# SciML/NeuralPDE.jl

Hardware: AMD Instinct MI355X
Metric: collocation-point residual+grad evals/sec, 2D Poisson 4x64 MLP (higher is better)
Workload: dtype f32, hidden-layer forward / dA / dW GEMMs as 3-piece bf16 split products (6 bf16 MFMAs per product block, fp32 accumulation; 24 mantissa bits rebuilt; the five small piece products on an accumulator of their own: zero-mean, a third of the rms error of an fp32-MFMA fmaf chain per GEMM output, tools/m

## Files before the change

### neuralpde.jl_amd/csrc/adam.cpp

```cpp
#include "resident.hpp"
#include "adam_host.hpp"
#include "adam_kernels.hpp"

using namespace pe;

namespace {

int adam_init_f32(pinn_engine& E, const float* theta) {
    const int64_t p = E.ntheta;
    const int K = (int)E.terms.size();
    if (!E.d_opt_theta) {
        E.d_opt_theta = (float*)plat_malloc(sizeof(float) * p);
        E.d_opt_m = (float*)plat_malloc(sizeof(float) * p);
        E.d_opt_v = (float*)plat_malloc(sizeof(float) * p);
        E.d_opt_out = (float*)plat_malloc(sizeof(float) * (p + K));
        E.d_w_over_n = (float*)plat_malloc(sizeof(float) * K);
        if (!E.d_opt_theta || !E.d_opt_m || !E.d_opt_v || !E.d_opt_out || !E.d_w_over_n) return fail("device allocation failed (optimiser state)");
    }
    plat_h2d(E.d_opt_theta, theta, sizeof(float) * p, E.stream);
    plat_memset(E.d_opt_m, 0, sizeof(float) * p, E.stream);
    plat_memset(E.d_opt_v, 0, sizeof(float) * p, E.stream);
    plat_sync(E.stream);
    E.opt_t = 0;
    return 0;
}

int adam_get_f32(pinn_engine& E, float* theta) {
    if (!E.d_opt_theta) return fail("pinn_adam_get: no optimiser state (call pinn_adam_init first)");
    if (plat_d2h(theta, E.d_opt_theta, sizeof(float) * E.ntheta, E.stream)) return fail("D2H copy failed");
    if (plat_sync(E.stream)) return fail(std::string("device error: ") + plat_last_error());
    return 0;
}

bool upload_c12(pinn_engine& E, int nsteps, float beta1, float beta2, std::vector<float>& c12) {
    if (!dev_grow(E.d_c12, E.c12_cap, 2 * (size_t)nsteps, E.stream)) return false;
    c12.resize(2 * (size_t)nsteps);
    for (int s = 0; s < nsteps; ++s) {
        c12[2 * s] = adam_bias(beta1, E.opt_t + s + 1);
        c12[2 * s + 1] = adam_bias(beta2, E.opt_t + s + 1);
    }
    plat_h2d(E.d_c12, c12.data(), sizeof(float) * c12.size(), E.stream);
    return true;
}

int upload_resample_table(pinn_engine& E, int* max_n) {
    std::vector<pk::TrainSampler> samp;
    *max_n = 0;
    for (auto& T : E.terms) {
        if (T.sampler == 0) continue;
        if (!T.emb_cols.empty() || T.ndata > 0 || T.pw_n > 0 || T.coupled >= 0 || T.src_root.size() > (size_t)aux::SRC_MAX) return -1;
        pk::TrainSampler S;
        std::memset(&S, 0, sizeof S);
        S.pts = T.d_pts; S.n = (int)T.n; S.d = T.d; S.kind = T.sampler; S.lb = T.d_lb; S.ub = T.d_ub;
        S.seed = sampler_seed(E, T); S.draw0 = T.draws;
        S.has_src = T.src_root.empty() ? 0 : 1;
        if (S.has_src) {
            S.src.pts = T.d_pts; S.src.N = (int)T.n; S.src.d = T.d; S.src.prog = T.d_src_prog; S.src.nops = (int)T.src_prog.size();
            S.src.nsrc = (int)T.src_root.size();
            for (int j = 0; j < S.src.nsrc; ++j) S.src.root[j] = T.src_root[(size_t)j];
            S.src.out = T.d_src; S.src.data = nullptr;
        }
        *max_n = std::max(*max_n, S.n);
        samp.push_back(S);
// ... 69 lines not shown
    const Group& G = E.groups[0];
    if (G.kind != 0 || !G.spec || G.spec->family != 1 || !G.spec->train) return false;
    if (G.ga.act != pk::ACT_TANH && G.ga.act != pk::ACT_SIGMOID) return false;
    const char* lim = std::getenv("PINN_REDUCE_DIRECT_MAX");
    const int direct_max = lim ? std::atoi(lim) : aux::REDUCE_DIRECT_MAX;
    return G.blocks <= direct_max && G.blocks <= 32 && G.blocks <= E.ncu;
}
bool train_thread_per_element(const pinn_engine& E) {
    return E.groups[0].blocks * 256 >= (int)E.ntheta + (int)E.terms.size() && E.max_contrib <= pk::TRAIN_MAX_CONTRIB;
}
bool train_eligible(pinn_engine& E) {
    if (!train_shape_ok(E) || E.ne != 0 || !E.inv_ok || !E.d_inv_ptr) return false;
    for (auto& T : E.terms)
        if (T.sampler != 0 && (!T.emb_cols.empty() || T.ndata > 0 || T.pw_n > 0 || T.coupled >= 0 || T.src_root.size() > (size_t)aux::SRC_MAX)) return false;
    if (!train_thread_per_element(E) || E.max_inv_pos > pk::TRAIN_MAX_POS) return std::getenv("PINN_TRAIN_GENERAL") != nullptr;
    return true;
}
bool eval_eligible(pinn_engine& E) {
    return E.timing_level == 0 && !std::getenv("PINN_NO_FUSED_EVAL") && train_shape_ok(E) && train_thread_per_element(E);
}

int train_common(pinn_engine& E, pk::TrainArgs& ta, const float* term_w) {
    const int K = (int)E.terms.size(), P = (int)E.ntheta;
    Group& G = E.groups[0];
    if (!E.d_bar) {
        E.d_bar = (unsigned*)plat_malloc(sizeof(unsigned) * 16);
        E.d_sums2 = (float*)plat_malloc(sizeof(float) * 2 * (size_t)std::max(K, 1));
        E.h_flag = (unsigned*)plat_host_alloc(sizeof(unsigned) * 4);
        if (!E.d_bar || !E.d_sums2 || !E.h_flag) return fail("device allocation failed (grid barrier words)");
        E.h_flag[0] = 0;
        E.bar_arrivals = 0;
        plat_memset(E.d_bar, 0, sizeof(unsigned) * 16, E.stream);
        if (plat_sync(E.stream)) return fail(std::string("device error: ") + plat_last_error());
    }
    for (size_t j = 0; j < G.terms.size(); ++j) {
        const int ti = G.terms[j];
        G.ga.terms[j].scale = (float)(2.0 * (double)(term_w ? term_w[ti] : 1.0f) / (double)E.terms[ti].n_norm);
    }
    G.ga.slabs = G.d_slabs;
    G.ga.chain = 0;
    G.active = true;
    G.timed = false;
    G.launched_blocks = G.blocks;
    G.launched_by = 0;
    std::memset(&ta, 0, sizeof ta);
    ta.slabs = G.d_slabs; ta.losspart = G.d_losspart; ta.row_ptr = E.d_gr_ptr; ta.row_ent = E.d_gr_ent;
    ta.slab_floats = G.slab_floats; ta.nblocks = G.blocks;
    ta.P = P; ta.K = K;
    ta.sums2 = E.d_sums2;
    ta.bar = E.d_bar;
    ta.hflag = E.h_flag;
    ta.cached = (train_thread_per_element(E) && E.max_inv_pos <= pk::TRAIN_MAX_POS && std::getenv("PINN_TRAIN_NO_CACHE") == nullptr) ? 1 : 0;
    if (ta.cached && (!E.d_own_r || E.own_blocks != G.blocks)) {
        const std::vector<int> own = train_thread_map(G.row_theta, G.row_ptr, G.row_off, G.blocks, P, K,
                                                      std::getenv("PINN_TRAIN_NO_COALESCE") == nullptr, &E.hist_gid);
        plat_sync(E.stream);
        plat_free(E.d_own_r);
        E.d_own_r = (int*)plat_malloc(sizeof(int) * own.size());
        if (!E.d_own_r) return fail("device allocation failed (training kernel: thread map)");
        plat_h2d(E.d_own_r, own.data(), sizeof(int) * own.size(), E.stream);
        if (plat_sync(E.stream)) return fail(std::string("device error: ") + plat_last_error());
        E.own_blocks = G.blocks;
    }
    ta.own_r = E.d_own_r;
    ta.hist_gid = ta.cached ? E.hist_gid : 0;
    return 0;
}
bool train_timed_out(pinn_engine& E) {
    if (E.h_flag[0] == 0 && std::getenv("PINN_TRAIN_FORCE_TIMEOUT") == nullptr) return false;
    E.h_flag[0] = 0;
    E.bar_arrivals = 0;
    plat_memset(E.d_bar, 0, sizeof(unsigned) * 16, E.stream);
    plat_sync(E.stream);
    E.persistent = false;
    std::fprintf(stderr, "[pinn] the persistent kernel's grid barrier timed out (its workgroups were not all resident: is the device shared?); "
                         "this handle continues with the stand-alone kernels\n");
    return true;
}

int eval_fused(pinn_engine& E, const float* d_theta, float* d_out, const float* term_w, double* lossraw) {
    Group& G = E.groups[0];
    pk::TrainArgs ta;
    if (train_common(E, ta, term_w)) return 1;
    pack_all(E, d_theta, false);
    ta.out = d_out; ta.lossraw = lossraw ? lossraw : E.d_lossraw;
    ta.eval_only = 1; ta.nsteps = 1;
    ta.arrivals0 = E.bar_arrivals;
    E.bar_arrivals += (unsigned)G.blocks;
    G.spec->train(G.ga, ta, G.blocks, E.stream);
    return 0;
}

void opt_snapshot(pinn_engine& E, bool restore) {
    const size_t P = (size_t)E.ntheta;
    float* const state[3] = {E.d_opt_theta, E.d_opt_m, E.d_opt_v};
    for (size_t j = 0; j < 3; ++j) {
        float* const bak = E.d_opt_bak + j * P;
        plat_d2d(restore ? state[j] : bak, restore ? bak : state[j], sizeof(float) * P, E.stream);
    }
}

int adam_steps_train(pinn_engine& E, int nsteps, float lr, float beta1, float beta2, float eps, const float* term_w) {
    const int P = (int)E.ntheta;
    Group& G = E.groups[0];
    pk::TrainArgs ta;
    if (train_common(E, ta, term_w)) return 1;
    std::vector<float> c12;
    if (!upload_c12(E, nsteps, beta1, beta2, c12)) return fail("device allocation failed (bias-correction table)");
    if (!E.d_opt_bak) {
        E.d_opt_bak = (float*)plat_malloc(sizeof(float) * 3 * (size_t)P);
        if (!E.d_opt_bak) return fail("device allocation failed (optimiser snapshot)");
    }
    opt_snapshot(E, false);
    std::vector<unsigned> draws0(E.terms.size());
    for (size_t t = 0; t < E.terms.size(); ++t) draws0[t] = E.terms[t].draws;
    if (plat_sync(E.stream)) return fail(std::string("device error: ") + plat_last_error());
    pack_all(E, E.d_opt_theta, false);
    ta.out = E.d_opt_out; ta.lossraw = E.d_lossraw;
    ta.theta = E.d_opt_theta; ta.m = E.d_opt_m; ta.v = E.d_opt_v;
    ta.lr = lr; ta.b1 = beta1; ta.b2 = beta2; ta.eps = eps;
    ta.inv_ptr = E.d_inv_ptr; ta.inv_pos = E.d_inv_pos; ta.packed = E.netplans[G.net].d_packed;
    ta.w_over_n = E.d_w_over_n;
    bool any_sampler = false;
    for (auto& T : E.terms) any_sampler = any_sampler || T.sampler != 0;
    ta.fenced = any_sampler ? 1 : 0;
    const char* chunk_env = std::getenv("PINN_TRAIN_CHUNK");
    const int TRAIN_CHUNK = (chunk_env && std::atoi(chunk_env) > 0) ? std::atoi(chunk_env) : 4096;
    for (int s0 = 0; s0 < nsteps; s0 += TRAIN_CHUNK) {
        ta.nsteps = std::min(TRAIN_CHUNK, nsteps - s0);
        ta.c12 = E.d_c12 + 2 * (size_t)s0;
        ta.hist = E.d_hist + s0;
        if (any_sampler) {
            int max_n = 0;
            const int ns = upload_resample_table(E, &max_n);
            if (ns < 0) return ns == -2 ? 1 : fail("pinn_adam_steps: a redrawn term of the persistent kernel carries embeddings or per-point data");
            aux::launch_resample((const pk::TrainSampler*)E.d_train_samp, ns, max_n, 0, E.stream);
            for (auto& T : E.terms) if (T.sampler != 0) T.draws += (unsigned)ta.nsteps;
            ta.nsamp = ns;
            ta.samp = (const pk::TrainSampler*)E.d_train_samp;
        }
        ta.arrivals0 = E.bar_arrivals;
        E.bar_arrivals += (unsigned)G.blocks * 2u * (unsigned)ta.nsteps;
        G.spec->train(G.ga, ta, G.blocks, E.stream);
    }
    if (plat_sync(E.stream)) return fail(std::string("device error: ") + plat_last_error());
    if (train_timed_out(E)) {
        opt_snapshot(E, true);
        for (size_t t = 0; t < E.terms.size(); ++t) E.terms[t].draws = draws0[t];
        if (plat_sync(E.stream)) return fail(std::string("device error: ") + plat_last_error());
        return 2;
    }
    E.opt_t += nsteps;
    return 0;
}

int adam_prepare(pinn_engine& E, int nsteps, const float* term_w, const char* who) {
    if (!E.d_opt_theta) return fail(std::string(who) + ": call pinn_adam_init first");
    if (nsteps <= 0) return fail(std::string(who) + ": nsteps must be positive");
    if (ensure_points(E)) return 1;
    const int K = (int)E.terms.size();
    for (auto& T : E.terms)
        if (T.sampler == 3 && T.seed == 0 && E.comm_size > 1)
            return fail(std::string(who) + ": an un-randomised Sobol design (seed 0) is the same on every rank and cannot be sharded; give the sampler a seed");
    if (!dev_grow(E.d_hist, E.hist_cap, (size_t)nsteps, E.stream)) return fail("device allocation failed (loss history)");
    std::vector<float> wn(K);
    for (int k = 0; k < K; ++k) wn[k] = (term_w ? term_w[k] : 1.0f) / (float)E.terms[k].n_norm;
    plat_h2d(E.d_w_over_n, wn.data(), sizeof(float) * K, E.stream);
    return plat_sync(E.stream) ? fail(std::string("device error: ") + plat_last_error()) : 0;
}

int adam_finish(pinn_engine** es, int ndev, int nsteps, double* loss_history, std::vector<float>* last_out = nullptr) {
    {
        pinn_engine& E = *es[0];
        DeviceScope scope(E.device);
        if (loss_history && plat_d2h(loss_history, E.d_hist, sizeof(double) * nsteps, E.stream)) return fail("D2H copy failed");
        if (last_out && plat_d2h(last_out->data(), E.d_opt_out, sizeof(float) * last_out->size(), E.stream)) return fail("D2H copy failed");
    }
    for (int i = 0; i < ndev; ++i) {
        DeviceScope scope(es[i]->device);
        if (plat_sync(es[i]->stream)) return fail(std::string("device error: ") + plat_last_error());
    }
    return 0;
}

}

int pe::eval_one_launch(pinn_engine& E, float* d_out, const float* term_w, double* lossraw) {
    if (!eval_eligible(E)) return 2;
    if (eval_fused(E, E.d_theta, d_out, term_w, lossraw)) return 1;
    if (plat_sync(E.stream)) return fail(std::string("device error: ") + plat_last_error());
    return train_timed_out(E) ? 2 : 0;
}

extern "C" {

int pinn_adam_steps(pinn_handle h, int nsteps, float lr, float beta1, float beta2, float eps, const float* term_w, double* loss_history) {
    if (!h) return fail("null handle");
    pinn_engine& E = *h;
    DeviceScope scope(E.device);
    if (E.comm && !E.comm_per_process && E.comm_size > 1)
        return fail("pinn_adam_steps: the handle belongs to a single-process communicator (pinn_comm_init_all): use pinn_adam_steps_sharded");
    if (E.f64) {
        if (nsteps <= 0) return fail("pinn_adam_steps: nsteps must be positive");
        E.adam_path = 1;
        return f64_adam_steps(E, nsteps, (double)lr, (double)beta1, (double)beta2, (double)eps, term_w, loss_history);
    }
    if (adam_prepare(E, nsteps, term_w, "pinn_adam_steps")) return 1;
    pinn_engine* es[1] = {&E};
    E.adam_path = 1;
    if (train_eligible(E)) {
        E.adam_path = 2;
        const int rc = adam_steps_train(E, nsteps, lr, beta1, beta2, eps, term_w);
        if (rc == 1) return 1;
        if (rc == 0) return adam_finish(es, 1, nsteps, loss_history);
        E.adam_path = 1;
    }
    if (adam_loop(es, 1, nsteps, lr, beta1, beta2, eps, term_w)) return 1;
    std::vector<float> gs;
    if (E.gemm_auto && !E.comm) gs.resize((size_t)E.ntheta + E.terms.size());
    if (adam_finish(es, 1, nsteps, loss_history, gs.empty() ? nullptr : &gs)) return 1;
    if (!gs.empty()) {
        measure_grad_health(E, gs.data(), term_w);
        if (gemm_auto_check(E, E.d_opt_theta, term_w, E.opt_t)) return 1;
// ... 81 lines not shown
```

### neuralpde.jl_amd/csrc/aux_kernels.hpp

```cpp
#pragma once
#include <cstdlib>
#include "aux_limits.hpp"
#include "int_limits.hpp"
#include "plat.hpp"
#include "rprog.hpp"
#include "sample_rules.hpp"

namespace aux {

#ifdef PINN_EMU
#define AUX_DEV inline
#else
#define AUX_DEV __device__ __forceinline__
#endif

struct alignas(16) F4 { float x, y, z, w; };

struct Reduce1Args {
    double* tmp[MAX_GROUPS];
    const float* slabs[MAX_GROUPS];
    const double* losspart[MAX_GROUPS];
    int slab[MAX_GROUPS], nblocks[MAX_GROUPS], nsplit[MAX_GROUPS], nent[MAX_GROUPS], active[MAX_GROUPS];
    int nwpb[MAX_GROUPS];
    int K;
};
struct Reduce2Args {
    float* out;
    float* sums;
    double* lossraw;
    const int* row_ptr;
    const int* row_grp;
    const int* row_ent;
    const double* tmp[MAX_GROUPS];
    int stride[MAX_GROUPS], nsplit[MAX_GROUPS], nent[MAX_GROUPS], active[MAX_GROUPS];
    int ent_active[MAX_GROUPS];
    int ngroups, P, K;
    int skip_grad;
    const int* perm;
};
struct ReduceOneArgs {
    const float* slabs;
    int slab, nblocks, nent;
    const int* ent_theta;
    float* out;
    float* sums;
    double* lossraw;
    int P, K;
    int nloss;
    const double* losspart[MAX_GROUPS];
    int nrows[MAX_GROUPS];
};
constexpr int RONE_CHUNKS = 32, RONE_ENT = 32;

struct ExprArgs {
    const float* pts;
    int N, d, nparams, nparams_estim;
    const float* params;
    int nslots;
    const float* jets[EXPR_MAX_SLOTS];
    float* ubar[EXPR_MAX_SLOTS];
    int nzero;
    float* zero[EXPR_MAX_SLOTS];
    const rp::Instr* prog;
    int nops, out_row;
    float scale;
    double* losspart;
    float* pslab;
    int K, term_id;
    float* resid;
    int loss_only;
    const float* data;
    const float* pw;
};
AUX_DEV float expr_point(int p, const ExprArgs& a, float (&pb)[4]) {
    float v[EXPR_MAX_ROWS], g[EXPR_MAX_ROWS];
    const int R0 = a.d + a.nparams + a.nslots;
    for (int i = 0; i < a.d; ++i) v[i] = a.pts[(size_t)p * a.d + i];
    for (int j = 0; j < a.nparams; ++j) v[a.d + j] = a.params[j];
    for (int s = 0; s < a.nslots; ++s) v[a.d + a.nparams + s] = a.jets[s][p];
    for (int q = 0; q < a.nops; ++q) {
        const rp::Instr ins = a.prog[q];
        const float va = rp::is_nullary(ins.code) ? 0.f : v[ins.a];
        const float vb = rp::is_binary(ins.code) ? v[ins.b] : 0.f;
        v[R0 + q] = (ins.code == rp::OP_DATA) ? a.data[(size_t)(int)ins.imm * a.N + p] : rp::apply<float>(ins.code, va, vb, ins.imm);
    }
    const float r = v[a.out_row];
// ... 132 lines not shown
    }
    for (int j = 0; j < a.nparams_estim; ++j) pb[j] = rbar * g[a.d + j];
    for (int k = 0; k < a.nnodes; ++k) {
        const IntNodeDev nd = a.node[k];
        const float ibar = rbar * g[RI + k] * half[k];
        const int Ri = a.d + a.nparams + nd.nslots;
        for (int q = 0; q < a.Q; ++q) {
            const int site = 1 + k * a.Q + q;
            int_integrand(p, site, nd, a, vi);
            for (int t = 0; t < Ri + nd.nops; ++t) gi[t] = 0.f;
            gi[nd.out_row] = 1.0f;
            for (int t = nd.nops - 1; t >= 0; --t) {
                const rp::Instr ins = a.iprog[nd.prog_off + t];
                if (rp::is_nullary(ins.code)) continue;
                const float vb = rp::is_binary(ins.code) ? vi[ins.b] : 0.f;
                float da, db;
                rp::adjoint<float>(ins.code, vi[ins.a], vb, vi[Ri + t], ins.imm, gi[Ri + t], da, db);
                gi[ins.a] += da;
                if (rp::is_binary(ins.code)) gi[ins.b] += db;
            }
            const float fbar = ibar * a.w[q];
            const size_t sp = (size_t)site * a.N + p;
            for (int c = 0; c < a.C; ++c) {
                const int s = a.node_slot_of_chan[k][c];
                a.ubar[(size_t)c * SN + sp] = s >= 0 ? fbar * gi[a.d + a.nparams + (s - nd.slot0)] : 0.f;
            }
            for (int j = 0; j < a.nparams_estim; ++j) pb[j] += fbar * gi[a.d + j];
        }
    }
    return rs;
}

AUX_DEV void sums_from_double_body(int k, float* out_sums, const double* raw) { out_sums[k] = (float)raw[k]; }
constexpr int PACK_BF_MAX_LAYERS = 16;
struct PackBfArgs {
    const float* theta;
    unsigned* out_fwd;
    unsigned* out_tr;
    int nhh, hp;
    float* packed;
    const int* idx;
    int n_gather;
    int woff[PACK_BF_MAX_LAYERS], nout[PACK_BF_MAX_LAYERS], nin[PACK_BF_MAX_LAYERS];
};
AUX_DEV unsigned bf16_rne(float x) {
    unsigned u;
    __builtin_memcpy(&u, &x, 4);
    if ((u & 0x7FFFFFFFu) > 0x7F800000u) return (u >> 16) | 0x40u;
    u += 0x7FFFu + ((u >> 16) & 1u);
    return u >> 16;
}
AUX_DEV float bf16_val(unsigned h) { const unsigned u = h << 16; float x; __builtin_memcpy(&x, &u, 4); return x; }
AUX_DEV unsigned bf16_piece(float v, int piece) {
    const unsigned h = bf16_rne(v);
    if (piece == 0) return h;
    const float r = v - bf16_val(h);
    const unsigned m = bf16_rne(r);
    if (piece == 1) return m;
    return bf16_rne(r - bf16_val(m));
}
AUX_DEV void pack_bf16_body(int e, const PackBfArgs& a) {
    const int mt = a.hp / 16, kbn = a.hp / 32;
    const int total = a.nhh * mt * kbn * 3 * 256;
    if (e >= 2 * total) return;
    const bool tr = e >= total;
    int r = tr ? e - total : e;
    const int j2 = r & 3; r >>= 2;
    const int lane = r & 63; r >>= 6;
    const int piece = r % 3; r /= 3;
    const int kb = r % kbn; r /= kbn;
    const int ta = r % mt; r /= mt;
    const int hl = r;
    const int g = lane >> 4, c = lane & 15;
    unsigned word = 0;
    for (int half = 0; half < 2; ++half) {
        const int j = 2 * j2 + half;
        const int other = 16 * (2 * kb + (j >> 2)) + 4 * g + (j & 3), mine = 16 * ta + c;
        const int out = tr ? other : mine, in = tr ? mine : other;
        const float v = (out < a.nout[hl] && in < a.nin[hl]) ? a.theta[a.woff[hl] + out + in * a.nout[hl]] : 0.f;
        word |= bf16_piece(v, piece) << (16 * half);
    }
    (tr ? a.out_tr : a.out_fwd)[tr ? e - total : e] = word;
}
struct EmbedArgs {
    const float* upts;
    float* pts;
    int n, du, dx;
    int src[4], is_cos[4];
    double omega[4];
};
AUX_DEV void embed_body(int p, const EmbedArgs& a) {
    if (p >= a.n) return;
    for (int i = 0; i < a.du; ++i) a.pts[(size_t)p * a.dx + i] = a.upts[(size_t)p * a.du + i];
    for (int k = 0; k < a.dx - a.du; ++k) {
        const double ph = a.omega[k] * (double)a.upts[(size_t)p * a.du + a.src[k]];
        a.pts[(size_t)p * a.dx + a.du + k] = (float)(a.is_cos[k] ? cos(ph) : sin(ph));
    }
}
AUX_DEV void pack_body(int i, float* packed, const int* idx, const float* theta) {
    const int j = idx[i];
    packed[i] = (j >= 0) ? theta[j] : 0.f;
}
AUX_DEV void params_body(int j, float* params, const float* theta, const float* defaults, int ne, int p_off) {
    params[j] = (j < ne) ? theta[p_off + j] : defaults[j];
}
#ifdef PINN_EMU
#define AUX_UNROLL8
#else
#define AUX_UNROLL8 _Pragma("unroll 8")
#endif
AUX_DEV void reduce1_body(int e4, int chunk, int g, const Reduce1Args& a) {
    if (!a.active[g] || chunk >= a.nsplit[g]) return;
    const int nb = a.nblocks[g], ns = a.nsplit[g];
    const int per = (nb + ns - 1) / ns;
    const int b0 = chunk * per, b1 = (b0 + per < nb) ? b0 + per : nb;
    double* out = a.tmp[g] + chunk;
    const int nq = a.nent[g] / 4;
    if (e4 < nq) {
        double s0 = 0.0, s1 = 0.0, s2 = 0.0, s3 = 0.0;
        const float* p = a.slabs[g] + 4 * e4;
        AUX_UNROLL8
        for (int b = b0; b < b1; ++b) {
            const F4 q = *reinterpret_cast<const F4*>(p + (size_t)b * a.slab[g]);
            s0 += (double)q.x; s1 += (double)q.y; s2 += (double)q.z; s3 += (double)q.w;
        }
        out[(size_t)(4 * e4) * ns] = s0; out[(size_t)(4 * e4 + 1) * ns] = s1;
        out[(size_t)(4 * e4 + 2) * ns] = s2; out[(size_t)(4 * e4 + 3) * ns] = s3;
    } else if (e4 < nq + a.K) {
        const int k = e4 - nq;
        const double* p = a.losspart[g] + k;
        double s = 0.0;
        AUX_UNROLL8
        for (int wv = b0 * a.nwpb[g]; wv < b1 * a.nwpb[g]; ++wv) s += p[(size_t)wv * a.K];
        out[(size_t)(a.nent[g] + k) * ns] = s;
    }
}
AUX_DEV void reduce_one_chunk(int e4, int ch, const ReduceOneArgs& a, double (&s)[4]) {
    const int per = (a.nblocks + RONE_CHUNKS - 1) / RONE_CHUNKS;
    const int b0 = ch * per, b1 = (b0 + per < a.nblocks) ? b0 + per : a.nblocks;
    s[0] = s[1] = s[2] = s[3] = 0.0;
    const float* p = a.slabs + 4 * e4;
    AUX_UNROLL8
    for (int b = b0; b < b1; ++b) {
        const F4 q = *reinterpret_cast<const F4*>(p + (size_t)b * a.slab);
        s[0] += (double)q.x; s[1] += (double)q.y; s[2] += (double)q.z; s[3] += (double)q.w;
    }
}
AUX_DEV double reduce_one_loss_part(int k, int t, int nthreads, const ReduceOneArgs& a) {
    double s = 0.0;
    for (int i = 0; i < a.nloss; ++i)
        for (int r = t; r < a.nrows[i]; r += nthreads) s += a.losspart[i][(size_t)r * a.K + k];
    return s;
}
AUX_DEV void reduce2_body(int r, const Reduce2Args& a) {
    if (r < a.P) {
        if (a.skip_grad) return;
        double s = 0.0;
        const int i0 = a.row_ptr[r], i1 = a.row_ptr[r + 1];
        for (int i = i0; i < i1; i += 4) {
            const double* t[4];
            int ns[4];
            for (int j = 0; j < 4; ++j) {
                const int ii = (i + j < i1) ? i + j : i;
                const int g = a.row_grp[ii];
                ns[j] = (i + j < i1 && a.ent_active[g]) ? a.nsplit[g] : 0;
                t[j] = a.tmp[g] + (size_t)a.row_ent[ii] * a.nsplit[g];
            }
            for (int j = 0; j < 4; ++j) {
                AUX_UNROLL8
                for (int ch = 0; ch < ns[j]; ++ch) s += t[j][ch];
            }
        }
        a.out[r] = (float)s;
    } else if (r < a.P + a.K) {
        const int k = r - a.P;
        double s = 0.0;
        for (int g = 0; g < a.ngroups; ++g) {
            if (!a.active[g]) continue;
            const double* t = a.tmp[g] + (size_t)(a.nent[g] + k) * a.nsplit[g];
            AUX_UNROLL8
            for (int ch = 0; ch < a.nsplit[g]; ++ch) s += t[ch];
        }
        a.sums[k] = (float)s;
        if (a.lossraw) a.lossraw[k] = s;
    }
}
// ... 16 lines not shown
    } else if (r < a.P + a.K) {
        const int k = r - a.P;
        double s = 0.0;
        for (int g = 0; g < a.ngroups; ++g) {
            if (!a.active[g]) continue;
            const double* p = a1.losspart[g] + k;
            const int nw = a1.nblocks[g] * a1.nwpb[g];
            AUX_UNROLL8
            for (int wv = 0; wv < nw; ++wv) s += p[(size_t)wv * a.K];
        }
        a.sums[k] = (float)s;
        if (a.lossraw) a.lossraw[k] = s;
    }
}

inline bool reduce_is_small(const Reduce1Args& a1, const Reduce2Args& a2) {
    const char* e = std::getenv("PINN_REDUCE_DIRECT_MAX");
    const int lim = e ? std::atoi(e) : REDUCE_DIRECT_MAX;
    for (int g = 0; g < a2.ngroups; ++g)
        if (a1.active[g] && a1.nblocks[g] > lim) return false;
    return true;
}
#ifdef PINN_EMU
inline void launch_pack(float* packed, const int* idx, const float* theta, int n, plat_stream) {
    for (int i = 0; i < n; ++i) pack_body(i, packed, idx, theta);
}
inline void launch_embed(const EmbedArgs& a, plat_stream) {
    for (int p = 0; p < a.n; ++p) embed_body(p, a);
}
inline void launch_params(float* params, const float* theta, const float* defaults, int np, int ne, int p_off, plat_stream) {
    for (int j = 0; j < np; ++j) params_body(j, params, theta, defaults, ne, p_off);
}
inline void launch_pack_bf16(const PackBfArgs& a, plat_stream) {
    const int total = a.nhh * (a.hp / 16) * (a.hp / 32) * 3 * 256;
    for (int i = 0; i < a.n_gather; ++i) pack_body(i, a.packed, a.idx, a.theta);
    for (int e = 0; e < 2 * total; ++e) pack_bf16_body(e, a);
}
inline void launch_sums_from_double(float* out_sums, const double* raw, int K, plat_stream) {
    for (int k = 0; k < K; ++k) sums_from_double_body(k, out_sums, raw);
}
inline void launch_sample(int kind, float* pts, int n_elems, int d, const float* lb, const float* ub, unsigned seed, unsigned draw, plat_stream) {
    for (int e = 0; e < n_elems; ++e) {
        if (kind == 3) sample_sobol_body(e, pts, d, lb, ub, seed, draw);
        else if (kind == 2) sample_lhs_body(e, pts, d, n_elems / d, lb, ub, seed, draw);
        else sample_body(e, pts, d, lb, ub, seed, draw);
    }
}
inline void launch_src(const SrcArgs& a, plat_stream) {
    for (int p = 0; p < a.N; ++p) src_point(p, a);
}
inline void launch_expr(const ExprArgs& a, int nblocks, plat_stream) {
    for (int b = 0; b < nblocks; ++b)
        for (int w = 0; w < 4; ++w) {
            double ls = 0.0;
            double ps[4] = {0, 0, 0, 0};
            for (int l = 0; l < 64; ++l) {
                const int p = (b * 4 + w) * 64 + l;
                if (p >= a.N) continue;
                float pb[4];
                const float r = expr_point(p, a, pb);
                ls += (double)r * (double)r;
                for (int j = 0; j < 4; ++j) ps[j] += (double)pb[j];
            }
            if (!a.resid) {
                a.losspart[(size_t)(b * 4 + w) * a.K + a.term_id] = ls;
                for (int j = 0; j < 4; ++j) a.pslab[(size_t)(b * 4 + w) * 4 + j] = (float)ps[j];
            }
        }
}
inline void launch_int_sites(const IntSitesArgs& a, plat_stream) {
    for (int e = 0; e < a.N * a.nnodes * a.Q; ++e) int_site_body(e, a);
}
inline void launch_int_expr(const IntExprArgs& a, int nblocks, plat_stream) {
    for (int b = 0; b < nblocks; ++b)
        for (int w = 0; w < 4; ++w) {
            double ls = 0.0;
            double ps[4] = {0, 0, 0, 0};
            for (int l = 0; l < 64; ++l) {
                const int p = (b * 4 + w) * 64 + l;
                if (p >= a.N) continue;
                float pb[4];
                const float r = int_expr_point(p, a, pb);
                ls += (double)r * (double)r;
                for (int j = 0; j < 4; ++j) ps[j] += (double)pb[j];
            }
            if (!a.resid) {
                a.losspart[(size_t)(b * 4 + w) * a.K + a.term_id] = ls;
                for (int j = 0; j < 4; ++j) a.pslab[(size_t)(b * 4 + w) * 4 + j] = (float)ps[j];
            }
        }
}
inline void launch_reduce_one(const ReduceOneArgs& a, plat_stream) {
    for (int e4 = 0; e4 < a.nent / 4; ++e4) {
        double tot[4] = {0, 0, 0, 0}, s[4];
        for (int ch = 0; ch < RONE_CHUNKS; ++ch) {
            reduce_one_chunk(e4, ch, a, s);
            for (int e = 0; e < 4; ++e) tot[e] += s[e];
        }
        for (int e = 0; e < 4; ++e)
            if (a.ent_theta[4 * e4 + e] >= 0) a.out[a.ent_theta[4 * e4 + e]] = (float)tot[e];
    }
    for (int k = 0; k < a.K; ++k) {
        double part[256], s = 0.0;
        for (int t = 0; t < 256; ++t) part[t] = reduce_one_loss_part(k, t, 256, a);
        for (int st = 128; st >= 1; st >>= 1)
            for (int t = 0; t < st; ++t) part[t] += part[t + st];
        s = part[0];
        a.sums[k] = (float)s;
        if (a.lossraw) a.lossraw[k] = s;
    }
}
inline void launch_reduce(const Reduce1Args& a1, const Reduce2Args& a2, int max_n1, int max_split, plat_stream) {
    if (reduce_is_small(a1, a2)) {
        for (int r = 0; r < a2.P + a2.K; ++r) reduce_direct_body(r, a1, a2);
        return;
    }
    for (int g = 0; g < a2.ngroups; ++g)
        for (int ch = 0; ch < max_split; ++ch)
            for (int e = 0; e < max_n1; ++e) reduce1_body(e, ch, g, a1);
    for (int r = 0; r < a2.P + a2.K; ++r) reduce2_body(r, a2);
}
#else
__global__ void k_pack(float* packed, const int* idx, const float* theta, int n) {
    const int i = blockIdx.x * blockDim.x + threadIdx.x;
    if (i < n) pack_body(i, packed, idx, theta);
}
__global__ void k_params(float* params, const float* theta, const float* defaults, int np, int ne, int p_off) {
    const int j = threadIdx.x;
    if (j < np) params_body(j, params, theta, defaults, ne, p_off);
}
__global__ void k_sample(float* pts, int n_elems, int d, const float* lb, const float* ub, unsigned seed, unsigned draw) {
    const int e = blockIdx.x * blockDim.x + threadIdx.x;
    if (e < n_elems) sample_body(e, pts, d, lb, ub, seed, draw);
}
__global__ void k_sample_lhs(float* pts, int n_elems, int d, const float* lb, const float* ub, unsigned seed, unsigned draw) {
    const int e = blockIdx.x * blockDim.x + threadIdx.x;
    if (e < n_elems) sample_lhs_body(e, pts, d, n_elems / d, lb, ub, seed, draw);
}
__global__ void k_sample_sobol(float* pts, int n_elems, int d, const float* lb, const float* ub, unsigned seed, unsigned draw) {
    const int e = blockIdx.x * blockDim.x + threadIdx.x;
    if (e < n_elems) sample_sobol_body(e, pts, d, lb, ub, seed, draw);
}
inline void launch_sample(int kind, float* pts, int n_elems, int d, const float* lb, const float* ub, unsigned seed, unsigned draw, plat_stream st) {
    if (kind == 3) hipLaunchKernelGGL(k_sample_sobol, dim3((n_elems + 255) / 256), dim3(256), 0, st, pts, n_elems, d, lb, ub, seed, draw);
// ... 4 lines not shown
    __shared__ double sh[5][256];
    const int p = blockIdx.x * 256 + threadIdx.x;
    float pb[4] = {0.f, 0.f, 0.f, 0.f};
    float r = 0.f;
    if (p < a.N) r = expr_point(p, a, pb);
    if (a.resid) return;
    sh[0][threadIdx.x] = (double)r * (double)r;
    for (int j = 0; j < 4; ++j) sh[1 + j][threadIdx.x] = (double)pb[j];
    __syncthreads();
    if (threadIdx.x < 20) {
        const int w = threadIdx.x & 3, q = threadIdx.x >> 2;
        double s = 0.0;
        for (int l = 0; l < 64; ++l) s += sh[q][w * 64 + l];
        if (q == 0) a.losspart[(size_t)(blockIdx.x * 4 + w) * a.K + a.term_id] = s;
        else a.pslab[(size_t)(blockIdx.x * 4 + w) * 4 + (q - 1)] = (float)s;
    }
}
__global__ void k_reduce1(const Reduce1Args a) {
    reduce1_body((int)(blockIdx.x * blockDim.x + threadIdx.x), (int)blockIdx.y, (int)blockIdx.z, a);
}
__global__ void k_reduce2(const Reduce2Args a) {
    reduce2_body((int)(blockIdx.x * blockDim.x + threadIdx.x), a);
}
inline void launch_pack(float* packed, const int* idx, const float* theta, int n, plat_stream st) {
    hipLaunchKernelGGL(k_pack, dim3((n + 255) / 256), dim3(256), 0, st, packed, idx, theta, n);
}
__global__ void k_embed(const EmbedArgs a) { embed_body((int)(blockIdx.x * blockDim.x + threadIdx.x), a); }
inline void launch_embed(const EmbedArgs& a, plat_stream st) {
    hipLaunchKernelGGL(k_embed, dim3((a.n + 255) / 256), dim3(256), 0, st, a);
}
inline void launch_params(float* params, const float* theta, const float* defaults, int np, int ne, int p_off, plat_stream st) {
    if (np > 0) hipLaunchKernelGGL(k_params, dim3(1), dim3(64), 0, st, params, theta, defaults, np, ne, p_off);
}
__global__ void k_pack_bf16(const PackBfArgs a) {
    const int e = (int)(blockIdx.x * blockDim.x + threadIdx.x);
    if (e < a.n_gather) pack_body(e, a.packed, a.idx, a.theta);
    else pack_bf16_body(e - a.n_gather, a);
}
inline void launch_pack_bf16(const PackBfArgs& a, plat_stream st) {
    const int total = a.nhh * (a.hp / 16) * (a.hp / 32) * 3 * 256;
    hipLaunchKernelGGL(k_pack_bf16, dim3((a.n_gather + 2 * total + 255) / 256), dim3(256), 0, st, a);
}
__global__ void k_sums_from_double(float* out_sums, const double* raw, int K) {
    const int k = (int)(blockIdx.x * blockDim.x + threadIdx.x);
    if (k < K) sums_from_double_body(k, out_sums, raw);
}
inline void launch_sums_from_double(float* out_sums, const double* raw, int K, plat_stream st) {
    hipLaunchKernelGGL(k_sums_from_double, dim3((K + 63) / 64), dim3(64), 0, st, out_sums, raw, K);
}
__global__ void __launch_bounds__(256) k_src(const SrcArgs a) {
    const int p = blockIdx.x * 256 + threadIdx.x;
    if (p < a.N) src_point(p, a);
}
inline void launch_src(const SrcArgs& a, plat_stream st) {
    hipLaunchKernelGGL(k_src, dim3((a.N + 255) / 256), dim3(256), 0, st, a);
}
inline void launch_expr(const ExprArgs& a, int nblocks, plat_stream st) {
    hipLaunchKernelGGL(k_expr, dim3(nblocks), dim3(256), 0, st, a);
}
__global__ void __launch_bounds__(256) k_int_sites(const IntSitesArgs a) { int_site_body((int)(blockIdx.x * 256 + threadIdx.x), a); }
inline void launch_int_sites(const IntSitesArgs& a, plat_stream st) {
    hipLaunchKernelGGL(k_int_sites, dim3((a.N * a.nnodes * a.Q + 255) / 256), dim3(256), 0, st, a);
}
__global__ void __launch_bounds__(256) k_int_expr(const IntExprArgs a) {
    __shared__ double sh[5][256];
    const int p = blockIdx.x * 256 + threadIdx.x;
    float pb[4] = {0.f, 0.f, 0.f, 0.f};
    float r = 0.f;
    if (p < a.N) r = int_expr_point(p, a, pb);
    if (a.resid) return;
    sh[0][threadIdx.x] = (double)r * (double)r;
    for (int j = 0; j < 4; ++j) sh[1 + j][threadIdx.x] = (double)pb[j];
    __syncthreads();
    if (threadIdx.x < 20) {
        const int w = threadIdx.x & 3, q = threadIdx.x >> 2;
        double s = 0.0;
        for (int l = 0; l < 64; ++l) s += sh[q][w * 64 + l];
        if (q == 0) a.losspart[(size_t)(blockIdx.x * 4 + w) * a.K + a.term_id] = s;
        else a.pslab[(size_t)(blockIdx.x * 4 + w) * 4 + (q - 1)] = (float)s;
    }
}
inline void launch_int_expr(const IntExprArgs& a, int nblocks, plat_stream st) {
    hipLaunchKernelGGL(k_int_expr, dim3(nblocks), dim3(256), 0, st, a);
}
__global__ void __launch_bounds__(256) k_reduce_one(const ReduceOneArgs a) {
    __shared__ double sh[RONE_CHUNKS][RONE_ENT + 1];
    const int tid = (int)threadIdx.x;
    const int nentblocks = (a.nent + RONE_ENT - 1) / RONE_ENT;
    if ((int)blockIdx.x < nentblocks) {
        const int j = tid & 7, ch = tid >> 3;
        const int e4 = (int)blockIdx.x * (RONE_ENT / 4) + j;
        double s[4] = {0.0, 0.0, 0.0, 0.0};
        if (4 * e4 < a.nent) reduce_one_chunk(e4, ch, a, s);
        for (int e = 0; e < 4; ++e) sh[ch][4 * j + e] = s[e];
        __syncthreads();
        if (tid < RONE_ENT) {
            const int ent = (int)blockIdx.x * RONE_ENT + tid;
            if (ent < a.nent) {
                double tot = 0.0;
                for (int c2 = 0; c2 < RONE_CHUNKS; ++c2) tot += sh[c2][tid];
                const int th = a.ent_theta[ent];
                if (th >= 0) a.out[th] = (float)tot;
            }
        }
    } else {
        const int k = (int)blockIdx.x - nentblocks;
        double* part = &sh[0][0];
        part[tid] = reduce_one_loss_part(k, tid, 256, a);
        __syncthreads();
        for (int st = 128; st >= 1; st >>= 1) {
            if (tid < st) part[tid] += part[tid + st];
            __syncthreads();
        }
        if (tid == 0) {
            a.sums[k] = (float)part[0];
            if (a.lossraw) a.lossraw[k] = part[0];
        }
    }
}
inline void launch_reduce_one(const ReduceOneArgs& a, plat_stream st) {
    hipLaunchKernelGGL(k_reduce_one, dim3((a.nent + RONE_ENT - 1) / RONE_ENT + a.K), dim3(256), 0, st, a);
}
__global__ void k_reduce_direct(const Reduce1Args a1, const Reduce2Args a2) {
    reduce_direct_body((int)(blockIdx.x * blockDim.x + threadIdx.x), a1, a2);
}
inline void launch_reduce(const Reduce1Args& a1, const Reduce2Args& a2, int max_n1, int max_split, plat_stream st) {
    if (reduce_is_small(a1, a2)) {
        hipLaunchKernelGGL(k_reduce_direct, dim3((a2.P + a2.K + 63) / 64), dim3(64), 0, st, a1, a2);
        return;
    }
    hipLaunchKernelGGL(k_reduce1, dim3((max_n1 + 255) / 256, max_split, a2.ngroups), dim3(256), 0, st, a1);
    hipLaunchKernelGGL(k_reduce2, dim3((a2.P + a2.K + 255) / 256), dim3(256), 0, st, a2);
}
#endif

}
```

### neuralpde.jl_amd/csrc/comm.cpp

```cpp
#include "engine_types.hpp"

using namespace pe;

#ifndef PINN_EMU
#include <dlfcn.h>
#include <rccl/rccl.h>

namespace {
struct Rccl {
    void* lib = nullptr;
    ncclResult_t (*GetUniqueId)(ncclUniqueId*) = nullptr;
    ncclResult_t (*CommInitRank)(ncclComm_t*, int, ncclUniqueId, int) = nullptr;
    ncclResult_t (*CommInitAll)(ncclComm_t*, int, const int*) = nullptr;
    ncclResult_t (*CommDestroy)(ncclComm_t) = nullptr;
    ncclResult_t (*AllReduce)(const void*, void*, size_t, ncclDataType_t, ncclRedOp_t, ncclComm_t, hipStream_t) = nullptr;
    ncclResult_t (*GroupStart)() = nullptr;
    ncclResult_t (*GroupEnd)() = nullptr;
    const char* (*GetErrorString)(ncclResult_t) = nullptr;
    std::string err;
};
Rccl& rccl() {
    static Rccl R = [] {
        Rccl r;
        for (const char* name : {"librccl.so.1", "librccl.so", "/opt/rocm/lib/librccl.so.1"}) {
// ... 251 lines not shown
        rc = comm_all_reduce_f64(es, 1, vec, E.ntheta + (int64_t)E.terms.size());
    }
    E.stream = saved;
    return rc;
}

int pinn_loss_grad_sharded_f64(pinn_handle* hs, int ndev, const double* theta, int64_t p, const double* term_w, double* term_losses, double* grad) {
    if (!hs || ndev < 1 || !theta) return fail("pinn_loss_grad_sharded_f64: null argument");
    for (int i = 0; i < ndev; ++i) {
        if (!hs[i] || !hs[i]->comm || hs[i]->comm_size != ndev || hs[i]->comm_rank != i)
            return fail("pinn_loss_grad_sharded_f64: pass the handles of one pinn_comm_init_all communicator, in rank order");
        if (!hs[i]->f64) return fail("pinn_loss_grad_sharded_f64: every handle must be in the float64 evaluation mode");
        if (p != hs[i]->ntheta) return fail("pinn_loss_grad_sharded_f64: theta length mismatch");
    }
    const int64_t P = hs[0]->ntheta;
    const int K = (int)hs[0]->terms.size();
    std::vector<double*> vec(ndev);
    for (int i = 0; i < ndev; ++i) {
        pinn_engine& E = *hs[i];
        DeviceScope scope(E.device);
        if (check_shards(E)) return 1;
        if (f64_eval_sharded_local(E, theta, term_w, &vec[i])) return 1;
    }
    if (comm_all_reduce_f64(hs, ndev, vec.data(), P + K)) return 1;
    std::vector<double> out((size_t)(P + K));
    {
        pinn_engine& E0 = *hs[0];
        DeviceScope scope(E0.device);
        if (plat_d2h(out.data(), vec[0], sizeof(double) * (size_t)(P + K), E0.stream)) return fail("D2H copy failed");
    }
    for (int i = 0; i < ndev; ++i) {
        DeviceScope scope(hs[i]->device);
        if (plat_sync(hs[i]->stream)) return fail(std::string("device error: ") + plat_last_error());
    }
    if (term_losses) for (int k = 0; k < K; ++k) term_losses[k] = out[(size_t)P + k] / (double)hs[0]->terms[k].n_norm;
    if (grad) std::memcpy(grad, out.data(), sizeof(double) * (size_t)P);
    return 0;
}

int pinn_loss_grad_sharded_device(pinn_handle h, const float* d_theta, const float* term_w, float* d_out, void* stream) {
    if (!h || !d_theta || !d_out) return fail("pinn_loss_grad_sharded_device: null argument");
    pinn_engine& E = *h;
    if (!E.comm) return fail("pinn_loss_grad_sharded_device: the handle has no communicator (pinn_comm_init_rank / pinn_comm_init_all)");
    DeviceScope scope(E.device);
    if (check_shards(E)) return 1;
    plat_stream st = (plat_stream)stream;
    plat_stream saved = E.stream;
    E.stream = st;
    int rc = run_loss_grad(E, d_theta, d_out, term_w, -1, true);
    E.stream = saved;
    if (rc) return rc;
    E.timing_valid = E.timing_level >= 2;
    if (!E.comm_per_process && E.comm_size > 1)
        return fail("pinn_loss_grad_sharded_device: the handle belongs to a single-process communicator (pinn_comm_init_all): use pinn_loss_grad_sharded");
    {
        pinn_engine* es[1] = {&E};
        float* vec[1] = {d_out};
        double* raw[1] = {E.d_lossraw};
        E.stream = st;
        rc = comm_all_reduce(es, 1, vec, raw);
        E.stream = saved;
        if (rc) return rc;
    }
    sums_from_double(d_out + E.ntheta, E.d_lossraw, (int)E.terms.size(), st);
    return 0;
}
// ... 2 lines not shown
    if (!hs || ndev < 1 || !theta) return fail("pinn_loss_grad_sharded: null argument");
    for (int i = 0; i < ndev; ++i) {
        if (!hs[i] || !hs[i]->comm || hs[i]->comm_size != ndev || hs[i]->comm_rank != i)
            return fail("pinn_loss_grad_sharded: pass the handles of one pinn_comm_init_all communicator, in rank order");
        if (i > 0 && hs[i]->comm != hs[0]->comm
#ifndef PINN_EMU
            && false
#endif
        ) return fail("pinn_loss_grad_sharded: handles of different communicators");
    }
    const int64_t P = hs[0]->ntheta;
    const int K = (int)hs[0]->terms.size();
    for (int i = 0; i < ndev; ++i) {
        pinn_engine& E = *hs[i];
        DeviceScope scope(E.device);
        if (check_shards(E) || upload_theta(E, theta, p)) return 1;
        if (run_loss_grad(E, E.d_theta, E.d_out, term_w, -1, false)) return 1;
    }
    {
        std::vector<float*> vec(ndev);
        std::vector<double*> raw(ndev);
        for (int i = 0; i < ndev; ++i) { vec[i] = hs[i]->d_out; raw[i] = hs[i]->d_lossraw; }
        if (comm_all_reduce(hs, ndev, vec.data(), raw.data())) return 1;
    }
    pinn_engine& E0 = *hs[0];
    {
        DeviceScope scope(E0.device);
        if (plat_d2h(E0.hp_out, E0.d_out, sizeof(float) * (P + K), E0.stream)) return fail("D2H copy failed");
        if (plat_d2h(E0.hp_raw, E0.d_lossraw, sizeof(double) * K, E0.stream)) return fail("D2H copy failed");
    }
    for (int i = 0; i < ndev; ++i) {
        DeviceScope scope(hs[i]->device);
        if (plat_sync(hs[i]->stream)) return fail(std::string("device error: ") + plat_last_error());
    }
    if (term_losses)
        for (int k = 0; k < K; ++k) term_losses[k] = E0.hp_raw[k] / (double)E0.terms[k].n_norm;
    if (grad) std::memcpy(grad, E0.hp_out, sizeof(float) * P);
    return 0;
}

}
```

### neuralpde.jl_amd/csrc/engine.cpp

```cpp
#include "resident.hpp"
#include "aux_kernels.hpp"

#ifdef PINN_EMU
namespace wv {
thread_local void (*emu_barrier_hook)(void*) = nullptr;
thread_local void* emu_barrier_ctx = nullptr;
thread_local void (*emu_grid_hook)(void*) = nullptr;
thread_local void* emu_grid_ctx = nullptr;
}
#endif

namespace pk {
std::deque<SpecInfo>& registry() {
    static std::deque<SpecInfo> r;
    return r;
}
std::deque<PairInfo>& pair_registry() {
    static std::deque<PairInfo> r;
    return r;
}
}

namespace pe {
thread_local std::string g_err;
// ... 35 lines not shown
    aux::launch_int_sites(a, E.stream);
}
void eval_sources(pinn_engine& E, Term& T) {
    if (T.src_root.empty() || T.coupled >= 0) return;
    aux::SrcArgs a;
    std::memset(&a, 0, sizeof a);
    a.pts = T.d_pts; a.N = (int)T.n; a.d = T.d; a.prog = T.d_src_prog; a.nops = (int)T.src_prog.size();
    a.nsrc = (int)T.src_root.size();
    for (int j = 0; j < a.nsrc; ++j) a.root[j] = T.src_root[j];
    a.out = T.d_src;
    a.data = T.d_data;
    if (T.ndata > 0 && T.data_n != T.n) return;
    aux::launch_src(a, E.stream);
}

}

void pe::redraw_term(pinn_engine& E, Term& T, bool sources) {
    aux::launch_sample(T.sampler, user_pts(T), (int)(T.n * T.d_user), T.d_user, T.d_lb, T.d_ub, sampler_seed(E, T), T.draws++, E.stream);
    embed_points(E, T);
    if (sources) eval_sources(E, T);
}

int pe::ensure_points(pinn_engine& E) {
    for (size_t t = 0; t < E.terms.size(); ++t) {
        if (!E.terms[t].d_pts || E.terms[t].n <= 0)
            return fail("term " + std::to_string(t) + " has no collocation points (call pinn_set_points first)");
        if (E.terms[t].ndata > 0 && E.terms[t].data_n != E.terms[t].n)
            return fail("term " + std::to_string(t) + " uses per-point data channels but none are installed for its current point set (call pinn_set_point_data after pinn_set_points)");
    }
    return 0;
}

void pe::pack_all(pinn_engine& E, const float* d_theta, bool packed_fresh) {
    const float* th = d_theta ? d_theta : E.d_theta;
    for (size_t n = 0; n < E.nets.size(); ++n) {
        NetPlan& NP = E.netplans[n];
        if (!NP.spec) continue;
        if (NP.spec->family == 3) { NP.cur = th + E.nets[n].theta_off; continue; }
        NP.cur = NP.d_packed;
        const bool gather = !packed_fresh;
        if (gather && !NP.spec->BFX) aux::launch_pack(NP.d_packed, NP.d_pack_idx, th, NP.npacked, E.stream);
        if (NP.spec->BFX) {
            const Net& N = E.nets[n];
            aux::PackBfArgs pa;
            std::memset(&pa, 0, sizeof pa);
            pa.theta = th; pa.out_fwd = (unsigned*)(NP.d_packed + NP.spec->OFF_WB); pa.out_tr = (unsigned*)(NP.d_packed + NP.spec->OFF_WTB);
            pa.nhh = NP.spec->NHH; pa.hp = NP.spec->HP;
            pa.packed = NP.d_packed; pa.idx = NP.d_pack_idx; pa.n_gather = gather ? NP.spec->OFF_WB : 0;
            if (pa.nhh > aux::PACK_BF_MAX_LAYERS) return;
            int o = N.theta_off;
            for (size_t j = 0; j + 1 < N.sizes.size(); ++j) {
                if (j >= 1 && j <= (size_t)pa.nhh) { pa.woff[j - 1] = o; pa.nin[j - 1] = N.sizes[j]; pa.nout[j - 1] = N.sizes[j + 1]; }
                o += N.sizes[j + 1] * N.sizes[j] + N.sizes[j + 1];
            }
            aux::launch_pack_bf16(pa, E.stream);
        }
    }
    for (auto& G : E.groups) G.ga.packed = E.netplans[G.net].cur;
    aux::launch_params(E.d_params, th, E.d_defaults, E.np, E.ne, E.p_theta_off, E.stream);
}

namespace {

aux::ExprArgs expr_args(pinn_engine& E, Coupled& Cp, float scale, float* resid) {
    Term& T = E.terms[Cp.term];
    aux::ExprArgs a;
    std::memset(&a, 0, sizeof a);
    a.pts = T.d_pts; a.N = (int)T.n; a.d = T.d; a.nparams = E.np; a.nparams_estim = E.ne; a.params = E.d_params;
    a.nslots = (int)T.slots.size();
    std::vector<std::vector<char>> used(Cp.nets.size());
    for (size_t i = 0; i < Cp.nets.size(); ++i) used[i].assign(E.groups[Cp.groups[i]].spec->C, 0);
    for (int si = 0; si < a.nslots; ++si) {
        const int i = Cp.slot_net[si], ch = T.chan_of_slot[si];
        a.jets[si] = Cp.d_jets[i] + (size_t)ch * T.n;
        a.ubar[si] = Cp.d_ubar[i] + (size_t)ch * T.n;
        used[i][ch] = 1;
    }
    for (size_t i = 0; i < Cp.nets.size(); ++i)
        for (size_t ch = 0; ch < used[i].size(); ++ch)
            if (!used[i][ch] && a.nzero < aux::EXPR_MAX_SLOTS) a.zero[a.nzero++] = Cp.d_ubar[i] + ch * T.n;
    a.prog = Cp.d_prog; a.nops = (int)T.ops.size(); a.out_row = T.out_row; a.scale = scale;
    a.losspart = Cp.d_losspart; a.pslab = Cp.d_pslab; a.K = (int)E.terms.size(); a.term_id = Cp.term; a.resid = resid;
    a.data = T.d_data;
    a.pw = (T.pw_n == T.n && T.pw_n > 0) ? T.d_pw : nullptr;
    return a;
}

aux::IntExprArgs int_expr_args(pinn_engine& E, Coupled& Cp, float scale, float* resid) {
// ... 23 lines not shown
    return a;
}

int upload_int_rule(pinn_engine& E, int q) {
    std::vector<double> xi((size_t)q), w((size_t)q);
    const double PI = 3.14159265358979323846264338327950288;
    for (int i = 0; i < q; ++i) {
        double x = -std::cos(PI * (i + 0.75) / (q + 0.5)), dp = 1.0;
        for (int it = 0; it < 100; ++it) {
            double p0 = 1.0, p1 = x;
            for (int n = 2; n <= q; ++n) { const double p2 = ((2.0 * n - 1.0) * x * p1 - (n - 1.0) * p0) / n; p0 = p1; p1 = p2; }
            dp = q * (x * p1 - p0) / (x * x - 1.0);
            const double dx = p1 / dp;
            x -= dx;
            if (std::fabs(dx) < 1e-16) break;
        }
        {
            double p0 = 1.0, p1 = x;
            for (int n = 2; n <= q; ++n) { const double p2 = ((2.0 * n - 1.0) * x * p1 - (n - 1.0) * p0) / n; p0 = p1; p1 = p2; }
            dp = q * (x * p1 - p0) / (x * x - 1.0);
        }
        xi[(size_t)i] = x;
        w[(size_t)i] = 2.0 / ((1.0 - x * x) * dp * dp);
    }
    std::vector<float> wf(w.begin(), w.end());
    if (!E.d_int_xi) {
        E.d_int_xi = (double*)plat_malloc(sizeof(double) * aux::INT_MAX_Q);
        E.d_int_w = (float*)plat_malloc(sizeof(float) * aux::INT_MAX_Q);
        if (!E.d_int_xi || !E.d_int_w) return fail("device allocation failed (quadrature rule)");
    }
    plat_h2d(E.d_int_xi, xi.data(), sizeof(double) * q, E.stream);
    plat_h2d(E.d_int_w, wf.data(), sizeof(float) * q, E.stream);
    if (plat_sync(E.stream)) return fail(std::string("device error: ") + plat_last_error());
    return 0;
}

}

int pe::run_loss_grad(pinn_engine& E, const float* d_theta, float* d_out, const float* term_w, int only_term , bool timing,
                  double* lossraw , bool packed_fresh, bool loss_only, float* d_sums) {
    if (!d_sums) d_sums = d_out + E.ntheta;
    if (ensure_points(E)) return 1;
    const int K = (int)E.terms.size();
    const bool phase_ev = timing && E.timing_level >= 2;
    auto group_ev = [&](size_t g) { return timing && E.timing_level >= 1 && (E.timing_group < 0 || E.timing_group == (int)g); };
    if (phase_ev) plat_event_record(E.ev0, E.stream);
    pack_all(E, d_theta, packed_fresh);
    if (phase_ev) plat_event_record(E.ev1, E.stream);
    aux::Reduce1Args a1;
    aux::Reduce2Args a2;
    std::memset(&a1, 0, sizeof a1);
    std::memset(&a2, 0, sizeof a2);
    int max_n1 = 1, max_split = 1;
    auto scale_of = [&](int ti) -> float {
        const float w = term_w ? term_w[ti] : 1.0f;
        const bool on = (only_term < 0 || only_term == ti);
        return on ? (float)(2.0 * (double)w / (double)E.terms[ti].n_norm) : 0.f;
    };
    int nfused_active = 0;
    bool all_small = true;
    for (auto& G : E.groups) {
        bool on = false;
        for (int ti : G.terms) on = on || (only_term < 0 || only_term == ti);
        if (G.kind == 0 && on) {
            ++nfused_active;
            const int per_round = G.max_blocks * (G.spec->family == 2 ? 1 : 4);
            if (2 * G.ga.ntiles > 3 * per_round) all_small = false;
        }
    }
    static const bool want_concurrent = std::getenv("PINN_CONCURRENT_GROUPS") != nullptr;
    const bool concurrent = want_concurrent && nfused_active >= 2 && all_small;
    static const bool no_chain = std::getenv("PINN_NO_CHAIN") != nullptr;
    const bool no_merge = std::getenv("PINN_NO_MERGE") != nullptr;
    const bool may_merge = !no_merge && !no_chain && !concurrent && only_term < 0;
    int nforked = 0;
    int nslabsets = 0, slabset_group = -1;
    if (concurrent) plat_event_record(E.ev_fork, E.stream);
    for (size_t g = 0; g < E.groups.size(); ++g) {
        Group& G = E.groups[g];
        bool any = false;
// ... 46 lines not shown
            ga_one.sub_terms0 = (int)G.terms.size();
            ga_one.sub_tiles0 = G.ga.ntiles;
            ga_one.ntiles = G.ga.ntiles + T2.ga.ntiles;
            ga_one.scratch = mu->d_scratch;
            ga_one.scr_stride = mu->pair->SCR;
            ga_one.losspart = mu->d_losspart;
            a1.losspart[g] = mu->d_losspart;
            ga_one.chain = 0;
            blocks = std::max(1, std::min(loss_only ? E.ncu * mu->pair->WG_FWD : mu->max_blocks, ga_one.ntiles));
            ga_launch = &ga_one;
        }
        G.launched_blocks = blocks;
        G.launched_by = (int)g;
        const int epe = G.spec->family == 1 ? 4 : 1;
        const int nsplit_g = std::max(1, std::min(REDUCE_SPLIT, (int)std::ceil(std::sqrt((double)blocks / epe))));
        a1.slab[g] = G.slab_floats; a1.nblocks[g] = blocks; a1.nsplit[g] = nsplit_g; a1.nent[g] = nent; a1.active[g] = any; a1.nwpb[g] = G.spec->NW;
        a2.stride[g] = nent + K; a2.nsplit[g] = nsplit_g; a2.nent[g] = nent; a2.active[g] = any;
        a2.ent_active[g] = any && !chained && !loss_only;
        if (!any) continue;
        if (a2.ent_active[g]) { ++nslabsets; slabset_group = (int)g; }
        max_n1 = std::max(max_n1, nent / 4 + K);
        max_split = std::max(max_split, nsplit_g);
        if (G.kind == 1) {
            G.spec->launch(G.ga, (G.use_rec && !loss_only) ? pk::MODE_FWDREC : pk::MODE_FWD,
                           std::max(1, std::min(E.ncu * G.spec->WG_FWD, G.spec->family == 1 ? (G.ga.ntiles + 3) / 4 : G.ga.ntiles)), E.stream);
            continue;
        }
        if (G.kind == 2) continue;
        plat_stream st = E.stream;
        const bool forked = concurrent && nforked++ > 0;
        if (forked) {
            st = E.aux_stream[nforked % 2];
            plat_stream_wait_event(st, E.ev_fork);
        }
        if (group_ev(g)) plat_event_record(G.ev_a, st);
        if (merged_head) mu->pair->launch(*ga_launch, loss_only ? pk::MODE_LOSS : pk::MODE_FUSED, blocks, st);
        else if (loss_only) {
            const int tiles = ga_launch->ntiles;
            const int fb = std::max(1, std::min(E.ncu * G.spec->WG_FWD, G.spec->family == 1 ? (tiles + 3) / 4 : tiles));
            a1.nblocks[g] = fb;
            G.launched_blocks = fb;
            G.spec->launch(*ga_launch, pk::MODE_LOSS, fb, st);
        } else G.spec->launch(*ga_launch, pk::MODE_FUSED, blocks, st);
        if (group_ev(g)) plat_event_record(G.ev_b, st);
        G.timed = group_ev(g);
        if (forked) {
            plat_event_record(E.ev_join[g], st);
            plat_stream_wait_event(E.stream, E.ev_join[g]);
        }
    }
    bool coupled_active = false;
    for (size_t c = 0; c < E.coupled.size(); ++c) {
        Coupled& Cp = E.coupled[c];
        const int g = (int)(E.groups.size() + c);
        const bool on = (only_term < 0 || only_term == Cp.term);
        const int nsplit = std::min(REDUCE_SPLIT, Cp.blocks);
        const int nent = loss_only ? 0 : 16;
        a1.tmp[g] = Cp.d_tmp; a1.slabs[g] = Cp.d_pslab; a1.losspart[g] = Cp.d_losspart;
        a1.slab[g] = 16; a1.nblocks[g] = Cp.blocks; a1.nsplit[g] = nsplit; a1.nent[g] = nent; a1.active[g] = on; a1.nwpb[g] = 4;
        a2.tmp[g] = Cp.d_tmp; a2.stride[g] = nent + K; a2.nsplit[g] = nsplit; a2.nent[g] = nent; a2.active[g] = on; a2.ent_active[g] = on && !loss_only;
        bool groups_active = false;
        for (int gi : Cp.groups) groups_active = groups_active || E.groups[gi].active;
        if (!groups_active) continue;
        coupled_active = true;
        if (Cp.tail >= 0) {
            Group& G = E.groups[Cp.groups[Cp.tail]];
// ... 8 lines not shown
            if (group_ev((size_t)Cp.groups[Cp.tail])) plat_event_record(G.ev_b, E.stream);
            G.timed = group_ev((size_t)Cp.groups[Cp.tail]);
            continue;
        }
        max_n1 = std::max(max_n1, nent / 4 + K);
        max_split = std::max(max_split, nsplit);
        if (!E.terms[Cp.term].inodes.empty()) {
            aux::IntExprArgs ia = int_expr_args(E, Cp, scale_of(Cp.term), nullptr);
            ia.loss_only = loss_only ? 1 : 0;
            aux::launch_int_expr(ia, Cp.blocks, E.stream);
            continue;
        }
        aux::ExprArgs ea = expr_args(E, Cp, scale_of(Cp.term), nullptr);
        ea.loss_only = loss_only ? 1 : 0;
        aux::launch_expr(ea, Cp.blocks, E.stream);
    }
    for (size_t g = 0; g < E.groups.size() && !loss_only; ++g) {
        Group& G = E.groups[g];
        if (G.kind != 1 || !G.active) continue;
        if (group_ev(g)) plat_event_record(G.ev_a, E.stream);
        G.spec->launch(G.ga, G.use_rec ? pk::MODE_GRADREC : pk::MODE_GRADIN, G.blocks, E.stream);
        if (group_ev(g)) plat_event_record(G.ev_b, E.stream);
        G.timed = group_ev(g);
    }
    if (phase_ev) plat_event_record(E.ev2, E.stream);
    a1.K = K;
    a2.out = d_out; a2.sums = d_sums; a2.lossraw = lossraw ? lossraw : E.d_lossraw; a2.row_ptr = E.d_gr_ptr; a2.row_grp = E.d_gr_grp; a2.row_ent = E.d_gr_ent;
    a2.ngroups = (int)(E.groups.size() + E.coupled.size()); a2.P = (int)E.ntheta; a2.K = K;
    a2.skip_grad = loss_only ? 1 : 0;
    a2.perm = std::getenv("PINN_NO_REDUCE_PERM") ? nullptr : E.d_red_perm;
    const bool no_reduce_one = std::getenv("PINN_NO_REDUCE_ONE") != nullptr;
    const Group* RG = (nslabsets == 1 && !coupled_active && !loss_only && !no_reduce_one) ? &E.groups[slabset_group] : nullptr;
    const bool one_kernel = ((RG && RG->d_ent_theta && RG->ent_covers_theta) || (loss_only && !no_reduce_one)) && !aux::reduce_is_small(a1, a2);
    if (one_kernel) {
        aux::ReduceOneArgs ro;
        std::memset(&ro, 0, sizeof ro);
        if (RG) { ro.slabs = RG->d_slabs; ro.slab = RG->slab_floats; ro.nblocks = a1.nblocks[slabset_group]; ro.nent = RG->nent; ro.ent_theta = RG->d_ent_theta; }
        ro.out = d_out; ro.sums = d_sums; ro.lossraw = a2.lossraw; ro.P = (int)E.ntheta; ro.K = K;
        for (int g = 0; g < a2.ngroups; ++g)
            if (a1.active[g]) { ro.losspart[ro.nloss] = a1.losspart[g]; ro.nrows[ro.nloss] = a1.nblocks[g] * a1.nwpb[g]; ++ro.nloss; }
        aux::launch_reduce_one(ro, E.stream);
    } else {
        aux::launch_reduce(a1, a2, max_n1, max_split, E.stream);
    }
    if (phase_ev) plat_event_record(E.ev3, E.stream);
    { const std::string e = jit_take_launch_error(); if (!e.empty()) return fail(e); }
    return 0;
}

void pe::sums_from_double(float* d_out_sums, const double* d_raw, int K, plat_stream st) { aux::launch_sums_from_double(d_out_sums, d_raw, K, st); }

int pe::upload_theta(pinn_engine& E, const float* theta, int64_t p) {
    if (p != E.ntheta) return fail("theta length " + std::to_string(p) + " != ntheta " + std::to_string(E.ntheta));
    std::memcpy(E.hp_theta, theta, sizeof(float) * p);
    if (plat_h2d(E.d_theta, E.hp_theta, sizeof(float) * p, E.stream)) return fail(std::string("H2D copy of theta failed: ") + plat_last_error());
    return 0;
}

extern "C" {

const char* pinn_backend(void) { return plat_name(); }
int pinn_abi_version(void) { return 1; }
const char* pinn_last_error(void) { return g_err.c_str(); }

int pinn_create(const char* descriptor, pinn_handle* out) { return pinn_create_on(descriptor, -1, out); }

int pinn_create_on(const char* descriptor, int device, pinn_handle* out) {
    if (!descriptor || !out) return fail("pinn_create: null argument");
    *out = nullptr;
    std::string err;
    if (plat_init(err)) return fail(err);
    if (device >= plat_device_count()) return fail("pinn_create_on: device " + std::to_string(device) + " does not exist (" + std::to_string(plat_device_count()) + " visible)");
    const int dev = device < 0 ? plat_get_device() : device;
    DeviceScope scope(dev);
    std::unique_ptr<pinn_engine> E(new pinn_engine());
    E->device = dev;
    if (const char* gm = std::getenv("PINN_GEMM")) {
        if (std::string(gm) == "fp32") E->gemm = pk::GEMM_FP32;
        else if (std::string(gm) == "split") E->gemm = pk::GEMM_SPLIT;
        else return fail(std::string("PINN_GEMM must be \"split\" or \"fp32\", not \"") + gm + "\"");
    }
    if (parse_descriptor(descriptor, *E)) return 1;
    E->terms0 = E->terms;
    E->ncu = plat_num_cus();
    E->stream = plat_stream_create();
    const int K = (int)E->terms.size();
    E->d_theta = (float*)plat_malloc(sizeof(float) * E->ntheta);
    E->d_params = (float*)plat_malloc(sizeof(float) * pk::MAX_PARAMS);
    E->d_defaults = (float*)plat_malloc(sizeof(float) * pk::MAX_PARAMS);
    E->d_lossraw = (double*)plat_malloc(sizeof(double) * K);
    E->d_out = (float*)plat_malloc(sizeof(float) * (E->ntheta + K));
    plat_event_create(E->ev0); plat_event_create(E->ev1); plat_event_create(E->ev2); plat_event_create(E->ev3);
    plat_event_create(E->ev_fork);
    for (auto& e : E->ev_join) plat_event_create(e);
    for (auto& st : E->aux_stream) st = plat_stream_create();
    if (!E->d_theta || !E->d_params || !E->d_defaults || !E->d_lossraw || !E->d_out) {
        pinn_destroy(E.release());
        return fail("device allocation failed");
    }
    plat_h2d(E->d_defaults, E->p_defaults32.data(), sizeof(float) * pk::MAX_PARAMS, E->stream);
    E->hp_theta = (float*)plat_host_alloc(sizeof(float) * (2 * E->ntheta + K + 2) + sizeof(double) * K);
    if (!E->hp_theta) {
        pinn_destroy(E.release());
        return fail("pinned host allocation failed");
    }
    E->hp_out = E->hp_theta + E->ntheta;
    E->hp_raw = (double*)(E->hp_theta + ((2 * E->ntheta + K + 1) / 2) * 2);
    bool any_int = false;
    for (auto& T : E->terms) any_int = any_int || !T.inodes.empty();
    if ((any_int && upload_int_rule(*E, E->int_q)) || build_plan(*E)) {
        const std::string msg = g_err;
        pinn_destroy(E.release());
        g_err = msg;
        return 1;
    }
    *out = E.release();
    return 0;
}

int pinn_destroy(pinn_handle h) {
    if (!h) return 0;
    pinn_engine& E = *h;
    DeviceScope scope(E.device);
    pinn_comm_destroy(h);
    plat_sync(E.stream);
    hmc_free(E);
    lbfgs_free(E);
    ens_free(E);
    f64_destroy(E);
    free_plan(E);
    for (auto& T : E.terms) { plat_free(T.d_pts); plat_free(T.d_upts); plat_free(T.d_resid); plat_free(T.d_lb); plat_free(T.d_ub); plat_free(T.d_data); plat_free(T.d_pw); }
    plat_free(E.d_opt_theta); plat_free(E.d_opt_m); plat_free(E.d_opt_v); plat_free(E.d_opt_out); plat_free(E.d_w_over_n); plat_free(E.d_hist); plat_free(E.d_c12); plat_free(E.d_bar); plat_free(E.d_sums2); plat_free(E.d_own_r); plat_free(E.d_train_samp); plat_free(E.d_opt_bak); plat_host_free(E.h_flag);
    plat_free(E.d_theta); plat_free(E.d_params); plat_free(E.d_defaults); plat_free(E.d_lossraw);
    plat_free(E.d_int_xi); plat_free(E.d_int_w);
    plat_free(E.d_out); plat_free(E.d_phi_pts); plat_free(E.d_phi_out); plat_free(E.d_phi_scr);
    plat_host_free(E.hp_theta);
    plat_event_destroy(E.ev0); plat_event_destroy(E.ev1); plat_event_destroy(E.ev2); plat_event_destroy(E.ev3);
    plat_event_destroy(E.ev_fork);
    for (auto& e : E.ev_join) plat_event_destroy(e);
    for (auto& st : E.aux_stream) plat_stream_destroy(st);
    if (E.own_stream) plat_stream_destroy(E.stream);
    delete h;
    return 0;
}

int pinn_num_terms(pinn_handle h) { return h ? (int)h->terms.size() : -1; }
int64_t pinn_num_theta(pinn_handle h) { return h ? h->ntheta : -1; }

static int term_installed(pinn_engine& E, int term);
static int set_points_impl(pinn_handle h, int term, const float* pts, int64_t n, int64_t n_norm, bool device) {
    if (!h) return fail("null handle");
    pinn_engine& E = *h;
    DeviceScope scope(E.device);
    if (term < 0 || term >= (int)E.terms.size()) return fail("pinn_set_points: term index out of range");
    if (!pts || n <= 0) return fail("pinn_set_points: empty point set (the reference's mean(abs2, .) over an empty set is NaN; refusing)");
    Term& T = E.terms[term];
    if (n * T.d >= (int64_t)1 << 31) return fail("pinn_set_points: point set too large for 32-bit indexing; shard it");
    const int64_t S = T.sites();
    if (S > 1 && n * S * std::max(T.d, aux::INT_MAX_C) >= (int64_t)1 << 31)
        return fail("pinn_set_points: the site set of integral term " + std::to_string(term) + " (" + std::to_string(n) + " points x (1 + " +
                    std::to_string(T.inodes.size()) + " integral node(s) x " + std::to_string(T.int_q) + " quadrature nodes) = " + std::to_string(n * S) +
                    " sites) exceeds what one launch group takes (32-bit indexing of its jet channels); shard the point set or lower integral_nodes");
    if (n > T.pts_cap || !T.d_pts) {
        plat_sync(E.stream);
        plat_free(T.d_pts);
        plat_free(T.d_upts);
        T.d_upts = nullptr;
// ... 65 lines not shown
    if (Cp.cap_blocks < Cp.blocks) {
        plat_free(Cp.d_losspart); plat_free(Cp.d_pslab);
        Cp.d_losspart = (double*)plat_malloc(sizeof(double) * (size_t)Cp.blocks * 4 * K);
        Cp.d_pslab = (float*)plat_malloc(sizeof(float) * (size_t)Cp.blocks * 16);
        if (!Cp.d_losspart || !Cp.d_pslab) return fail("device allocation failed (coupled partials)");
        plat_memset(Cp.d_losspart, 0, sizeof(double) * (size_t)Cp.blocks * 4 * K, E.stream);
        plat_memset(Cp.d_pslab, 0, sizeof(float) * (size_t)Cp.blocks * 16, E.stream);
        plat_sync(E.stream);
        Cp.cap_blocks = Cp.blocks;
    }
    for (int gi : Cp.groups) retile(E, gi);
    return 0;
}
int pinn_set_points(pinn_handle h, int term, const float* pts, int64_t n, int64_t n_norm) { return set_points_impl(h, term, pts, n, n_norm, false); }
int pinn_set_points_device(pinn_handle h, int term, const float* d_pts, int64_t n, int64_t n_norm) { return set_points_impl(h, term, d_pts, n, n_norm, true); }
int pinn_set_points_f64(pinn_handle h, int term, const double* pts, int64_t n, int64_t n_norm) {
    if (!h || !pts || n <= 0) return fail("pinn_set_points_f64: null argument / empty point set");
    if (term < 0 || term >= (int)h->terms.size()) return fail("pinn_set_points_f64: term index out of range");
    auto p32 = as<float>(pts, (size_t)n * h->terms[term].d_user);
    if (set_points_impl(h, term, p32.get(), n, n_norm, false)) return 1;
    if (!h->f64) return 0;
    DeviceScope scope(h->device);
    return f64_set_points(*h, term, pts, n);
}

extern "C++" int pe::eval_and_sync(pinn_engine& E, float* d_out, const float* term_w, double* lossraw, bool timing) {
    E.eval_path = 1;
    if (ensure_points(E)) return 1;
    const int one = eval_one_launch(E, d_out, term_w, lossraw);
    if (one == 1) return 1;
    if (one == 0) { E.eval_path = 2; return 0; }
    if (run_loss_grad(E, E.d_theta, d_out, term_w, -1, timing, lossraw, false, false)) return 1;
    if (plat_sync(E.stream)) return fail(std::string("device error: ") + plat_last_error());
    return 0;
}

static int loss_grad_f32(pinn_engine& E, const float* theta, const float* term_w, double* term_losses, float* grad) {
    const int K = (int)E.terms.size();
    if (upload_theta(E, theta, E.ntheta)) return 1;
    if (grad) {
        if (eval_and_sync(E, E.hp_out, term_w, E.hp_raw, true)) return 1;
    } else {
        if (run_loss_grad(E, E.d_theta, E.hp_out, term_w, -1, true, E.hp_raw, false, true)) return 1;
        if (plat_sync(E.stream)) return fail(std::string("device error: ") + plat_last_error());
    }
    E.timing_valid = E.timing_level >= 2;
    if (term_losses)
        for (int k = 0; k < K; ++k) term_losses[k] = E.hp_raw[k] / (double)E.terms[k].n_norm;
    if (grad) std::memcpy(grad, E.hp_out, sizeof(float) * E.ntheta);
    if (grad && E.gemm_auto) {
        std::vector<float> gs((size_t)E.ntheta + K);
        std::memcpy(gs.data(), E.hp_out, sizeof(float) * E.ntheta);
        for (int k = 0; k < K; ++k) gs[(size_t)E.ntheta + k] = (float)E.hp_raw[k];
        measure_grad_health(E, gs.data(), term_w);
        if (gemm_auto_check(E, E.d_theta, term_w, ++E.eval_count)) return 1;
    }
    return 0;
}

static void loglik_from_sse(const pinn_engine& E, const double* stds, const double* sse, double* loglik, double* grad_std) {
    const int K = (int)E.terms.size();
    double ll = 0.0;
    for (int k = 0; k < K; ++k) {
        const double N = (double)E.terms[k].n, sd = stds[k];
        ll += -0.5 * N * std::log(2.0 * 3.14159265358979323846) - N * std::log(sd) - sse[k] / (2.0 * sd * sd);
        if (grad_std) grad_std[k] = -N / sd + sse[k] / (sd * sd * sd);
    }
    *loglik = ll;
}
static int loglik_f64(pinn_engine& E, const double* theta, const double* stds, double* loglik, double* grad_theta, double* grad_std) {
    const int K = (int)E.terms.size();
    std::vector<double> w(K), L(K), g(grad_theta ? (size_t)E.ntheta : 0);
    for (int k = 0; k < K; ++k) w[k] = (double)E.terms[k].n_norm / (2.0 * stds[k] * stds[k]);
    if (f64_eval(E, theta, w.data(), L.data(), grad_theta ? g.data() : nullptr)) return 1;
    for (int k = 0; k < K; ++k) L[k] *= (double)E.terms[k].n_norm;
    loglik_from_sse(E, stds, L.data(), loglik, grad_std);
    if (grad_theta) for (int64_t i = 0; i < E.ntheta; ++i) grad_theta[i] = -g[(size_t)i];
    return 0;
}

static int loglik_f32(pinn_engine& E, const float* theta, const double* stds, double* loglik, float* grad_theta, double* grad_std) {
    const int K = (int)E.terms.size();
    std::vector<float> w(K);
    for (int k = 0; k < K; ++k) w[k] = (float)((double)E.terms[k].n_norm / (2.0 * stds[k] * stds[k]));
    if (upload_theta(E, theta, E.ntheta)) return 1;
    if (run_loss_grad(E, E.d_theta, E.hp_out, w.data(), -1, false, E.hp_raw)) return 1;
    if (plat_sync(E.stream)) return fail(std::string("device error: ") + plat_last_error());
    loglik_from_sse(E, stds, E.hp_raw, loglik, grad_std);
    if (grad_theta)
        for (int64_t i = 0; i < E.ntheta; ++i) grad_theta[i] = -E.hp_out[i];
    return 0;
}

static int term_grads_f64(pinn_engine& E, const double* theta, double* term_losses, double* term_grads) {
    const int K = (int)E.terms.size();
    const int64_t p = E.ntheta;
    std::vector<double> w(K), L(K);
    for (int k = 0; k < K; ++k) {
        for (int j = 0; j < K; ++j) w[j] = (j == k) ? 1.0 : 0.0;
        if (f64_eval(E, theta, w.data(), L.data(), term_grads + (size_t)k * p)) return 1;
        if (term_losses) term_losses[k] = L[k];
    }
    return 0;
}

static int term_grads_f32(pinn_engine& E, const float* theta, double* term_losses, float* term_grads) {
    const int K = (int)E.terms.size();
    const int64_t p = E.ntheta;
    if (upload_theta(E, theta, p)) return 1;
    for (int k = 0; k < K; ++k) {
        if (run_loss_grad(E, E.d_theta, E.hp_out, nullptr, k, false, E.hp_raw)) return 1;
        if (plat_sync(E.stream)) return fail(std::string("device error: ") + plat_last_error());
        std::memcpy(term_grads + (size_t)k * p, E.hp_out, sizeof(float) * p);
        if (term_losses) term_losses[k] = E.hp_raw[k] / (double)E.terms[k].n_norm;
    }
    return 0;
}

int pinn_loss_grad_device(pinn_handle h, const float* d_theta, const float* term_w, float* d_out, void* stream) {
    if (!h || !d_theta || !d_out) return fail("pinn_loss_grad_device: null argument");
    pinn_engine& E = *h;
    DeviceScope scope(E.device);
    const int K = (int)E.terms.size();
    plat_stream user = (plat_stream)stream;
    plat_stream saved = E.stream;
    E.stream = user;
    int rc = E.f64 ? f64_eval_from_device_f32(E, d_theta, term_w, d_out, true) : run_loss_grad(E, d_theta, d_out, term_w, -1, true);
    E.stream = saved;
    if (rc && g_err.empty()) return fail("pinn_loss_grad_device failed");
    E.timing_valid = (rc == 0) && E.timing_level >= 2;
    return rc;
}

int pinn_loss_grad_device_f64(pinn_handle h, const double* d_theta, const float* term_w, double* d_out, void* stream) {
    if (!h || !d_theta || !d_out) return fail("pinn_loss_grad_device_f64: null argument");
    pinn_engine& E = *h;
    if (!E.f64) return fail("pinn_loss_grad_device_f64: the handle is not in the float64 evaluation mode (pinn_set_option(h, \"precision\", \"f64\"))");
    DeviceScope scope(E.device);
    plat_stream saved = E.stream;
    E.stream = (plat_stream)stream;
    const int rc = f64_eval_from_device_f64(E, d_theta, term_w, d_out);
    E.stream = saved;
    if (rc && g_err.empty()) return fail("pinn_loss_grad_device_f64 failed");
    return rc;
}
// ... 15 lines not shown
    if (!h || group < 0 || group >= (int)h->groups.size()) return -1;
    return h->groups[group].launched_by;
}

static int residual_f32(pinn_engine& E, int term, const float* theta, float* r) {
    Term& T = E.terms[term];
    if (!T.d_pts) return fail("pinn_residual: term has no points");
    if (upload_theta(E, theta, E.ntheta)) return 1;
    pack_all(E);
    jit_take_launch_error();
    if (T.resid_cap < T.n) {
        plat_free(T.d_resid);
        T.d_resid = (float*)plat_malloc(sizeof(float) * T.n);
        T.resid_cap = T.n;
        if (!T.d_resid) return fail("device allocation failed (residual)");
    }
    if (T.coupled >= 0) {
        Coupled& Cp = E.coupled[T.coupled];
        for (int gi : Cp.groups) {
            Group& G = E.groups[gi];
            pk::GroupArgs ga = G.ga;
            int j = 0;
            for (size_t q = 0; q < G.terms.size(); ++q) if (G.terms[q] == term) j = (int)q;
            ga.nterms = 1;
            ga.terms[0] = G.ga.terms[j];
            ga.terms[0].tile0 = 0;
            ga.ntiles = ga.terms[0].ntiles;
            G.spec->launch(ga, pk::MODE_FWD, std::max(1, std::min(E.ncu * G.spec->WG_FWD, G.spec->family == 1 ? (ga.ntiles + 3) / 4 : ga.ntiles)), E.stream);
        }
        if (!T.inodes.empty()) aux::launch_int_expr(int_expr_args(E, Cp, 0.f, T.d_resid), Cp.blocks, E.stream);
        else aux::launch_expr(expr_args(E, Cp, 0.f, T.d_resid), Cp.blocks, E.stream);
        if (plat_d2h(r, T.d_resid, sizeof(float) * T.n, E.stream)) return fail("D2H copy failed");
        if (plat_sync(E.stream)) return fail(std::string("device error: ") + plat_last_error());
        { const std::string le = jit_take_launch_error(); if (!le.empty()) return fail("pinn_residual: " + le); }
        return 0;
    }
    Group& G = E.groups[T.group];
    pk::GroupArgs ga = G.ga;
    ga.nterms = 1;
    ga.terms[0] = G.ga.terms[T.slot_in_group];
    ga.terms[0].tile0 = 0;
    ga.terms[0].out = T.d_resid;
    ga.ntiles = ga.terms[0].ntiles;
    const int blocks = std::max(1, std::min(E.ncu * G.spec->WG_FWD, G.spec->family == 1 ? (ga.ntiles + 3) / 4 : ga.ntiles));
    G.spec->launch(ga, pk::MODE_RESID, blocks, E.stream);
    if (plat_d2h(r, T.d_resid, sizeof(float) * T.n, E.stream)) return fail("D2H copy failed");
    if (plat_sync(E.stream)) return fail(std::string("device error: ") + plat_last_error());
    { const std::string le = jit_take_launch_error(); if (!le.empty()) return fail("pinn_residual: " + le); }
    return 0;
}

static int forward_jets(pinn_engine& E, int net, const pk::SpecInfo* sp, const float* theta, const float* pts, int64_t n) {
    const Net& N = E.nets[net];
    if (!E.netplans[net].spec) return fail("network is not used by any term");
    if (sp->family != E.netplans[net].spec->family || sp->PACKED != E.netplans[net].spec->PACKED)
        return fail("internal: forward kernel and the network's packed weight image disagree");
    if (upload_theta(E, theta, E.ntheta)) return 1;
    pack_all(E);
    jit_take_launch_error();
    if (E.phi_cap < n || E.phi_chan < sp->C) {
        plat_sync(E.stream);
        plat_free(E.d_phi_pts); plat_free(E.d_phi_out);
        E.phi_cap = std::max(E.phi_cap, n);
        E.phi_chan = std::max(E.phi_chan, sp->C);
        E.d_phi_pts = (float*)plat_malloc(sizeof(float) * E.phi_cap * 8);
        E.d_phi_out = (float*)plat_malloc(sizeof(float) * E.phi_cap * E.phi_chan);
        if (!E.d_phi_pts || !E.d_phi_out) { E.phi_cap = 0; E.phi_chan = 0; return fail("device allocation failed (phi)"); }
    }
    if (!N.emb_idx.empty()) {
        const std::vector<float> feats = N.features(pts, n);
        plat_h2d(E.d_phi_pts, feats.data(), sizeof(float) * feats.size(), E.stream);
        plat_sync(E.stream);
    } else
        plat_h2d(E.d_phi_pts, pts, sizeof(float) * n * N.sizes[0], E.stream);
    pk::GroupArgs ga;
    std::memset(&ga, 0, sizeof ga);
    ga.packed = E.netplans[net].cur;
    ga.params = E.d_params;
    ga.nterms = 1;
    ga.nterms_total = 1;
// ... 20 lines not shown
        ga.dgm_modes = N.sizes[1];
        ga.dgm_npad = ga.ntiles * 64;
        ga.dgm_nparams = N.nparams();
    }
    const int blocks = std::max(1, std::min(E.ncu * sp->WG_FWD, sp->family == 1 ? (ga.ntiles + 3) / 4 : ga.ntiles));
    sp->launch(ga, pk::MODE_FWD, blocks, E.stream);
    { const std::string le = jit_take_launch_error(); if (!le.empty()) return fail("forward kernel: " + le); }
    return 0;
}

static int net_eval_f32(const char* who, pinn_engine& E, int net, const float* theta, const float* pts, int64_t n, int order, const int* axes, float* out) {
    GemmScope gs(E.gemm);
    const Net& N = E.nets[net];
    if (!E.netplans[net].spec) return fail(std::string(who) + ": network is not used by any term");
    Slot sl;
    sl.net = net; sl.order = order; sl.lap = 0;
    for (int a = 0; a < MAX_DERIV_ORDER; ++a) sl.axes[a] = a < order ? axes[a] : 0;
    std::sort(sl.axes, sl.axes + order);
    unsigned need_first = 0, need_hi = 0;
    std::vector<std::pair<int, int>> need_pairs;
    if (slot_is_general(sl)) need_hi = GEN_FLAG | (unsigned)gen_set_id({slot_mi(sl)});
    else {
        for (int a = 0; a < order; ++a) need_first |= 1u << sl.axes[a];
        if (order >= 2) need_pairs.push_back({sl.axes[0], sl.axes[1]});
        if (order >= 3) need_hi = (unsigned)order << (4 * sl.axes[0]);
    }
    const pk::SpecInfo* sp = ensure_spec(N, need_first, need_pairs, need_hi, E.netplans[net].spec->family);
    if (!sp) return fail(std::string(who) + (order == 0 ? ": no value-only kernel" : ": no kernel carries this derivative") + " for this network shape (" + g_err + ")");
    const int ch = chan_of(*sp, sl);
    if (ch < 0) return fail("internal: derivative has no channel");
    if (forward_jets(E, net, sp, theta, pts, n)) return 1;
    if (plat_d2h(out, E.d_phi_out + (size_t)ch * n, sizeof(float) * n, E.stream)) return fail("D2H copy failed");
    if (plat_sync(E.stream)) return fail(std::string("device error: ") + plat_last_error());
    return 0;
}

int pinn_set_sampler(pinn_handle h, int term, int kind, const float* lb, const float* ub, int64_t n, uint64_t seed) {
    if (!h) return fail("null handle");
    pinn_engine& E = *h;
    DeviceScope scope(E.device);
    if (term < 0 || term >= (int)E.terms.size()) return fail("pinn_set_sampler: term index out of range");
    Term& T = E.terms[term];
    if (kind < 0 || kind > 3) return fail("pinn_set_sampler: kind must be 0 (fixed set), 1 (uniform), 2 (Latin hypercube) or 3 (Sobol)");
    if (kind == 3 && T.d_user > 8) return fail("pinn_set_sampler: the Sobol sampler covers up to 8 axes");
    if (kind == 0) { T.sampler = 0; return 0; }
    if (!lb || !ub || n <= 0) return fail("pinn_set_sampler: bounds and a positive point count are required");
    if (!T.d_lb) { T.d_lb = (float*)plat_malloc(sizeof(float) * 8); T.d_ub = (float*)plat_malloc(sizeof(float) * 8); }
    if (!T.d_lb || !T.d_ub) return fail("device allocation failed (sampler)");
    plat_h2d(T.d_lb, lb, sizeof(float) * T.d_user, E.stream);
    plat_h2d(T.d_ub, ub, sizeof(float) * T.d_user, E.stream);
    T.seed = (unsigned)(seed ^ (seed >> 32)) + 0x9E3779B9U * (unsigned)(term + 1);
    if (kind == 3 && seed == 0) T.seed = 0;
    T.draws = 0;
    std::vector<float> tmp((size_t)n * T.d_user, 0.f);
    if (set_points_impl(h, term, tmp.data(), n, 0, false)) return 1;
    T.sampler = kind;
    aux::launch_sample(kind, user_pts(T), (int)(n * T.d_user), T.d_user, T.d_lb, T.d_ub, T.seed, T.draws++, E.stream);
    embed_points(E, T);
    eval_sources(E, T);
    if (E.f64 && f64_points_from_device(E, term)) return 1;
    plat_sync(E.stream);
    return 0;
}

int pinn_set_point_data(pinn_handle h, int term, const float* data, int ndata, int64_t n) {
    if (!h || !data) return fail("pinn_set_point_data: null argument");
    pinn_engine& E = *h;
    DeviceScope scope(E.device);
    if (term < 0 || term >= (int)E.terms.size()) return fail("pinn_set_point_data: term index out of range");
    Term& T = E.terms[term];
    if (T.ndata == 0) return fail("pinn_set_point_data: the term's residual has no DATA channels");
    if (ndata != T.ndata) return fail("pinn_set_point_data: the term's residual uses " + std::to_string(T.ndata) + " data channel(s)");
    if (!T.d_pts || n != T.n) return fail("pinn_set_point_data: the term holds " + std::to_string(T.n) + " points (install the point set first)");
    if (T.sampler != 0) return fail("pinn_set_point_data: per-point data cannot follow a resampled point set");
    plat_sync(E.stream);
    if (T.data_cap < n) {
        plat_free(T.d_data);
        T.d_data = (float*)plat_malloc(sizeof(float) * (size_t)T.ndata * n);
        if (!T.d_data) return fail("device allocation failed (point data)");
        T.data_cap = n;
    }
    if (plat_h2d(T.d_data, data, sizeof(float) * (size_t)T.ndata * n, E.stream)) return fail("H2D copy of point data failed");
    T.data_n = n;
    eval_sources(E, T);
    if (plat_sync(E.stream)) return fail(std::string("device error: ") + plat_last_error());
    return f64_set_point_data(E, term, nullptr);
}
int pinn_set_point_data_f64(pinn_handle h, int term, const double* data, int ndata, int64_t n) {
    if (!h || !data || ndata <= 0 || n <= 0) return fail("pinn_set_point_data_f64: null argument / empty data");
    auto d32 = as<float>(data, (size_t)ndata * (size_t)n);
    if (pinn_set_point_data(h, term, d32.get(), ndata, n)) return 1;
    if (!h->f64) return 0;
    DeviceScope scope(h->device);
    return f64_set_point_data(*h, term, data);
}

int pinn_set_point_weights(pinn_handle h, int term, const float* w, int64_t n) {
    if (!h) return fail("pinn_set_point_weights: null handle");
    pinn_engine& E = *h;
    DeviceScope scope(E.device);
    if (term < 0 || term >= (int)E.terms.size()) return fail("pinn_set_point_weights: term index out of range");
    Term& T = E.terms[term];
    plat_sync(E.stream);
    if (!w) {
        T.pw_n = 0;
    } else {
        if (!T.d_pts || n != T.n) return fail("pinn_set_point_weights: the term holds " + std::to_string(T.n) + " points (install the point set first)");
        if (T.sampler != 0) return fail("pinn_set_point_weights: weights cannot follow a resampled point set");
        std::vector<float> s((size_t)n);
        for (int64_t i = 0; i < n; ++i) {
            if (!(w[i] >= 0.f)) return fail("pinn_set_point_weights: weights must be non-negative");
            s[i] = (float)std::sqrt((double)w[i] * (double)T.n_norm);
        }
        if (T.pw_cap < n) {
            plat_free(T.d_pw);
            T.d_pw = (float*)plat_malloc(sizeof(float) * (size_t)n);
            if (!T.d_pw) return fail("device allocation failed (point weights)");
            T.pw_cap = n;
        }
        if (plat_h2d(T.d_pw, s.data(), sizeof(float) * (size_t)n, E.stream)) return fail("H2D copy of point weights failed");
        if (plat_sync(E.stream)) return fail(std::string("device error: ") + plat_last_error());
        T.pw_n = n;
    }
    if (T.coupled < 0) retile(E, T.group);
    else for (int gi : E.coupled[T.coupled].groups) retile(E, gi);
    return 0;
}

int pinn_get_points(pinn_handle h, int term, float* pts, int64_t n) {
    if (!h || !pts) return fail("pinn_get_points: null argument");
    pinn_engine& E = *h;
    DeviceScope scope(E.device);
    if (term < 0 || term >= (int)E.terms.size()) return fail("pinn_get_points: term index out of range");
    Term& T = E.terms[term];
    if (!T.d_pts || n != T.n) return fail("pinn_get_points: the term holds " + std::to_string(T.n) + " points");
    if (plat_d2h(pts, user_pts(T), sizeof(float) * (size_t)n * T.d_user, E.stream)) return fail("D2H copy failed");
    if (plat_sync(E.stream)) return fail(std::string("device error: ") + plat_last_error());
    return 0;
}

extern "C++" int pe::replan_gemm(pinn_engine& E, int mode) {
    if (mode == E.gemm) return 0;
    if (plat_sync(E.stream)) return fail(std::string("device error: ") + plat_last_error());
    const int prev = E.gemm;
    free_plan(E);
    E.gemm = mode;
    int rc = build_plan(E);
    if (rc) {
        const std::string why = g_err;
        free_plan(E);
        E.gemm = prev;
        if (build_plan(E)) return fail("pinn_set_option: the kernel plan could not be rebuilt (" + why + "); the handle is unusable");
        g_err = why;
    }
    for (size_t t = 0; t < E.terms.size(); ++t)
        if (E.terms[t].d_pts && E.terms[t].n > 0 && term_installed(E, (int)t)) return 1;
    for (size_t t = 0; t < E.terms.size(); ++t) {
        Term& T = E.terms[t];
        if (T.ndata > 0 && T.data_n == T.n && T.n > 0) eval_sources(E, T);
    }
    if (plat_sync(E.stream)) return fail(std::string("device error: ") + plat_last_error());
    return rc;
}

constexpr double GEMM_DELTA_UP = 1e-5, GEMM_DELTA_DOWN = 3e-6;
constexpr long long GEMM_CHECK_EVERY = 1000;
extern "C++" void pe::measure_grad_health(pinn_engine& E, const float* grad_and_sums, const float* term_w) {
    const int K = (int)E.terms.size();
    const int64_t P = E.ntheta;
    double g2 = 0.0, L = 0.0;
    for (int64_t i = 0; i < P; ++i) g2 += (double)grad_and_sums[i] * (double)grad_and_sums[i];
    for (int k = 0; k < K; ++k) L += (term_w ? (double)term_w[k] : 1.0) * (double)grad_and_sums[P + k] / (double)E.terms[k].n_norm;
    E.grad_health = L > 0.0 ? std::sqrt(g2) / std::sqrt(L) : -1.0;
}
extern "C++" int pe::gemm_auto_check(pinn_engine& E, const float* d_theta, const float* term_w, long long now) {
    if (!E.gemm_auto || E.f64 || E.comm) return 0;
    if (E.gemm_check_t >= 0 && now - E.gemm_check_t < GEMM_CHECK_EVERY && now >= E.gemm_check_t) return 0;
    bool has_twin = false;
    for (const NetPlan& NP : E.netplans) has_twin = has_twin || (NP.spec && NP.spec->family == 2 && NP.spec->twin);
    if (!has_twin) return 0;
    const int64_t P = E.ntheta;
    const int start = E.gemm;
    std::vector<float> ga((size_t)P), gb((size_t)P);
    if (run_loss_grad(E, d_theta, E.d_out, term_w, -1, false)) return 1;
    if (plat_d2h(ga.data(), E.d_out, sizeof(float) * P, E.stream) || plat_sync(E.stream)) return fail("D2H copy failed");
    if (replan_gemm(E, start == pk::GEMM_SPLIT ? pk::GEMM_FP32 : pk::GEMM_SPLIT)) return 1;
    if (E.gemm == start) return 0;
    if (run_loss_grad(E, d_theta, E.d_out, term_w, -1, false)) return 1;
    if (plat_d2h(gb.data(), E.d_out, sizeof(float) * P, E.stream) || plat_sync(E.stream)) return fail("D2H copy failed");
    const std::vector<float>& gs = start == pk::GEMM_SPLIT ? ga : gb;
    const std::vector<float>& gf = start == pk::GEMM_SPLIT ? gb : ga;
    double d2 = 0.0, n2 = 0.0;
    for (int64_t i = 0; i < P; ++i) { const double d = (double)gs[(size_t)i] - (double)gf[(size_t)i]; d2 += d * d; n2 += (double)gf[(size_t)i] * (double)gf[(size_t)i]; }
    E.gemm_delta = n2 > 0.0 ? std::sqrt(d2 / n2) : 0.0;
    E.gemm_check_t = now;
    const int want = (start == pk::GEMM_SPLIT) ? (E.gemm_delta > GEMM_DELTA_UP ? pk::GEMM_FP32 : pk::GEMM_SPLIT)
                                               : (E.gemm_delta < GEMM_DELTA_DOWN ? pk::GEMM_SPLIT : pk::GEMM_FP32);
    return replan_gemm(E, want);
}

int pinn_set_option(pinn_handle h, const char* name, const char* value) {
    if (!h || !name || !value) return fail("pinn_set_option: null argument");
    pinn_engine& E = *h;
    DeviceScope scope(E.device);
    const std::string k = name, v = value;
    if (k == "gemm") {
        if (v == "split") { E.gemm_auto = false; return replan_gemm(E, pk::GEMM_SPLIT); }
        if (v == "fp32") { E.gemm_auto = false; return replan_gemm(E, pk::GEMM_FP32); }
        if (v == "auto") { E.gemm_auto = true; E.gemm_check_t = -1; return 0; }
        return fail("pinn_set_option: gemm must be \"split\", \"fp32\" or \"auto\"");
    }
    if (k == "precision") {
        if (v == "f64") return f64_enable(E);
        if (v == "f32") { plat_sync(E.stream); f64_destroy(E); return 0; }
        return fail("pinn_set_option: precision must be \"f32\" or \"f64\"");
    }
    if (k == "persistent") {
        if (v == "on" || v == "1") { E.persistent = true; return 0; }
        if (v == "off" || v == "0") { E.persistent = false; return 0; }
        return fail("pinn_set_option: persistent must be \"on\" or \"off\"");
    }
    if (k == "integral_nodes") {
        char* end = nullptr;
        const long q = std::strtol(v.c_str(), &end, 10);
        if (v.empty() || *end || q < 2 || q > aux::INT_MAX_Q) return fail("pinn_set_option: integral_nodes must be an integer in 2.." + std::to_string(aux::INT_MAX_Q) + ", not \"" + v + "\"");
        if (plat_sync(E.stream)) return fail(std::string("device error: ") + plat_last_error());
        for (auto& T : E.terms)
            if (!T.inodes.empty() && T.d_pts && T.n > 0 && T.n * (1 + (int64_t)T.inodes.size() * q) * std::max(T.d, aux::INT_MAX_C) >= (int64_t)1 << 31)
                return fail("pinn_set_option: integral_nodes = " + std::to_string(q) + " makes a site set of " + std::to_string(T.n * (1 + (int64_t)T.inodes.size() * q)) +
                            " sites, more than one launch group takes; the handle keeps " + std::to_string(E.int_q));
        bool any = false;
        for (auto& T : E.terms) any = any || !T.inodes.empty();
        if (!any) { E.int_q = (int)q; return 0; }
        std::vector<float*> nbuf(E.terms.size(), nullptr);
        for (size_t t = 0; t < E.terms.size(); ++t) {
            Term& T = E.terms[t];
            if (T.inodes.empty() || !T.d_pts || T.n <= 0) continue;
            const int64_t new_sites = 1 + (int64_t)T.inodes.size() * q;
            if (T.n * new_sites <= T.pts_cap * (int64_t)T.sites()) continue;
            nbuf[t] = (float*)plat_malloc(sizeof(float) * (size_t)T.n * new_sites * T.d);
            if (!nbuf[t]) {
                for (float* b : nbuf) plat_free(b);
                return fail("pinn_set_option: device allocation failed (site set for integral_nodes = " + std::to_string(q) + "); the handle keeps " + std::to_string(E.int_q));
            }
        }
        if (upload_int_rule(E, (int)q)) {
            for (float* b : nbuf) plat_free(b);
            if (E.d_int_xi) upload_int_rule(E, E.int_q);
            return 1;
        }
        E.int_q = (int)q;
        for (size_t t = 0; t < E.terms.size(); ++t) {
            Term& T = E.terms[t];
            if (T.inodes.empty()) continue;
            const int64_t room = T.pts_cap * (int64_t)T.sites();
            T.int_q = E.int_q;
            if (!T.d_pts || T.n <= 0) { T.pts_cap = 0; continue; }
            if (nbuf[t]) {
                plat_d2d(nbuf[t], T.d_pts, sizeof(float) * (size_t)T.n * T.d, E.stream);
                plat_sync(E.stream);
                plat_free(T.d_pts);
                T.d_pts = nbuf[t];
                T.pts_cap = T.n;
            } else T.pts_cap = room / T.sites();
            expand_sites(E, T);
            if (term_installed(E, (int)t)) return 1;
        }
        if (plat_sync(E.stream)) return fail(std::string("device error: ") + plat_last_error());
        return 0;
    }
    if (k == "derivative") {
        if (v == "stencil") return f64_stencil_enable(E, true);
        if (v == "exact") return E.f64 ? f64_stencil_enable(E, false) : 0;
        return fail("pinn_set_option: derivative must be \"exact\" or \"stencil\"");
    }
    if (k == "lbfgs_chunk") {
        char* end = nullptr;
        const long q = std::strtol(v.c_str(), &end, 10);
        if (v.empty() || *end || q < 1 || q > 64) return fail("pinn_set_option: lbfgs_chunk must be an integer in 1..64, not \"" + v + "\"");
        E.lbfgs_chunk = (int)q;
        return 0;
    }
    return fail("pinn_set_option: unknown option \"" + k + "\" (known: gemm, precision, persistent, derivative, integral_nodes, lbfgs_chunk)");
}

int pinn_get_option(pinn_handle h, const char* name, char* buf, int64_t buflen) {
    if (!h || !name || !buf || buflen <= 0) return fail("pinn_get_option: bad argument");
    const std::string k = name;
    if (k == "gemm") { std::snprintf(buf, (size_t)buflen, h->gemm_auto ? "auto(%s)" : "%s", h->gemm == pk::GEMM_FP32 ? "fp32" : "split"); return 0; }
    if (k == "grad_health") { std::snprintf(buf, (size_t)buflen, "%.9g", h->grad_health); return 0; }
    if (k == "gemm_delta") { std::snprintf(buf, (size_t)buflen, "%.9g", h->gemm_delta); return 0; }
    if (k == "precision") { std::snprintf(buf, (size_t)buflen, "%s", h->f64 ? "f64" : "f32"); return 0; }
    if (k == "persistent") { std::snprintf(buf, (size_t)buflen, "%s", h->persistent ? "on" : "off"); return 0; }
    if (k == "integral_nodes") { std::snprintf(buf, (size_t)buflen, "%d", h->int_q); return 0; }
    if (k == "derivative") { std::snprintf(buf, (size_t)buflen, "%s", pe::f64_stencil_on(*h) ? "stencil" : "exact"); return 0; }
    if (k == "eval_path") { std::snprintf(buf, (size_t)buflen, "%s", h->eval_path == 2 ? "one launch" : (h->eval_path == 1 ? "stand-alone kernels" : "none")); return 0; }
    if (k == "f64_path") { std::snprintf(buf, (size_t)buflen, "%s", pe::f64_path(*h)); return 0; }
    if (k == "f64_affine") { std::snprintf(buf, (size_t)buflen, "%d", pe::f64_affine_terms(*h)); return 0; }
    if (k == "f64_merged") { std::snprintf(buf, (size_t)buflen, "%d", pe::f64_merged(*h)); return 0; }
    if (k == "f64_chunks") { std::snprintf(buf, (size_t)buflen, "%d", pe::f64_chunks(*h)); return 0; }
    if (k == "adam_path") { std::snprintf(buf, (size_t)buflen, "%s", h->adam_path == 2 ? "persistent" : (h->adam_path == 1 ? "loop" : "none")); return 0; }
    if (k == "lbfgs_chunk") { std::snprintf(buf, (size_t)buflen, "%d", h->lbfgs_chunk); return 0; }
    if (k == "ens_passes") { std::snprintf(buf, (size_t)buflen, "%d", pe::ens_counter(*h, 0)); return 0; }
    if (k == "ens_point_passes") { std::snprintf(buf, (size_t)buflen, "%d", pe::ens_counter(*h, 1)); return 0; }
    if (k == "ens_scratch_passes") { std::snprintf(buf, (size_t)buflen, "%d", pe::ens_counter(*h, 2)); return 0; }
    return fail("pinn_get_option: unknown option \"" + k + "\" (known: gemm, precision, persistent, derivative, integral_nodes, lbfgs_chunk, grad_health, gemm_delta, adam_path, eval_path, f64_path, f64_merged, f64_chunks, f64_affine, ens_passes, ens_point_passes, ens_scratch_passes)");
}

int pinn_set_timing(pinn_handle h, int level, int group) {
    if (!h) return fail("pinn_set_timing: null handle");
    if (level < 0 || level > 2) return fail("pinn_set_timing: level must be 0, 1 or 2");
    if (group < -1 || group >= (int)h->groups.size()) return fail("pinn_set_timing: group index out of range");
    h->timing_level = level; h->timing_group = group;
    h->timing_valid = false;
    for (auto& G : h->groups) G.timed = false;
    return 0;
}

int pinn_last_timing(pinn_handle h, float* kernel_ms, float* total_ms) {
    if (!h) return fail("null handle");
    if (!h->timing_valid) return fail("no timing available: switch the phase events on (pinn_set_timing(h, 2, -1)), then call pinn_loss_grad");
    plat_event_sync(h->ev3);
    if (kernel_ms) *kernel_ms = plat_event_ms(h->ev1, h->ev2);
    if (total_ms) *total_ms = plat_event_ms(h->ev0, h->ev3);
    return 0;
}

int pinn_num_groups(pinn_handle h) { return h ? (int)h->groups.size() : -1; }

#ifdef PINN_STAMP
int pinn_debug_train_stamps(pinn_handle h, unsigned long long* out4) {
    if (!h || !h->d_bar || !out4) return -1;
    plat_sync(h->stream);
    plat_d2h(out4, h->d_bar + 4, sizeof(unsigned long long) * 4, h->stream);
    plat_sync(h->stream);
    return 0;
}
int pinn_debug_slab(pinn_handle h, int group, int blk, float* dst, int64_t n) {
    if (!h || group < 0 || group >= (int)h->groups.size()) return -1;
// ... 189 lines not shown
```

### neuralpde.jl_amd/csrc/engine_types.hpp

```cpp
#pragma once
#include <algorithm>
#include <cmath>
#include <cstdio>
#include <cstdlib>
#include <map>
#include <memory>
#include <sstream>
#include <string>
#include <type_traits>
#include <vector>

#include "../../include/pinn_hip.h"
#include "aux_limits.hpp"
#include "int_limits.hpp"
#include "plat.hpp"
#include "spec_registry.hpp"

namespace pe {

constexpr int REDUCE_SPLIT = 32;

extern thread_local std::string g_err;
int fail(const std::string& m);

// ... 216 lines not shown
    double* hp_raw = nullptr;
    plat_event ev0, ev1, ev2, ev3;
    plat_stream aux_stream[2] = {nullptr, nullptr};
    plat_event ev_fork, ev_join[aux::MAX_GROUPS];
    float last_kernel_ms = 0.f, last_total_ms = 0.f;
    bool timing_valid = false;
    int timing_level = 0;
    int timing_group = -1;
    float* d_opt_theta = nullptr;
    float* d_opt_m = nullptr;
    float* d_opt_v = nullptr;
    float* d_opt_out = nullptr;
    float* d_w_over_n = nullptr;
    double* d_hist = nullptr;
    size_t hist_cap = 0;
    long long opt_t = 0;
    int adam_path = 0;
    int* d_inv_ptr = nullptr;
    int* d_inv_pos = nullptr;
    bool inv_ok = false;
    int max_contrib = 0, max_inv_pos = 0;
    bool persistent = true;
    float* d_c12 = nullptr;
    size_t c12_cap = 0;
    unsigned* d_bar = nullptr;
    unsigned* h_flag = nullptr;
    unsigned bar_arrivals = 0;
    float* d_sums2 = nullptr;
    int* d_own_r = nullptr;
    int own_blocks = 0, hist_gid = 0;
    void* d_train_samp = nullptr;
    size_t train_samp_cap = 0;
    float* d_opt_bak = nullptr;
    int eval_path = 0;
    int int_q = 16;
    double* d_int_xi = nullptr;
    float* d_int_w = nullptr;
    float* d_phi_pts = nullptr;
    float* d_phi_out = nullptr;
    float* d_phi_scr = nullptr;
    size_t phi_scr_cap = 0;
    int64_t phi_cap = 0;
    int phi_chan = 0;
    pe::HmcState* hmc = nullptr;
    pe::LbfgsState* lbfgs = nullptr;
    int lbfgs_history = 0;
    int lbfgs_chunk = 8;
    pe::EnsState* ens = nullptr;
};

namespace pe {
int parse_descriptor(const char* text, pinn_engine& E);
int apply_embeddings(pinn_engine& E);
struct SexprContext {
    std::vector<std::string> params;
    std::vector<std::string> depvars;
    std::vector<std::vector<std::string>> depvar_inputs;
};
int lower_sexpr_term(const SexprContext& C, const std::vector<std::string>& indvars, const std::string& lhs, const std::string& rhs,
                     int np, Term& T);
void analyse_static(Term& T, int np);
bool fuse_laplacian(Term& T, int np);
int run_loss_grad(pinn_engine& E, const float* d_theta, float* d_out, const float* term_w, int only_term, bool timing, double* lossraw = nullptr,
                  bool packed_fresh = false, bool loss_only = false, float* d_sums = nullptr);
int upload_theta(pinn_engine& E, const float* theta, int64_t p);
void sums_from_double(float* d_out_sums, const double* d_raw, int K, plat_stream st);
int ensure_points(pinn_engine& E);
int eval_and_sync(pinn_engine& E, float* d_out, const float* term_w, double* lossraw, bool timing);
int replan_gemm(pinn_engine& E, int mode);
void pack_all(pinn_engine& E, const float* d_theta = nullptr, bool packed_fresh = false);
inline unsigned sampler_seed(const pinn_engine& E, const Term& T) {
    return E.comm_size > 1 ? T.seed + 0x85EBCA6BU * (unsigned)(E.comm_rank + 1) : T.seed;
}
void redraw_term(pinn_engine& E, Term& T, bool sources);
void measure_grad_health(pinn_engine& E, const float* grad_and_sums, const float* term_w);
int gemm_auto_check(pinn_engine& E, const float* d_theta, const float* term_w, long long now);
int eval_one_launch(pinn_engine& E, float* d_out, const float* term_w, double* lossraw);
inline int check_theta(const pinn_engine& E, const char* who, int64_t p) {
    return p == E.ntheta ? 0 : fail(std::string(who) + ": theta length " + std::to_string(p) + " != ntheta " + std::to_string(E.ntheta));
}
template <class V, class T> class As {
    static constexpr bool same = std::is_same_v<V, std::remove_const_t<T>>;
    T* x_;
    std::vector<V> copy_;
public:
    As(T* x, size_t n) : x_(x) {
        if constexpr (!same) {
            if (x && std::is_const_v<T>) copy_.assign(x, x + n);
            else if (x) copy_.resize(n);
        }
    }
    auto get() {
        if constexpr (same) return x_;
        else return x_ ? copy_.data() : nullptr;
    }
    int put() {
        if constexpr (!same) if (x_) std::copy(copy_.begin(), copy_.end(), x_);
        return 0;
    }
};
template <class V, class T> As<V, T> as(T* x, size_t n) { return As<V, T>(x, n); }
void hmc_free(pinn_engine& E);
void lbfgs_free(pinn_engine& E);
// ... 66 lines not shown
```

### neuralpde.jl_amd/csrc/hmc.cpp

```cpp
#include "resident.hpp"
#include "hmc_kernels.hpp"

using namespace pe;

struct pe::HmcState {
    hmc::Args a;
    ResidentEval ev;
    double* d_state = nullptr;
    double* d_tab = nullptr;
    int* d_kind = nullptr;
    double* d_samples = nullptr; double* d_stat = nullptr; double* d_mom = nullptr; double* d_uni = nullptr;
    size_t samples_cap = 0, stat_cap = 0, mom_cap = 0, uni_cap = 0;
    unsigned long long draws = 0;
};

namespace {

void hmc_release(HmcState* H) {
    if (!H) return;
    H->ev.release();
    plat_free(H->d_state); plat_free(H->d_tab); plat_free(H->d_kind);
    plat_free(H->d_samples); plat_free(H->d_stat); plat_free(H->d_mom); plat_free(H->d_uni);
    delete H;
}
// ... 61 lines not shown
    a.P = (int)p; a.K = K; a.n_prior = n_prior; a.nn = (int)p - n_prior;
    a.sse_roundtrip = f64 ? 1 : 0;
    a.th_cur = H->d_state; a.th_prop = a.th_cur + P; a.r = a.th_prop + P; a.g_cur = a.r + P; a.g_prop = a.g_cur + P;
    double* minv = a.g_prop + P;
    a.minv = minv; a.sc = minv + P;
    a.nn_mu = nn_mu; a.nn_sigma = nn_sigma; a.nn_var = nn_sigma * nn_sigma;
    a.nn_const = (double)a.nn * (std::log(nn_sigma) + 0.5 * std::log(2.0 * 3.14159265358979323846));
    double* tab = H->d_tab;
    a.pr_mu = tab; a.pr_sigma = tab + n_prior; a.lik_c = tab + 2 * n_prior; a.lik_d = a.lik_c + K; a.lik_n = a.lik_d + K;
    a.pr_kind = H->d_kind;
    a.th_eval64 = H->ev.theta64(E);
    a.th_eval32 = H->ev.theta32();
    std::vector<double> st(6 * P + hmc::SC_COUNT, 0.0);
    std::copy(theta, theta + P, st.begin());
    std::copy(theta, theta + P, st.begin() + P);
    std::fill(st.begin() + 5 * P, st.begin() + 6 * P, 1.0);
    std::vector<int> kinds(prior_kind, prior_kind + n_prior);
    if (plat_h2d(H->d_state, st.data(), sizeof(double) * st.size(), E.stream) || plat_h2d(H->d_tab, tb.data(), sizeof(double) * tb.size(), E.stream) ||
        (n_prior > 0 && plat_h2d(H->d_kind, kinds.data(), sizeof(int) * kinds.size(), E.stream)))
        return fail(std::string(who) + ": H2D copy failed");
    if (f64) {
        if (plat_h2d(a.th_eval64, theta, sizeof(double) * P, E.stream)) return fail(std::string(who) + ": H2D copy failed");
    } else {
        std::vector<float> t32(P);
        for (size_t i = 0; i < P; ++i) t32[i] = (float)theta[i];
        if (plat_h2d(a.th_eval32, t32.data(), sizeof(float) * P, E.stream) || plat_sync(E.stream)) return fail(std::string(who) + ": H2D copy failed");
    }
    if (H->ev.eval(E)) return 1;
    hmc_leap(E, *H, true, 0.0, 0.0, 0);
    hmc::launch_energy(a, 1, H->ev.sums(P), E.stream);
    plat_d2d(a.g_cur, a.g_prop, sizeof(double) * P, E.stream);
    plat_d2d(a.sc + hmc::SC_LP_CUR, a.sc + hmc::SC_LP_PROP, sizeof(double), E.stream);
    if (plat_sync(E.stream)) return fail(std::string("device error: ") + plat_last_error());
    hmc_free(E);
    E.hmc = H.release();
    return 0;
}

int pinn_hmc_set_metric(pinn_handle h, const double* inv_metric, int64_t p) {
    const char* who = "pinn_hmc_set_metric";
    if (!h) return fail(std::string(who) + ": null argument");
    pinn_engine& E = *h;
    if (hmc_ready(E, who) || check_theta(E, who, p)) return 1;
    HmcState& H = *E.hmc;
    std::vector<double> m((size_t)p, 1.0);
    for (int64_t i = 0; inv_metric && i < p; ++i) {
        if (!(inv_metric[i] > 0.0) || !std::isfinite(inv_metric[i])) return fail(std::string(who) + ": the inverse metric must be positive and finite");
        m[(size_t)i] = inv_metric[i];
    }
    DeviceScope scope(E.device);
    if (plat_h2d((double*)H.a.minv, m.data(), sizeof(double) * (size_t)p, E.stream) || plat_sync(E.stream)) return fail(std::string(who) + ": H2D copy failed");
    return 0;
}

int pinn_hmc_draws(pinn_handle h, int ndraws, int n_leapfrog, double eps, uint64_t seed, const double* momenta, const double* uniforms,
                   double* samples, int64_t p, double* accept_prob, double* logp) {
    const char* who = "pinn_hmc_draws";
    if (!h || !accept_prob || !logp) return fail(std::string(who) + ": null argument");
    pinn_engine& E = *h;
    if (hmc_ready(E, who) || check_theta(E, who, p) || hmc_refuse_target(E, who)) return 1;
    if (ndraws < 1) return fail(std::string(who) + ": ndraws must be at least 1");
    if (n_leapfrog < 1) return fail(std::string(who) + ": n_leapfrog must be at least 1");
    if (!(eps > 0.0) || !std::isfinite(eps)) return fail(std::string(who) + ": the step size eps must be positive and finite");
    HmcState& H = *E.hmc;
    DeviceScope scope(E.device);
    H.a.th_eval64 = H.ev.theta64(E);
    const size_t P = (size_t)p, nd = (size_t)ndraws;
    if ((samples && !dev_grow(H.d_samples, H.samples_cap, nd * P, E.stream)) || !dev_grow(H.d_stat, H.stat_cap, 2 * nd, E.stream) ||
        (momenta && !dev_grow(H.d_mom, H.mom_cap, nd * P, E.stream)) || (uniforms && !dev_grow(H.d_uni, H.uni_cap, nd, E.stream)))
        return fail(std::string(who) + ": device allocation failed");
    if ((momenta && plat_h2d(H.d_mom, momenta, sizeof(double) * nd * P, E.stream)) || (uniforms && plat_h2d(H.d_uni, uniforms, sizeof(double) * nd, E.stream)))
        return fail(std::string(who) + ": H2D copy failed");
    double* d_acc = H.d_stat;
    double* d_lp = H.d_stat + nd;
    for (int d = 0; d < ndraws; ++d) {
        const unsigned ctr = (unsigned)H.draws;
        hmc::launch_momentum(H.a, momenta ? H.d_mom + (size_t)d * P : nullptr, seed, ctr, E.stream);
        hmc::launch_energy(H.a, 0, nullptr, E.stream);
        hmc_leap(E, H, false, 0.5 * eps, eps, 1);
        for (int s = 0; s < n_leapfrog; ++s) {
            if (H.ev.eval(E)) return 1;
            const bool last = s == n_leapfrog - 1;
            hmc_leap(E, H, true, last ? 0.5 * eps : eps, eps, last ? 0 : 1);
        }
        hmc::launch_energy(H.a, 1, H.ev.sums(P), E.stream);
        hmc::launch_accept(H.a, d, uniforms ? H.d_uni : nullptr, seed, ctr, samples ? H.d_samples : nullptr, d_acc, d_lp, E.stream);
        ++H.draws;
    }
    if ((samples && plat_d2h(samples, H.d_samples, sizeof(double) * nd * P, E.stream)) || plat_d2h(accept_prob, d_acc, sizeof(double) * nd, E.stream) ||
        plat_d2h(logp, d_lp, sizeof(double) * nd, E.stream))
        return fail(std::string(who) + ": D2H copy failed");
    if (plat_sync(E.stream)) return fail(std::string("device error: ") + plat_last_error());
    return 0;
}

int pinn_hmc_get(pinn_handle h, double* theta, int64_t p, double* logp, double* grad) {
    const char* who = "pinn_hmc_get";
    if (!h || !theta) return fail(std::string(who) + ": null argument");
    pinn_engine& E = *h;
    if (hmc_ready(E, who) || check_theta(E, who, p)) return 1;
    HmcState& H = *E.hmc;
    DeviceScope scope(E.device);
    if (plat_d2h(theta, H.a.th_cur, sizeof(double) * (size_t)p, E.stream) || (logp && plat_d2h(logp, H.a.sc + hmc::SC_LP_CUR, sizeof(double), E.stream)) ||
        (grad && plat_d2h(grad, H.a.g_cur, sizeof(double) * (size_t)p, E.stream)) || plat_sync(E.stream))
        return fail(std::string(who) + ": D2H copy failed");
    return 0;
}

}
```

### neuralpde.jl_amd/csrc/lbfgs.cpp

```cpp
#include "resident.hpp"
#include "lbfgs_kernels.hpp"

using namespace pe;

namespace {

struct GemmFloorSwitch {
    pinn_engine& E;
    bool switched = false, armed = false, has_twin = false;
    explicit GemmFloorSwitch(pinn_engine& e) : E(e) {
        for (const NetPlan& NP : E.netplans) has_twin = has_twin || (NP.spec && NP.spec->family == 2 && NP.spec->twin);
    }
    ~GemmFloorSwitch() { if (armed && E.gemm != pk::GEMM_SPLIT) { const std::string keep = g_err; replan_gemm(E, pk::GEMM_SPLIT); if (!keep.empty()) g_err = keep; } }
    bool eligible() const { return !E.f64 && E.gemm == pk::GEMM_SPLIT && !switched && has_twin && std::getenv("PINN_LBFGS_KEEP_GEMM") == nullptr; }
    int engage() {
        if (replan_gemm(E, pk::GEMM_FP32)) { if (E.gemm != pk::GEMM_SPLIT || E.groups.empty()) return 1; g_err.clear(); return 2; }
        switched = E.gemm == pk::GEMM_FP32;
        armed = switched;
        return 0;
    }
    int finish() {
        if (!switched) return 0;
        armed = false;
        return replan_gemm(E, pk::GEMM_SPLIT) ? 1 : 0;
// ... 4 lines not shown

extern "C" {

int pinn_lbfgs(pinn_handle h, double* theta, int64_t p, int maxiters, int history, double gtol, const float* term_w, double* loss_history,
               int* iters_done) {
    if (!h || !theta) return fail("pinn_lbfgs: null argument");
    pinn_engine& E = *h;
    DeviceScope scope(E.device);
    if (p != E.ntheta) return fail("pinn_lbfgs: theta length " + std::to_string(p) + " != ntheta " + std::to_string(E.ntheta));
    if (maxiters <= 0 || history <= 0 || history > 64) return fail("pinn_lbfgs: maxiters must be positive and history in 1..64");
    for (auto& T : E.terms)
        if (T.sampler != 0) return fail("pinn_lbfgs: a term redraws its points on the device; L-BFGS needs a fixed objective (fixed point sets)");
    if (ensure_points(E)) return 1;
    const int K = (int)E.terms.size();
    const size_t P = (size_t)p;
    std::vector<float> th32(P);
    std::vector<double> g(P), x(theta, theta + P), xn(P), gn(P), d(P), q(P);
    auto eval = [&](const std::vector<double>& at, std::vector<double>* grad, double& f) -> int {
        if (E.f64) {
            std::vector<double> w(K, 1.0), L(K);
            if (term_w) for (int k = 0; k < K; ++k) w[k] = term_w[k];
            if (f64_eval(E, at.data(), w.data(), L.data(), grad ? grad->data() : nullptr)) return 1;
            f = 0.0;
            for (int k = 0; k < K; ++k) f += w[k] * L[k];
            return 0;
        }
        for (size_t i = 0; i < P; ++i) th32[i] = (float)at[i];
        if (upload_theta(E, th32.data(), p)) return 1;
        if (grad) {
            if (eval_and_sync(E, E.hp_out, term_w, E.hp_raw, false)) return 1;
        } else {
            if (run_loss_grad(E, E.d_theta, E.hp_out, term_w, -1, false, E.hp_raw, false, true)) return 1;
            if (plat_sync(E.stream)) return fail(std::string("device error: ") + plat_last_error());
        }
        f = 0.0;
        for (int k = 0; k < K; ++k) f += (double)(term_w ? term_w[k] : 1.0f) * E.hp_raw[k] / (double)E.terms[k].n_norm;
        if (grad)
            for (size_t i = 0; i < P; ++i) (*grad)[i] = (double)E.hp_out[i];
        return 0;
    };
    auto dot = [&](const std::vector<double>& a, const std::vector<double>& b) { double s = 0.0; for (size_t i = 0; i < P; ++i) s += a[i] * b[i]; return s; };
    double f = 0.0;
    if (eval(x, &g, f)) return 1;
    std::deque<std::vector<double>> S, Y;
    std::deque<double> RHO;
    GemmFloorSwitch floor_switch(E);
    int it = 0;
    for (; it < maxiters; ++it) {
        double gmax = 0.0;
        for (size_t i = 0; i < P; ++i) gmax = std::max(gmax, std::fabs(g[i]));
        if (!(gmax > gtol)) break;
        q = g;
        std::vector<double> alpha(S.size());
        for (int i = (int)S.size() - 1; i >= 0; --i) {
            alpha[i] = RHO[i] * dot(S[i], q);
            for (size_t j = 0; j < P; ++j) q[j] -= alpha[i] * Y[i][j];
        }
        double gamma = 1.0;
        if (!S.empty()) gamma = dot(S.back(), Y.back()) / dot(Y.back(), Y.back());
        for (size_t j = 0; j < P; ++j) q[j] *= gamma;
        for (size_t i = 0; i < S.size(); ++i) {
            const double beta = RHO[i] * dot(Y[i], q);
            for (size_t j = 0; j < P; ++j) q[j] += (alpha[i] - beta) * S[i][j];
        }
        for (size_t j = 0; j < P; ++j) d[j] = -q[j];
        double gd = dot(g, d);
// ... 54 lines not shown
    double* d_state = nullptr;
    lbfgs::Ctl* d_ctl = nullptr;
    double* d_tab = nullptr;
    double* d_hist = nullptr;
    size_t hist_cap = 0;
};

namespace {

void lbfgs_release(LbfgsState* H) {
    if (!H) return;
    H->ev.release();
    plat_free(H->d_state); plat_free(H->d_ctl); plat_free(H->d_tab); plat_free(H->d_hist);
    delete H;
}

int lbfgs_ready(pinn_engine& E, const char* who) {
    if (!E.lbfgs) return fail(std::string(who) + ": no optimiser state (call pinn_lbfgs_init first)");
    return E.lbfgs->ev.ready(E, who, "pinn_lbfgs_init");
}
int lbfgs_refuse_target(pinn_engine& E, const char* who) {
    return resident_refuse_target(E, who, "the resident L-BFGS loop runs on a single device only", "L-BFGS needs a fixed objective");
}
void lbfgs_step(pinn_engine& E, LbfgsState& H, int mode, int it0, int it_end, double gtol) {
    if (H.ev.f64) lbfgs::launch_step<double>(H.a, H.ev.out<double>(), mode, it0, it_end, gtol, E.stream);
    else lbfgs::launch_step<float>(H.a, H.ev.out<float>(), mode, it0, it_end, gtol, E.stream);
}
int lbfgs_adopt(pinn_engine& E, LbfgsState& H) {
    lbfgs_step(E, H, lbfgs::MODE_LOAD, 0, 0, 0.0);
    if (H.ev.eval(E)) return 1;
    lbfgs_step(E, H, lbfgs::MODE_ADOPT, 0, 0, 0.0);
    if (plat_d2h(&H.ctl, H.d_ctl, sizeof(lbfgs::Ctl), E.stream)) return fail("D2H copy failed");
    if (plat_sync(E.stream)) return fail(std::string("device error: ") + plat_last_error());
    return 0;
}

}

void pe::lbfgs_free(pinn_engine& E) {
    lbfgs_release(E.lbfgs);
    E.lbfgs = nullptr;
    E.lbfgs_history = 0;
}

extern "C" {

int pinn_lbfgs_init(pinn_handle h, const double* theta, int64_t p, int history, const float* term_w) {
    const char* who = "pinn_lbfgs_init";
    if (!h || !theta) return fail(std::string(who) + ": null argument");
    pinn_engine& E = *h;
    if (check_theta(E, who, p)) return 1;
    if (history < 1 || history > lbfgs::MAX_HISTORY) return fail(std::string(who) + ": history must be in 1.." + std::to_string(lbfgs::MAX_HISTORY));
    if (lbfgs_refuse_target(E, who)) return 1;
    DeviceScope scope(E.device);
    if (!E.f64 && ensure_points(E)) return 1;
    const size_t P = (size_t)p, m = (size_t)history;
    const int K = (int)E.terms.size();
    std::unique_ptr<LbfgsState, void (*)(LbfgsState*)> H(new LbfgsState, lbfgs_release);
    const size_t nstate = 4 * P + 2 * m * P + m;
    H->d_state = (double*)plat_malloc(sizeof(double) * nstate);
    H->d_ctl = (lbfgs::Ctl*)plat_malloc(sizeof(lbfgs::Ctl));
    H->d_tab = (double*)plat_malloc(sizeof(double) * (size_t)(2 * K));
    if (!H->d_state || !H->d_ctl || !H->d_tab) return fail(std::string(who) + ": device allocation failed");
    std::vector<double> tb((size_t)(2 * K));
    for (int k = 0; k < K; ++k) {
        tb[k] = term_w ? (double)term_w[k] : 1.0;
// ... 19 lines not shown
    E.lbfgs = H.release();
    E.lbfgs_history = history;
    return 0;
}

int pinn_lbfgs_steps(pinn_handle h, int maxiters, int max_evals, double gtol, double* loss_history, int* iters_done, int* evals_done, int* status) {
    const char* who = "pinn_lbfgs_steps";
    if (!h) return fail(std::string(who) + ": null argument");
    pinn_engine& E = *h;
    if (lbfgs_ready(E, who) || lbfgs_refuse_target(E, who)) return 1;
    if (maxiters < 1) return fail(std::string(who) + ": maxiters must be at least 1");
    if (max_evals < 1) return fail(std::string(who) + ": max_evals must be at least 1");
    LbfgsState& H = *E.lbfgs;
    DeviceScope scope(E.device);
    H.a.th_eval64 = H.ev.theta64(E);
    if (!dev_grow(H.d_hist, H.hist_cap, (size_t)maxiters, E.stream)) return fail(std::string(who) + ": device allocation failed");
    H.a.loss_hist = H.d_hist;
    if (H.ctl.status >= lbfgs::ST_CONVERGED) {
        H.ctl.status = lbfgs::ST_RUN;
        if (plat_h2d(H.d_ctl, &H.ctl, sizeof(lbfgs::Ctl), E.stream) || plat_sync(E.stream)) return fail(std::string(who) + ": H2D copy failed");
    }
    const int it0 = H.ctl.it, it_end = it0 + maxiters, ev0 = H.ctl.evals;
    GemmFloorSwitch floor_switch(E);
    for (;;) {
        const int left = max_evals - (H.ctl.evals - ev0);
        if (left <= 0) break;
        const int n = std::min(E.lbfgs_chunk, left);
        for (int s = 0; s < n; ++s) {
            lbfgs_step(E, H, lbfgs::MODE_SLOT, it0, it_end, gtol);
            if (H.ev.eval(E)) return 1;
        }
        if (plat_d2h(&H.ctl, H.d_ctl, sizeof(lbfgs::Ctl), E.stream)) return fail(std::string(who) + ": D2H copy failed");
        if (plat_sync(E.stream)) return fail(std::string("device error: ") + plat_last_error());
        if (H.ctl.status < lbfgs::ST_CONVERGED) continue;
        if (H.ctl.status == lbfgs::ST_STALLED && floor_switch.eligible()) {
            const int sw = floor_switch.engage();
            if (sw == 1) return 1;
            if (sw == 0 && floor_switch.switched) {
                if (lbfgs_adopt(E, H)) return 1;
                continue;
            }
        }
        break;
    }
    const int done = H.ctl.it - it0;
    if (loss_history) {
        if (done > 0 && (plat_d2h(loss_history, H.d_hist, sizeof(double) * (size_t)done, E.stream) || plat_sync(E.stream))) return fail(std::string(who) + ": D2H copy failed");
        for (int i = done; i < maxiters; ++i) loss_history[i] = H.ctl.f;
    }
    if (iters_done) *iters_done = done;
    if (evals_done) *evals_done = H.ctl.evals - ev0;
    if (status) *status = H.ctl.status;
    return floor_switch.finish();
}

int pinn_lbfgs_get(pinn_handle h, double* theta, int64_t p, double* f, double* grad) {
    const char* who = "pinn_lbfgs_get";
    if (!h || !theta) return fail(std::string(who) + ": null argument");
    pinn_engine& E = *h;
    if (lbfgs_ready(E, who) || check_theta(E, who, p)) return 1;
    LbfgsState& H = *E.lbfgs;
    DeviceScope scope(E.device);
    if (plat_d2h(theta, H.a.x, sizeof(double) * (size_t)p, E.stream) || (grad && plat_d2h(grad, H.a.g, sizeof(double) * (size_t)p, E.stream)) || plat_sync(E.stream))
        return fail(std::string(who) + ": D2H copy failed");
    if (f) *f = H.ctl.f;
    return 0;
// ... 4 lines not shown
```

### neuralpde.jl_amd/csrc/pinn_kernels.hpp

```cpp
#pragma once
#include "rprog.hpp"
#include "vec.hpp"

#ifndef PINN_F1_PREFETCH
#define PINN_F1_PREFETCH 1
#endif
#ifndef PINN_F1_RESIDENT
#define PINN_F1_RESIDENT 3
#endif

namespace pk {
using namespace wv;

enum Act : int { ACT_TANH = 0, ACT_SIGMOID = 1, ACT_SIN = 2,
                 ACT_MIXED = 3 ,
                 ACT_SWISH = 4  };
constexpr int NUM_ACTS = 5;
enum ActClass : int { ACLS_A = 0 ,
                      ACLS_Z_SIN = 1 , ACLS_Z_SWISH = 2  };
constexpr int act_class(int actk) { return actk == ACT_SIN ? ACLS_Z_SIN : (actk == ACT_SWISH ? ACLS_Z_SWISH : ACLS_A); }
constexpr bool act_records_z(int acls) { return acls != ACLS_A; }
enum Variant : int { VARIANT_SIN = 1, VARIANT_MIXED = 2, VARIANT_SWISH = 4 };
enum Mode : int { MODE_FUSED = 0, MODE_RESID = 1, MODE_FWD = 2, MODE_GRADIN = 3, MODE_FWDREC = 4, MODE_GRADREC = 5, MODE_LOSS = 6 };
constexpr bool mode_is_forward_only(int mode) { return mode == MODE_RESID || mode == MODE_FWD || mode == MODE_FWDREC || mode == MODE_LOSS; }

constexpr int MAX_GROUP_TERMS = 12;
constexpr int ND = 8;
constexpr int MAX_PARAMS = 4;
constexpr int LIN_MAX_C = 8, LIN_MAX_SRC = 4;

template <unsigned D1MASK_, unsigned long long PAIRS_, int NPAIR_, unsigned HI_>
struct JetSet {
    static constexpr int popc(unsigned x) { int n = 0; while (x) { n += x & 1; x >>= 1; } return n; }
// ... 126 lines not shown
    int dt;
    int hetero;
    int imap[4];
    const float* pw;
    int linear;
    float lin_k;
    float lin_a[LIN_MAX_C];
    float lin_b[LIN_MAX_SRC];
};

struct GroupArgs {
    const float* packed;
    const float* params;
    const rp::Instr* prog;
    float* slabs;
    double* losspart;
    float* scratch;
    float* rec;
    int nterms_total;
    int nterms;
    int ntiles;
    int nparams;
    int nparams_estim;
    int act;
    int act_layers;
    int dgm_modes;
    int dgm_npad;
    int dgm_slab;
    int dgm_nparams;
    int chain;
    int sub_terms0, sub_tiles0;
    int scr_stride;
    TermDev terms[MAX_GROUP_TERMS];
};

template <class V> DEV V sig_poly6(V s) {
    return vfma(vfma(vfma(vfma(vfma(V(-720.0f), s, V(1800.0f)), s, V(-1560.0f)), s, V(540.0f)), s, V(-62.0f)), s, V(1.0f));
}
template <class V> DEV V sig_poly7(V s) {
    return vfma(vfma(vfma(vfma(vfma(vfma(V(5040.0f), s, V(-15120.0f)), s, V(16800.0f)), s, V(-8400.0f)), s, V(1806.0f)), s, V(-126.0f)), s, V(1.0f));
}
template <int NORD, int ACLS, bool MIXED = false, class V = vfloat>
DEV void act_derivs_n(int act, V a, V (&d)[ND]) {
    if (MIXED) {
        const float m = 2.0f - (float)act, im = 0.5f + 0.5f * (float)act, m2 = m * m;
        const V s = (a + V(m - 1.0f)) * V(im);
        const V s1 = s * (V(1.0f) - s);
        const V s2 = s1 * vfma(V(-2.0f), s, V(1.0f));
        const V s3 = s1 * vfma(V(-6.0f), s1, V(1.0f));
        d[1] = V(m2) * s1;
        d[2] = V(m2 * m) * s2;
        d[3] = V(m2 * m2) * s3;
        if (NORD >= 4) d[4] = V(m2 * m2 * m) * (s2 * vfma(V(-12.0f), s1, V(1.0f)));
        if (NORD >= 5) d[5] = V(m2 * m2 * m2) * vfma(s3, vfma(V(-12.0f), s1, V(1.0f)), V(-12.0f) * s2 * s2);
        if (NORD >= 6) d[6] = V(m2 * m2 * m2 * m) * s1 * sig_poly6(s);
        if (NORD >= 7) d[7] = V(m2 * m2 * m2 * m2) * s1 * sig_poly7(s);
        return;
    }
    if (ACLS == ACLS_Z_SWISH) {
        const V z = a, s = vsigmoid_fast(z);
        const V s1 = s * (V(1.0f) - s);
        const V s2 = s1 * vfma(V(-2.0f), s, V(1.0f));
        const V s3 = s1 * vfma(V(-6.0f), s1, V(1.0f));
        d[1] = vfma(z, s1, s);
        d[2] = vfma(z, s2, V(2.0f) * s1);
        d[3] = vfma(z, s3, V(3.0f) * s2);
// ... 719 lines not shown
```

### neuralpde.jl_amd/csrc/pinn_kernels2.hpp

```cpp
#pragma once
#include "pinn_kernels.hpp"

#if defined(PINN_STAMP) && !defined(PINN_EMU)
#define STAMP_MEMBERS unsigned st_acc[24]; unsigned long long st_last;
#define STAMP_INIT(ac) { for (int i_ = 0; i_ < 24; ++i_) (ac).st_acc[i_] = 0; (ac).st_last = __builtin_amdgcn_s_memtime(); }
#define STAMP(i) { const unsigned long long st_now = __builtin_amdgcn_s_memtime(); ac.st_acc[i] += (unsigned)(st_now - ac.st_last); ac.st_last = st_now; }
#define STAMP_EXTRA 128
#else
#define STAMP_MEMBERS
#define STAMP_INIT(ac)
#define STAMP(i)
#define STAMP_EXTRA 0
#endif

#ifndef PINN_F2_REC_LDS
#define PINN_F2_REC_LDS 1
#endif
#ifndef PINN_F2_SWP
#define PINN_F2_SWP 7
#endif
#ifndef PINN_PROBE
#define PINN_PROBE 0
#endif
#ifndef PINN_F2_ADJ_IL
// ... 1119 lines not shown
        v = row_allsum16(v);
        return v;
    };
    PINN_UNROLL for (int t = 0; t < MTW; ++t)
        PINN_UNROLL for (int r = 0; r < 4; ++r) {
            const vint n = vint(16 * (w * MTW + t) + r) + (g << 2);
            PINN_UNROLL for (int l = 0; l < LH; ++l) gstore_masked(slab + S::O_BH + l * HP, n, reduce_cols(ac.bbar[l][t][r]), c0);
            PINN_UNROLL for (int i = 0; i < D; ++i) gstore_masked(slab + S::O_W1 + i * HP, n, reduce_cols(ac.w1bar[i][t][r]), c0);
            gstore_masked(slab + S::O_WL, n, reduce_cols(ac.wLbar[t][r]), c0);
        }
    static_assert(4 * MAX_PARAMS <= 16, "UB holds the per-wave parameter partials");
    const vbool all = vlt(lane, 64);
    float* UBp = UP + S::NW * NG * 16;
    if (w > 0 && w < PG)
        PINN_UNROLL for (int j = 0; j < MAX_PARAMS; ++j)
            lds_store(UBp, vint(w * MAX_PARAMS + j) + (lane & vint(0)), vfloat((float)wave_sum_d(ac.pbar[j], all)));
    if (PG > 1) wg_barrier();
    if (w == 0) {
        float s = (float)wave_sum_d(ac.bLbar, all);
        gstore_masked(slab + S::O_BL, vint(0), vfloat(s), veq(lane, 0));
        PINN_UNROLL for (int j = 0; j < MAX_PARAMS; ++j) {
            vfloat sp = vfloat((float)wave_sum_d(ac.pbar[j], all));
            PINN_UNROLL for (int ws = 1; ws < PG; ++ws) sp = sp + lds_load(UBp, vint(ws * MAX_PARAMS + j) + (lane & vint(0)));
            gstore_masked(slab + S::O_P, vint(j), sp, veq(lane, 0));
        }
    }
#if defined(PINN_STAMP) && !defined(PINN_EMU)
    STAMP(14)
    if ((threadIdx.x & 63) == 0)
        for (int i = 0; i < 24; ++i) reinterpret_cast<unsigned*>(slab + S::SLAB - 128)[w * 24 + i] = ac.st_acc[i];
#endif
}

template <class S, int MODE, int ACTK>
DEV void wave_main2(const GroupArgs& ga, int blk, int nblocks, int w, float* lds) {
    constexpr bool BWD = (MODE == MODE_FUSED || MODE == MODE_GRADIN || MODE == MODE_GRADREC);
    constexpr bool SUMS = (MODE == MODE_FUSED || MODE == MODE_LOSS);
    const int wave = blk * S::NW + w;
    Acc2<typename S::Shape> ac;
    acc2_init<S>(ac, ga, blk, w, BWD);
    if (SUMS)
        for (int j = 0; j < ga.nterms; ++j) ga.losspart[(size_t)wave * ga.nterms_total + ga.terms[j].term_id] = 0.0;
    wave_tiles2<S, MODE, ACTK>(ga, blk, nblocks, w, lds, ac, 0, ga.nterms, 0, ga.ntiles);
    if (SUMS && ac.cur_term >= 0)
        ga.losspart[(size_t)wave * ga.nterms_total + ga.terms[ac.cur_term].term_id] = wave_sum_dd(ac.lsum, veq(lane_id() >> 4, 0));
    if (!BWD) return;
    acc2_store<S>(ac, ga, blk, w, lds);
}

template <class S0, class S1, int ACTK, int MODE = MODE_FUSED>
DEV void wave_main2m(const GroupArgs& ga, int blk, int nblocks, int w, float* lds) {
    static_assert(same_type<typename S0::Shape, typename S1::Shape>::value, "merged launches need members of one network shape and neuron split");
    static_assert(S0::SLAB == S1::SLAB && S0::PACKED == S1::PACKED, "merged launches share the slab and the packed weight image");
    static_assert(S0::DW_NATURAL == S1::DW_NATURAL && S0::BFX_TR == S1::BFX_TR, "merged launches: one order of the dW tiles in the slab, one exchange-image layout");
    static_assert(MODE == MODE_FUSED || MODE == MODE_LOSS, "merged launches: the fused evaluation and the loss-only evaluation");
    const int wave = blk * S0::NW + w;
    Acc2<typename S0::Shape> ac;
    acc2_init<S0>(ac, ga, blk, w, MODE == MODE_FUSED);
    for (int j = 0; j < ga.nterms; ++j) ga.losspart[(size_t)wave * ga.nterms_total + ga.terms[j].term_id] = 0.0;
    wave_tiles2<S0, MODE, ACTK>(ga, blk, nblocks, w, lds, ac, 0, ga.sub_terms0, 0, ga.sub_tiles0);
    wg_barrier();
    wave_tiles2<S1, MODE, ACTK>(ga, blk, nblocks, w, lds, ac, ga.sub_terms0, ga.nterms, ga.sub_tiles0, ga.ntiles);
    if (ac.cur_term >= 0)
        ga.losspart[(size_t)wave * ga.nterms_total + ga.terms[ac.cur_term].term_id] = wave_sum_dd(ac.lsum, veq(lane_id() >> 4, 0));
    if (MODE != MODE_FUSED) return;
    wg_barrier();
    acc2_store<S0, (S0::PG > S1::PG ? S0::PG : S1::PG)>(ac, ga, blk, w, lds);
}

}
```

Baseline: 236.5 million.

## Fold bf16 weight packing and final reduction into the fused evaluation launch

Moves the bf16 three-piece weight-image pack into the head of the fused kernel: the first workgroups to take a ticket do the packing, and every workgroup spin-waits on a device-scope counter before its tiles. It also moves the slab reduction to the tail, where the last R workgroups to finish wait for all blocks and then run the reduce-one blocks. This removes two separate kernel launches and their launch gaps per evaluation. In exchange it adds cross-workgroup spin waits that depend on the workgroups being co-resident, guarded by a timeout flag the host checks after every sync (il_check), which falls back to the separate kernels.

```diff
diff --git a/neuralpde.jl_amd/csrc/adam.cpp b/neuralpde.jl_amd/csrc/adam.cpp
--- a/neuralpde.jl_amd/csrc/adam.cpp
+++ b/neuralpde.jl_amd/csrc/adam.cpp
@@ -29,6 +29,7 @@
     if (!E.d_opt_theta) return fail("pinn_adam_get: no optimiser state (call pinn_adam_init first)");
     if (plat_d2h(theta, E.d_opt_theta, sizeof(float) * E.ntheta, E.stream)) return fail("D2H copy failed");
     if (plat_sync(E.stream)) return fail(std::string("device error: ") + plat_last_error());
+    if (il_check(E)) return 1;
     return 0;
 }
 
@@ -164,6 +165,7 @@
         E.bar_arrivals = 0;
         plat_memset(E.d_bar, 0, sizeof(unsigned) * 16, E.stream);
         if (plat_sync(E.stream)) return fail(std::string("device error: ") + plat_last_error());
+        if (il_check(E)) return 1;
     }
     for (size_t j = 0; j < G.terms.size(); ++j) {
         const int ti = G.terms[j];
@@ -192,6 +194,7 @@
         if (!E.d_own_r) return fail("device allocation failed (training kernel: thread map)");
         plat_h2d(E.d_own_r, own.data(), sizeof(int) * own.size(), E.stream);
         if (plat_sync(E.stream)) return fail(std::string("device error: ") + plat_last_error());
+        if (il_check(E)) return 1;
         E.own_blocks = G.blocks;
     }
     ta.own_r = E.d_own_r;
@@ -247,6 +250,7 @@
     std::vector<unsigned> draws0(E.terms.size());
     for (size_t t = 0; t < E.terms.size(); ++t) draws0[t] = E.terms[t].draws;
     if (plat_sync(E.stream)) return fail(std::string("device error: ") + plat_last_error());
+    if (il_check(E)) return 1;
     pack_all(E, E.d_opt_theta, false);
     ta.out = E.d_opt_out; ta.lossraw = E.d_lossraw;
     ta.theta = E.d_opt_theta; ta.m = E.d_opt_m; ta.v = E.d_opt_v;
@@ -276,10 +280,12 @@
         G.spec->train(G.ga, ta, G.blocks, E.stream);
     }
     if (plat_sync(E.stream)) return fail(std::string("device error: ") + plat_last_error());
+    if (il_check(E)) return 1;
     if (train_timed_out(E)) {
         opt_snapshot(E, true);
         for (size_t t = 0; t < E.terms.size(); ++t) E.terms[t].draws = draws0[t];
         if (plat_sync(E.stream)) return fail(std::string("device error: ") + plat_last_error());
+        if (il_check(E)) return 1;
         return 2;
     }
     E.opt_t += nsteps;
@@ -311,6 +317,7 @@
     for (int i = 0; i < ndev; ++i) {
         DeviceScope scope(es[i]->device);
         if (plat_sync(es[i]->stream)) return fail(std::string("device error: ") + plat_last_error());
+        if (il_check(*es[i])) return 1;
     }
     return 0;
 }
@@ -321,6 +328,7 @@
     if (!eval_eligible(E)) return 2;
     if (eval_fused(E, E.d_theta, d_out, term_w, lossraw)) return 1;
     if (plat_sync(E.stream)) return fail(std::string("device error: ") + plat_last_error());
+    if (il_check(E)) return 1;
     return train_timed_out(E) ? 2 : 0;
 }
 
diff --git a/neuralpde.jl_amd/csrc/aux_kernels.hpp b/neuralpde.jl_amd/csrc/aux_kernels.hpp
--- a/neuralpde.jl_amd/csrc/aux_kernels.hpp
+++ b/neuralpde.jl_amd/csrc/aux_kernels.hpp
@@ -1,20 +1,13 @@
 #pragma once
 #include <cstdlib>
 #include "aux_limits.hpp"
+#include "inlaunch.hpp"
 #include "int_limits.hpp"
 #include "plat.hpp"
 #include "rprog.hpp"
 #include "sample_rules.hpp"
 
 namespace aux {
-
-#ifdef PINN_EMU
-#define AUX_DEV inline
-#else
-#define AUX_DEV __device__ __forceinline__
-#endif
-
-struct alignas(16) F4 { float x, y, z, w; };
 
 struct Reduce1Args {
     double* tmp[MAX_GROUPS];
@@ -38,20 +31,6 @@
     int skip_grad;
     const int* perm;
 };
-struct ReduceOneArgs {
-    const float* slabs;
-    int slab, nblocks, nent;
-    const int* ent_theta;
-    float* out;
-    float* sums;
-    double* lossraw;
-    int P, K;
-    int nloss;
-    const double* losspart[MAX_GROUPS];
-    int nrows[MAX_GROUPS];
-};
-constexpr int RONE_CHUNKS = 32, RONE_ENT = 32;
-
 struct ExprArgs {
     const float* pts;
     int N, d, nparams, nparams_estim;
@@ -250,56 +229,6 @@
 }
 
 AUX_DEV void sums_from_double_body(int k, float* out_sums, const double* raw) { out_sums[k] = (float)raw[k]; }
-constexpr int PACK_BF_MAX_LAYERS = 16;
-struct PackBfArgs {
-    const float* theta;
-    unsigned* out_fwd;
-    unsigned* out_tr;
-    int nhh, hp;
-    float* packed;
-    const int* idx;
-    int n_gather;
-    int woff[PACK_BF_MAX_LAYERS], nout[PACK_BF_MAX_LAYERS], nin[PACK_BF_MAX_LAYERS];
-};
-AUX_DEV unsigned bf16_rne(float x) {
-    unsigned u;
-    __builtin_memcpy(&u, &x, 4);
-    if ((u & 0x7FFFFFFFu) > 0x7F800000u) return (u >> 16) | 0x40u;
-    u += 0x7FFFu + ((u >> 16) & 1u);
-    return u >> 16;
-}
-AUX_DEV float bf16_val(unsigned h) { const unsigned u = h << 16; float x; __builtin_memcpy(&x, &u, 4); return x; }
-AUX_DEV unsigned bf16_piece(float v, int piece) {
-    const unsigned h = bf16_rne(v);
-    if (piece == 0) return h;
-    const float r = v - bf16_val(h);
-    const unsigned m = bf16_rne(r);
-    if (piece == 1) return m;
-    return bf16_rne(r - bf16_val(m));
-}
-AUX_DEV void pack_bf16_body(int e, const PackBfArgs& a) {
-    const int mt = a.hp / 16, kbn = a.hp / 32;
-    const int total = a.nhh * mt * kbn * 3 * 256;
-    if (e >= 2 * total) return;
-    const bool tr = e >= total;
-    int r = tr ? e - total : e;
-    const int j2 = r & 3; r >>= 2;
-    const int lane = r & 63; r >>= 6;
-    const int piece = r % 3; r /= 3;
-    const int kb = r % kbn; r /= kbn;
-    const int ta = r % mt; r /= mt;
-    const int hl = r;
-    const int g = lane >> 4, c = lane & 15;
-    unsigned word = 0;
-    for (int half = 0; half < 2; ++half) {
-        const int j = 2 * j2 + half;
-        const int other = 16 * (2 * kb + (j >> 2)) + 4 * g + (j & 3), mine = 16 * ta + c;
-        const int out = tr ? other : mine, in = tr ? mine : other;
-        const float v = (out < a.nout[hl] && in < a.nin[hl]) ? a.theta[a.woff[hl] + out + in * a.nout[hl]] : 0.f;
-        word |= bf16_piece(v, piece) << (16 * half);
-    }
-    (tr ? a.out_tr : a.out_fwd)[tr ? e - total : e] = word;
-}
 struct EmbedArgs {
     const float* upts;
     float* pts;
@@ -315,18 +244,9 @@
         a.pts[(size_t)p * a.dx + a.du + k] = (float)(a.is_cos[k] ? cos(ph) : sin(ph));
     }
 }
-AUX_DEV void pack_body(int i, float* packed, const int* idx, const float* theta) {
-    const int j = idx[i];
-    packed[i] = (j >= 0) ? theta[j] : 0.f;
-}
 AUX_DEV void params_body(int j, float* params, const float* theta, const float* defaults, int ne, int p_off) {
     params[j] = (j < ne) ? theta[p_off + j] : defaults[j];
 }
-#ifdef PINN_EMU
-#define AUX_UNROLL8
-#else
-#define AUX_UNROLL8 _Pragma("unroll 8")
-#endif
 AUX_DEV void reduce1_body(int e4, int chunk, int g, const Reduce1Args& a) {
     if (!a.active[g] || chunk >= a.nsplit[g]) return;
     const int nb = a.nblocks[g], ns = a.nsplit[g];
@@ -353,23 +273,6 @@
         out[(size_t)(a.nent[g] + k) * ns] = s;
     }
 }
-AUX_DEV void reduce_one_chunk(int e4, int ch, const ReduceOneArgs& a, double (&s)[4]) {
-    const int per = (a.nblocks + RONE_CHUNKS - 1) / RONE_CHUNKS;
-    const int b0 = ch * per, b1 = (b0 + per < a.nblocks) ? b0 + per : a.nblocks;
-    s[0] = s[1] = s[2] = s[3] = 0.0;
-    const float* p = a.slabs + 4 * e4;
-    AUX_UNROLL8
-    for (int b = b0; b < b1; ++b) {
-        const F4 q = *reinterpret_cast<const F4*>(p + (size_t)b * a.slab);
-        s[0] += (double)q.x; s[1] += (double)q.y; s[2] += (double)q.z; s[3] += (double)q.w;
-    }
-}
-AUX_DEV double reduce_one_loss_part(int k, int t, int nthreads, const ReduceOneArgs& a) {
-    double s = 0.0;
-    for (int i = 0; i < a.nloss; ++i)
-        for (int r = t; r < a.nrows[i]; r += nthreads) s += a.losspart[i][(size_t)r * a.K + k];
-    return s;
-}
 AUX_DEV void reduce2_body(int r, const Reduce2Args& a) {
     if (r < a.P) {
         if (a.skip_grad) return;
@@ -452,9 +355,7 @@
     for (int j = 0; j < np; ++j) params_body(j, params, theta, defaults, ne, p_off);
 }
 inline void launch_pack_bf16(const PackBfArgs& a, plat_stream) {
-    const int total = a.nhh * (a.hp / 16) * (a.hp / 32) * 3 * 256;
-    for (int i = 0; i < a.n_gather; ++i) pack_body(i, a.packed, a.idx, a.theta);
-    for (int e = 0; e < 2 * total; ++e) pack_bf16_body(e, a);
+    for (int e = 0; e < pack_image_elems(a); ++e) pack_image_body(e, a);
 }
 inline void launch_sums_from_double(float* out_sums, const double* raw, int K, plat_stream) {
     for (int k = 0; k < K; ++k) sums_from_double_body(k, out_sums, raw);
@@ -510,26 +411,7 @@
             }
         }
 }
-inline void launch_reduce_one(const ReduceOneArgs& a, plat_stream) {
-    for (int e4 = 0; e4 < a.nent / 4; ++e4) {
-        double tot[4] = {0, 0, 0, 0}, s[4];
-        for (int ch = 0; ch < RONE_CHUNKS; ++ch) {
-            reduce_one_chunk(e4, ch, a, s);
-            for (int e = 0; e < 4; ++e) tot[e] += s[e];
-        }
-        for (int e = 0; e < 4; ++e)
-            if (a.ent_theta[4 * e4 + e] >= 0) a.out[a.ent_theta[4 * e4 + e]] = (float)tot[e];
-    }
-    for (int k = 0; k < a.K; ++k) {
-        double part[256], s = 0.0;
-        for (int t = 0; t < 256; ++t) part[t] = reduce_one_loss_part(k, t, 256, a);
-        for (int st = 128; st >= 1; st >>= 1)
-            for (int t = 0; t < st; ++t) part[t] += part[t + st];
-        s = part[0];
-        a.sums[k] = (float)s;
-        if (a.lossraw) a.lossraw[k] = s;
-    }
-}
+inline void launch_reduce_one(const ReduceOneArgs& a, plat_stream) { reduce_one_all(a); }
 inline void launch_reduce(const Reduce1Args& a1, const Reduce2Args& a2, int max_n1, int max_split, plat_stream) {
     if (reduce_is_small(a1, a2)) {
         for (int r = 0; r < a2.P + a2.K; ++r) reduce_direct_body(r, a1, a2);
@@ -600,14 +482,9 @@
 inline void launch_params(float* params, const float* theta, const float* defaults, int np, int ne, int p_off, plat_stream st) {
     if (np > 0) hipLaunchKernelGGL(k_params, dim3(1), dim3(64), 0, st, params, theta, defaults, np, ne, p_off);
 }
-__global__ void k_pack_bf16(const PackBfArgs a) {
-    const int e = (int)(blockIdx.x * blockDim.x + threadIdx.x);
-    if (e < a.n_gather) pack_body(e, a.packed, a.idx, a.theta);
-    else pack_bf16_body(e - a.n_gather, a);
-}
+__global__ void k_pack_bf16(const PackBfArgs a) { pack_image_body((int)(blockIdx.x * blockDim.x + threadIdx.x), a); }
 inline void launch_pack_bf16(const PackBfArgs& a, plat_stream st) {
-    const int total = a.nhh * (a.hp / 16) * (a.hp / 32) * 3 * 256;
-    hipLaunchKernelGGL(k_pack_bf16, dim3((a.n_gather + 2 * total + 255) / 256), dim3(256), 0, st, a);
+    hipLaunchKernelGGL(k_pack_bf16, dim3((pack_image_elems(a) + 255) / 256), dim3(256), 0, st, a);
 }
 __global__ void k_sums_from_double(float* out_sums, const double* raw, int K) {
     const int k = (int)(blockIdx.x * blockDim.x + threadIdx.x);
@@ -651,43 +528,12 @@
 inline void launch_int_expr(const IntExprArgs& a, int nblocks, plat_stream st) {
     hipLaunchKernelGGL(k_int_expr, dim3(nblocks), dim3(256), 0, st, a);
 }
-__global__ void __launch_bounds__(256) k_reduce_one(const ReduceOneArgs a) {
-    __shared__ double sh[RONE_CHUNKS][RONE_ENT + 1];
-    const int tid = (int)threadIdx.x;
-    const int nentblocks = (a.nent + RONE_ENT - 1) / RONE_ENT;
-    if ((int)blockIdx.x < nentblocks) {
-        const int j = tid & 7, ch = tid >> 3;
-        const int e4 = (int)blockIdx.x * (RONE_ENT / 4) + j;
-        double s[4] = {0.0, 0.0, 0.0, 0.0};
-        if (4 * e4 < a.nent) reduce_one_chunk(e4, ch, a, s);
-        for (int e = 0; e < 4; ++e) sh[ch][4 * j + e] = s[e];
-        __syncthreads();
-        if (tid < RONE_ENT) {
-            const int ent = (int)blockIdx.x * RONE_ENT + tid;
-            if (ent < a.nent) {
-                double tot = 0.0;
-                for (int c2 = 0; c2 < RONE_CHUNKS; ++c2) tot += sh[c2][tid];
-                const int th = a.ent_theta[ent];
-                if (th >= 0) a.out[th] = (float)tot;
-            }
-        }
-    } else {
-        const int k = (int)blockIdx.x - nentblocks;
-        double* part = &sh[0][0];
-        part[tid] = reduce_one_loss_part(k, tid, 256, a);
-        __syncthreads();
-        for (int st = 128; st >= 1; st >>= 1) {
-            if (tid < st) part[tid] += part[tid + st];
-            __syncthreads();
-        }
-        if (tid == 0) {
-            a.sums[k] = (float)part[0];
-            if (a.lossraw) a.lossraw[k] = part[0];
-        }
-    }
+__global__ void __launch_bounds__(RONE_THREADS) k_reduce_one(const ReduceOneArgs a) {
+    __shared__ double sh[RONE_LDS_DOUBLES];
+    reduce_one_block((int)blockIdx.x, (int)threadIdx.x, a, sh);
 }
 inline void launch_reduce_one(const ReduceOneArgs& a, plat_stream st) {
-    hipLaunchKernelGGL(k_reduce_one, dim3((a.nent + RONE_ENT - 1) / RONE_ENT + a.K), dim3(256), 0, st, a);
+    hipLaunchKernelGGL(k_reduce_one, dim3(reduce_one_blocks(a.nent, a.K)), dim3(RONE_THREADS), 0, st, a);
 }
 __global__ void k_reduce_direct(const Reduce1Args a1, const Reduce2Args a2) {
     reduce_direct_body((int)(blockIdx.x * blockDim.x + threadIdx.x), a1, a2);
diff --git a/neuralpde.jl_amd/csrc/comm.cpp b/neuralpde.jl_amd/csrc/comm.cpp
--- a/neuralpde.jl_amd/csrc/comm.cpp
+++ b/neuralpde.jl_amd/csrc/comm.cpp
@@ -307,6 +307,7 @@
     for (int i = 0; i < ndev; ++i) {
         DeviceScope scope(hs[i]->device);
         if (plat_sync(hs[i]->stream)) return fail(std::string("device error: ") + plat_last_error());
+        if (il_check(*hs[i])) return 1;
     }
     if (term_losses) for (int k = 0; k < K; ++k) term_losses[k] = out[(size_t)P + k] / (double)hs[0]->terms[k].n_norm;
     if (grad) std::memcpy(grad, out.data(), sizeof(double) * (size_t)P);
@@ -375,6 +376,7 @@
     for (int i = 0; i < ndev; ++i) {
         DeviceScope scope(hs[i]->device);
         if (plat_sync(hs[i]->stream)) return fail(std::string("device error: ") + plat_last_error());
+        if (il_check(*hs[i])) return 1;
     }
     if (term_losses)
         for (int k = 0; k < K; ++k) term_losses[k] = E0.hp_raw[k] / (double)E0.terms[k].n_norm;
diff --git a/neuralpde.jl_amd/csrc/engine.cpp b/neuralpde.jl_amd/csrc/engine.cpp
--- a/neuralpde.jl_amd/csrc/engine.cpp
+++ b/neuralpde.jl_amd/csrc/engine.cpp
@@ -91,29 +91,37 @@
     return 0;
 }
 
-void pe::pack_all(pinn_engine& E, const float* d_theta, bool packed_fresh) {
+namespace {
+aux::PackBfArgs pack_bf_args(const pinn_engine& E, size_t n, const float* th, bool gather) {
+    const NetPlan& NP = E.netplans[n];
+    const Net& N = E.nets[n];
+    aux::PackBfArgs pa;
+    std::memset(&pa, 0, sizeof pa);
+    pa.theta = th; pa.out_fwd = (unsigned*)(NP.d_packed + NP.spec->OFF_WB); pa.out_tr = (unsigned*)(NP.d_packed + NP.spec->OFF_WTB);
+    pa.nhh = NP.spec->NHH; pa.hp = NP.spec->HP;
+    pa.packed = NP.d_packed; pa.idx = NP.d_pack_idx; pa.n_gather = gather ? NP.spec->OFF_WB : 0;
+    int o = N.theta_off;
+    for (size_t j = 0; j + 1 < N.sizes.size(); ++j) {
+        if (j >= 1 && j <= (size_t)pa.nhh && j - 1 < (size_t)aux::PACK_BF_MAX_LAYERS) { pa.woff[j - 1] = o; pa.nin[j - 1] = N.sizes[j]; pa.nout[j - 1] = N.sizes[j + 1]; }
+        o += N.sizes[j + 1] * N.sizes[j] + N.sizes[j + 1];
+    }
+    return pa;
+}
+}
+
+void pe::pack_all(pinn_engine& E, const float* d_theta, bool packed_fresh, int skip_net) {
     const float* th = d_theta ? d_theta : E.d_theta;
     for (size_t n = 0; n < E.nets.size(); ++n) {
         NetPlan& NP = E.netplans[n];
         if (!NP.spec) continue;
         if (NP.spec->family == 3) { NP.cur = th + E.nets[n].theta_off; continue; }
         NP.cur = NP.d_packed;
+        if ((int)n == skip_net) continue;
         const bool gather = !packed_fresh;
         if (gather && !NP.spec->BFX) aux::launch_pack(NP.d_packed, NP.d_pack_idx, th, NP.npacked, E.stream);
         if (NP.spec->BFX) {
-            const Net& N = E.nets[n];
-            aux::PackBfArgs pa;
-            std::memset(&pa, 0, sizeof pa);
-            pa.theta = th; pa.out_fwd = (unsigned*)(NP.d_packed + NP.spec->OFF_WB); pa.out_tr = (unsigned*)(NP.d_packed + NP.spec->OFF_WTB);
-            pa.nhh = NP.spec->NHH; pa.hp = NP.spec->HP;
-            pa.packed = NP.d_packed; pa.idx = NP.d_pack_idx; pa.n_gather = gather ? NP.spec->OFF_WB : 0;
-            if (pa.nhh > aux::PACK_BF_MAX_LAYERS) return;
-            int o = N.theta_off;
-            for (size_t j = 0; j + 1 < N.sizes.size(); ++j) {
-                if (j >= 1 && j <= (size_t)pa.nhh) { pa.woff[j - 1] = o; pa.nin[j - 1] = N.sizes[j]; pa.nout[j - 1] = N.sizes[j + 1]; }
-                o += N.sizes[j + 1] * N.sizes[j] + N.sizes[j + 1];
-            }
-            aux::launch_pack_bf16(pa, E.stream);
+            if (NP.spec->NHH > aux::PACK_BF_MAX_LAYERS) return;
+            aux::launch_pack_bf16(pack_bf_args(E, n, th, gather), E.stream);
         }
     }
     for (auto& G : E.groups) G.ga.packed = E.netplans[G.net].cur;
@@ -203,9 +211,47 @@
     plat_h2d(E.d_int_xi, xi.data(), sizeof(double) * q, E.stream);
     plat_h2d(E.d_int_w, wf.data(), sizeof(float) * q, E.stream);
     if (plat_sync(E.stream)) return fail(std::string("device error: ") + plat_last_error());
-    return 0;
-}
-
+    if (il_check(E)) return 1;
+    return 0;
+}
+
+}
+
+int pe::il_check(pinn_engine& E) {
+    if (!E.h_il_flag || *(volatile unsigned*)E.h_il_flag == 0u) return 0;
+    E.h_il_flag[0] = 0u;
+    E.il_off = true;
+    std::fprintf(stderr, "[pinn] a bounded wait inside the fused launch (in-launch pack / reduction) timed out; this handle continues with separate launches\n");
+    return fail("the fused launch's in-kernel pack / reduction timed out (its results are invalid); the handle has switched to separate pack, residual and "
+                "reduction launches: repeat the call");
+}
+
+namespace {
+int il_plan(const pinn_engine& E, int only_term, bool loss_only, int* blocks_out) {
+    const char* want = std::getenv("PINN_INLAUNCH");
+    if (!want || want[0] == '0' || want[0] == 0) return -1;
+    if (E.il_off || !E.d_il || loss_only || only_term >= 0 || !E.coupled.empty() || E.nets.size() != 1) return -1;
+    if (std::getenv("PINN_NO_INLAUNCH") || std::getenv("PINN_NO_REDUCE_ONE") || std::getenv("PINN_CONCURRENT_GROUPS")) return -1;
+    int head = 0, blocks = 0;
+    auto fits = [](const pk::SpecInfo* s) { return s && s->family == 2 && s->BFX && s->LDS_WG >= aux::IL_LDS_FLOATS && s->NHH <= aux::PACK_BF_MAX_LAYERS; };
+    if (E.groups.size() == 1) {
+        if (E.groups[0].merged >= 0) return -1;
+        blocks = E.groups[0].blocks;
+    } else if (E.groups.size() == 2) {
+        const int m = E.groups[0].merged;
+        if (m < 0 || m != E.groups[1].merged || std::getenv("PINN_NO_MERGE") || std::getenv("PINN_NO_CHAIN")) return -1;
+        const MergedUnit& mu = E.merged[(size_t)m];
+        head = mu.head;
+        if (head < 0 || mu.tail < 0 || !fits(E.groups[(size_t)mu.tail].spec) || E.groups[(size_t)mu.tail].kind != 0) return -1;
+        blocks = std::max(1, std::min(mu.max_blocks, E.groups[(size_t)head].ga.ntiles + E.groups[(size_t)mu.tail].ga.ntiles));
+    } else return -1;
+    const Group& G = E.groups[(size_t)head];
+    if (G.kind != 0 || !fits(G.spec) || !G.d_ent_theta || !G.ent_covers_theta || G.nent <= 0) return -1;
+    const char* e = std::getenv("PINN_REDUCE_DIRECT_MAX");
+    if (blocks <= (e ? std::atoi(e) : aux::REDUCE_DIRECT_MAX)) return -1;
+    *blocks_out = blocks;
+    return head;
+}
 }
 
 int pe::run_loss_grad(pinn_engine& E, const float* d_theta, float* d_out, const float* term_w, int only_term , bool timing,
@@ -215,8 +261,13 @@
     const int K = (int)E.terms.size();
     const bool phase_ev = timing && E.timing_level >= 2;
     auto group_ev = [&](size_t g) { return timing && E.timing_level >= 1 && (E.timing_group < 0 || E.timing_group == (int)g); };
+    if (il_check(E)) return 1;
+    int il_blocks = 0;
+    const int il_g = il_plan(E, only_term, loss_only, &il_blocks);
+    bool il_launched = false, il_reduces = false;
+    E.launch_path = 1;
     if (phase_ev) plat_event_record(E.ev0, E.stream);
-    pack_all(E, d_theta, packed_fresh);
+    pack_all(E, d_theta, packed_fresh, il_g >= 0 ? E.groups[(size_t)il_g].net : -1);
     if (phase_ev) plat_event_record(E.ev1, E.stream);
     aux::Reduce1Args a1;
     aux::Reduce2Args a2;
@@ -329,6 +380,31 @@
         if (forked) {
             st = E.aux_stream[nforked % 2];
             plat_stream_wait_event(st, E.ev_fork);
+        }
+        if (il_g == (int)g) {
+            if (blocks != il_blocks || chained || forked || (E.groups.size() == 2 && !merged_head))
+                return fail("internal error: the fused launch was planned to pack and reduce in-kernel but is not the launch that was planned");
+            if (ga_launch != &ga_one) { ga_one = *ga_launch; ga_launch = &ga_one; }
+            aux::InLaunch& il = ga_one.il;
+            std::memset(&il, 0, sizeof il);
+            il.on = 1;
+#ifdef PINN_EMU
+            il.nprod = 1; il.R = 1;
+#else
+            const char* re = std::getenv("PINN_INLAUNCH_R");
+            const int capacity = E.ncu * (merged_head ? mu->pair->WG_PER_CU : G.spec->WG_PER_CU);
+            il.nprod = std::min(aux::IL_MAX_PROD, blocks);
+            il.R = std::max(1, std::min(std::min(blocks, capacity), (re && std::atoi(re) > 0) ? std::atoi(re) : aux::IL_MAX_R));
+            if (re && std::atoi(re) == 0 && re[0] == '0') il.R = 0;
+#endif
+            il_reduces = il.R > 0;
+            il.ctr = E.d_il; il.hflag = E.h_il_flag;
+            il.t_start = E.il_start; il.t_packed = E.il_packed; il.t_finish = E.il_finish;
+            E.il_start += (unsigned)blocks; E.il_packed += (unsigned)il.nprod; E.il_finish += (unsigned)blocks;
+            il.pack = pack_bf_args(E, (size_t)G.net, d_theta ? d_theta : E.d_theta, !packed_fresh);
+            il.ent_theta = G.d_ent_theta; il.out = d_out; il.sums = d_sums; il.lossraw = lossraw ? lossraw : E.d_lossraw;
+            il.slab = G.slab_floats; il.nent = G.nent; il.P = (int)E.ntheta; il.K = K;
+            il_launched = true;
         }
         if (group_ev(g)) plat_event_record(G.ev_a, st);
         if (merged_head) mu->pair->launch(*ga_launch, loss_only ? pk::MODE_LOSS : pk::MODE_FUSED, blocks, st);
@@ -403,7 +479,15 @@
     const bool no_reduce_one = std::getenv("PINN_NO_REDUCE_ONE") != nullptr;
     const Group* RG = (nslabsets == 1 && !coupled_active && !loss_only && !no_reduce_one) ? &E.groups[slabset_group] : nullptr;
     const bool one_kernel = ((RG && RG->d_ent_theta && RG->ent_covers_theta) || (loss_only && !no_reduce_one)) && !aux::reduce_is_small(a1, a2);
-    if (one_kernel) {
+    if (il_g >= 0) {
+        if (!il_launched || !one_kernel || RG != &E.groups[(size_t)il_g] || a1.nblocks[il_g] != il_blocks)
+            return fail("internal error: the evaluation planned for the in-kernel reduction is not the one-kernel reduction's");
+        for (int g = 0; g < a2.ngroups; ++g)
+            if (a1.active[g] && g != il_g) return fail("internal error: a second launch's loss partials beside the in-kernel reduction");
+        E.launch_path = 2;
+    }
+    if (il_g >= 0 && il_reduces) {
+    } else if (one_kernel) {
         aux::ReduceOneArgs ro;
         std::memset(&ro, 0, sizeof ro);
         if (RG) { ro.slabs = RG->d_slabs; ro.slab = RG->slab_floats; ro.nblocks = a1.nblocks[slabset_group]; ro.nent = RG->nent; ro.ent_theta = RG->d_ent_theta; }
@@ -470,6 +554,18 @@
         return fail("device allocation failed");
     }
     plat_h2d(E->d_defaults, E->p_defaults32.data(), sizeof(float) * pk::MAX_PARAMS, E->stream);
+    E->d_il = (unsigned*)plat_malloc(sizeof(unsigned) * 4);
+    E->h_il_flag = (unsigned*)plat_host_alloc(sizeof(unsigned) * 4);
+    if (!E->d_il || !E->h_il_flag) {
+        pinn_destroy(E.release());
+        return fail("device allocation failed (in-launch pack / reduction words)");
+    }
+    E->h_il_flag[0] = 0u;
+    plat_memset(E->d_il, 0, sizeof(unsigned) * 4, E->stream);
+    if (plat_sync(E->stream)) {
+        pinn_destroy(E.release());
+        return fail(std::string("device error: ") + plat_last_error());
+    }
     E->hp_theta = (float*)plat_host_alloc(sizeof(float) * (2 * E->ntheta + K + 2) + sizeof(double) * K);
     if (!E->hp_theta) {
         pinn_destroy(E.release());
@@ -504,6 +600,7 @@
     plat_free(E.d_opt_theta); plat_free(E.d_opt_m); plat_free(E.d_opt_v); plat_free(E.d_opt_out); plat_free(E.d_w_over_n); plat_free(E.d_hist); plat_free(E.d_c12); plat_free(E.d_bar); plat_free(E.d_sums2); plat_free(E.d_own_r); plat_free(E.d_train_samp); plat_free(E.d_opt_bak); plat_host_free(E.h_flag);
     plat_free(E.d_theta); plat_free(E.d_params); plat_free(E.d_defaults); plat_free(E.d_lossraw);
     plat_free(E.d_int_xi); plat_free(E.d_int_w);
+    plat_free(E.d_il); plat_host_free(E.h_il_flag);
     plat_free(E.d_out); plat_free(E.d_phi_pts); plat_free(E.d_phi_out); plat_free(E.d_phi_scr);
     plat_host_free(E.hp_theta);
     plat_event_destroy(E.ev0); plat_event_destroy(E.ev1); plat_event_destroy(E.ev2); plat_event_destroy(E.ev3);
@@ -635,6 +732,7 @@
     if (one == 0) { E.eval_path = 2; return 0; }
     if (run_loss_grad(E, E.d_theta, d_out, term_w, -1, timing, lossraw, false, false)) return 1;
     if (plat_sync(E.stream)) return fail(std::string("device error: ") + plat_last_error());
+    if (il_check(E)) return 1;
     return 0;
 }
 
@@ -646,6 +744,7 @@
     } else {
         if (run_loss_grad(E, E.d_theta, E.hp_out, term_w, -1, true, E.hp_raw, false, true)) return 1;
         if (plat_sync(E.stream)) return fail(std::string("device error: ") + plat_last_error());
+        if (il_check(E)) return 1;
     }
     E.timing_valid = E.timing_level >= 2;
     if (term_losses)
@@ -689,6 +788,7 @@
     if (upload_theta(E, theta, E.ntheta)) return 1;
     if (run_loss_grad(E, E.d_theta, E.hp_out, w.data(), -1, false, E.hp_raw)) return 1;
     if (plat_sync(E.stream)) return fail(std::string("device error: ") + plat_last_error());
+    if (il_check(E)) return 1;
     loglik_from_sse(E, stds, E.hp_raw, loglik, grad_std);
     if (grad_theta)
         for (int64_t i = 0; i < E.ntheta; ++i) grad_theta[i] = -E.hp_out[i];
@@ -714,6 +814,7 @@
     for (int k = 0; k < K; ++k) {
         if (run_loss_grad(E, E.d_theta, E.hp_out, nullptr, k, false, E.hp_raw)) return 1;
         if (plat_sync(E.stream)) return fail(std::string("device error: ") + plat_last_error());
+        if (il_check(E)) return 1;
         std::memcpy(term_grads + (size_t)k * p, E.hp_out, sizeof(float) * p);
         if (term_losses) term_losses[k] = E.hp_raw[k] / (double)E.terms[k].n_norm;
     }
@@ -795,6 +896,7 @@
         else aux::launch_expr(expr_args(E, Cp, 0.f, T.d_resid), Cp.blocks, E.stream);
         if (plat_d2h(r, T.d_resid, sizeof(float) * T.n, E.stream)) return fail("D2H copy failed");
         if (plat_sync(E.stream)) return fail(std::string("device error: ") + plat_last_error());
+        if (il_check(E)) return 1;
         { const std::string le = jit_take_launch_error(); if (!le.empty()) return fail("pinn_residual: " + le); }
         return 0;
     }
@@ -809,6 +911,7 @@
     G.spec->launch(ga, pk::MODE_RESID, blocks, E.stream);
     if (plat_d2h(r, T.d_resid, sizeof(float) * T.n, E.stream)) return fail("D2H copy failed");
     if (plat_sync(E.stream)) return fail(std::string("device error: ") + plat_last_error());
+    if (il_check(E)) return 1;
     { const std::string le = jit_take_launch_error(); if (!le.empty()) return fail("pinn_residual: " + le); }
     return 0;
 }
@@ -895,6 +998,7 @@
     if (forward_jets(E, net, sp, theta, pts, n)) return 1;
     if (plat_d2h(out, E.d_phi_out + (size_t)ch * n, sizeof(float) * n, E.stream)) return fail("D2H copy failed");
     if (plat_sync(E.stream)) return fail(std::string("device error: ") + plat_last_error());
+    if (il_check(E)) return 1;
     return 0;
 }
 
@@ -947,6 +1051,7 @@
     T.data_n = n;
     eval_sources(E, T);
     if (plat_sync(E.stream)) return fail(std::string("device error: ") + plat_last_error());
+    if (il_check(E)) return 1;
     return f64_set_point_data(E, term, nullptr);
 }
 int pinn_set_point_data_f64(pinn_handle h, int term, const double* data, int ndata, int64_t n) {
@@ -983,6 +1088,7 @@
         }
         if (plat_h2d(T.d_pw, s.data(), sizeof(float) * (size_t)n, E.stream)) return fail("H2D copy of point weights failed");
         if (plat_sync(E.stream)) return fail(std::string("device error: ") + plat_last_error());
+        if (il_check(E)) return 1;
         T.pw_n = n;
     }
     if (T.coupled < 0) retile(E, T.group);
@@ -999,12 +1105,14 @@
     if (!T.d_pts || n != T.n) return fail("pinn_get_points: the term holds " + std::to_string(T.n) + " points");
     if (plat_d2h(pts, user_pts(T), sizeof(float) * (size_t)n * T.d_user, E.stream)) return fail("D2H copy failed");
     if (plat_sync(E.stream)) return fail(std::string("device error: ") + plat_last_error());
+    if (il_check(E)) return 1;
     return 0;
 }
 
 extern "C++" int pe::replan_gemm(pinn_engine& E, int mode) {
     if (mode == E.gemm) return 0;
     if (plat_sync(E.stream)) return fail(std::string("device error: ") + plat_last_error());
+    if (il_check(E)) return 1;
     const int prev = E.gemm;
     free_plan(E);
     E.gemm = mode;
@@ -1023,6 +1131,7 @@
         if (T.ndata > 0 && T.data_n == T.n && T.n > 0) eval_sources(E, T);
     }
     if (plat_sync(E.stream)) return fail(std::string("device error: ") + plat_last_error());
+    if (il_check(E)) return 1;
     return rc;
 }
 
@@ -1088,6 +1197,7 @@
         const long q = std::strtol(v.c_str(), &end, 10);
         if (v.empty() || *end || q < 2 || q > aux::INT_MAX_Q) return fail("pinn_set_option: integral_nodes must be an integer in 2.." + std::to_string(aux::INT_MAX_Q) + ", not \"" + v + "\"");
         if (plat_sync(E.stream)) return fail(std::string("device error: ") + plat_last_error());
+        if (il_check(E)) return 1;
         for (auto& T : E.terms)
             if (!T.inodes.empty() && T.d_pts && T.n > 0 && T.n * (1 + (int64_t)T.inodes.size() * q) * std::max(T.d, aux::INT_MAX_C) >= (int64_t)1 << 31)
                 return fail("pinn_set_option: integral_nodes = " + std::to_string(q) + " makes a site set of " + std::to_string(T.n * (1 + (int64_t)T.inodes.size() * q)) +
@@ -1130,6 +1240,7 @@
             if (term_installed(E, (int)t)) return 1;
         }
         if (plat_sync(E.stream)) return fail(std::string("device error: ") + plat_last_error());
+        if (il_check(E)) return 1;
         return 0;
     }
     if (k == "derivative") {
@@ -1157,6 +1268,7 @@
     if (k == "persistent") { std::snprintf(buf, (size_t)buflen, "%s", h->persistent ? "on" : "off"); return 0; }
     if (k == "integral_nodes") { std::snprintf(buf, (size_t)buflen, "%d", h->int_q); return 0; }
     if (k == "derivative") { std::snprintf(buf, (size_t)buflen, "%s", pe::f64_stencil_on(*h) ? "stencil" : "exact"); return 0; }
+    if (k == "launch_path") { std::snprintf(buf, (size_t)buflen, "%s", h->launch_path == 2 ? "one launch" : (h->launch_path == 1 ? "separate launches" : "none")); return 0; }
     if (k == "eval_path") { std::snprintf(buf, (size_t)buflen, "%s", h->eval_path == 2 ? "one launch" : (h->eval_path == 1 ? "stand-alone kernels" : "none")); return 0; }
     if (k == "f64_path") { std::snprintf(buf, (size_t)buflen, "%s", pe::f64_path(*h)); return 0; }
     if (k == "f64_affine") { std::snprintf(buf, (size_t)buflen, "%d", pe::f64_affine_terms(*h)); return 0; }
@@ -1167,7 +1279,7 @@
     if (k == "ens_passes") { std::snprintf(buf, (size_t)buflen, "%d", pe::ens_counter(*h, 0)); return 0; }
     if (k == "ens_point_passes") { std::snprintf(buf, (size_t)buflen, "%d", pe::ens_counter(*h, 1)); return 0; }
     if (k == "ens_scratch_passes") { std::snprintf(buf, (size_t)buflen, "%d", pe::ens_counter(*h, 2)); return 0; }
-    return fail("pinn_get_option: unknown option \"" + k + "\" (known: gemm, precision, persistent, derivative, integral_nodes, lbfgs_chunk, grad_health, gemm_delta, adam_path, eval_path, f64_path, f64_merged, f64_chunks, f64_affine, ens_passes, ens_point_passes, ens_scratch_passes)");
+    return fail("pinn_get_option: unknown option \"" + k + "\" (known: gemm, precision, persistent, derivative, integral_nodes, lbfgs_chunk, grad_health, gemm_delta, adam_path, eval_path, launch_path, f64_path, f64_merged, f64_chunks, f64_affine, ens_passes, ens_point_passes, ens_scratch_passes)");
 }
 
 int pinn_set_timing(pinn_handle h, int level, int group) {
diff --git a/neuralpde.jl_amd/csrc/engine_types.hpp b/neuralpde.jl_amd/csrc/engine_types.hpp
--- a/neuralpde.jl_amd/csrc/engine_types.hpp
+++ b/neuralpde.jl_amd/csrc/engine_types.hpp
@@ -272,6 +272,11 @@
     void* d_train_samp = nullptr;
     size_t train_samp_cap = 0;
     float* d_opt_bak = nullptr;
+    unsigned* d_il = nullptr;
+    unsigned* h_il_flag = nullptr;
+    unsigned il_start = 0, il_packed = 0, il_finish = 0;
+    bool il_off = false;
+    int launch_path = 0;
     int eval_path = 0;
     int int_q = 16;
     double* d_int_xi = nullptr;
@@ -308,7 +313,8 @@
 int ensure_points(pinn_engine& E);
 int eval_and_sync(pinn_engine& E, float* d_out, const float* term_w, double* lossraw, bool timing);
 int replan_gemm(pinn_engine& E, int mode);
-void pack_all(pinn_engine& E, const float* d_theta = nullptr, bool packed_fresh = false);
+void pack_all(pinn_engine& E, const float* d_theta = nullptr, bool packed_fresh = false, int skip_net = -1);
+int il_check(pinn_engine& E);
 inline unsigned sampler_seed(const pinn_engine& E, const Term& T) {
     return E.comm_size > 1 ? T.seed + 0x85EBCA6BU * (unsigned)(E.comm_rank + 1) : T.seed;
 }
diff --git a/neuralpde.jl_amd/csrc/hmc.cpp b/neuralpde.jl_amd/csrc/hmc.cpp
--- a/neuralpde.jl_amd/csrc/hmc.cpp
+++ b/neuralpde.jl_amd/csrc/hmc.cpp
@@ -117,6 +117,7 @@
     plat_d2d(a.g_cur, a.g_prop, sizeof(double) * P, E.stream);
     plat_d2d(a.sc + hmc::SC_LP_CUR, a.sc + hmc::SC_LP_PROP, sizeof(double), E.stream);
     if (plat_sync(E.stream)) return fail(std::string("device error: ") + plat_last_error());
+    if (il_check(E)) return 1;
     hmc_free(E);
     E.hmc = H.release();
     return 0;
@@ -176,6 +177,7 @@
         plat_d2h(logp, d_lp, sizeof(double) * nd, E.stream))
         return fail(std::string(who) + ": D2H copy failed");
     if (plat_sync(E.stream)) return fail(std::string("device error: ") + plat_last_error());
+    if (il_check(E)) return 1;
     return 0;
 }
 
diff --git a/neuralpde.jl_amd/csrc/inlaunch.hpp b/neuralpde.jl_amd/csrc/inlaunch.hpp
--- /dev/null
+++ b/neuralpde.jl_amd/csrc/inlaunch.hpp
@@ -0,0 +1,213 @@
+#pragma once
+#include "aux_limits.hpp"
+
+namespace aux {
+
+#ifdef PINN_EMU
+#define AUX_DEV inline
+#define AUX_HD inline
+#else
+#define AUX_DEV __device__ __forceinline__
+#define AUX_HD __host__ __device__ __forceinline__
+#endif
+#ifdef PINN_EMU
+#define AUX_UNROLL8
+#else
+#define AUX_UNROLL8 _Pragma("unroll 8")
+#endif
+
+struct alignas(16) F4 { float x, y, z, w; };
+
+template <int NL> struct ReduceOneArgsT {
+    const float* slabs;
+    int slab, nblocks, nent;
+    const int* ent_theta;
+    float* out;
+    float* sums;
+    double* lossraw;
+    int P, K;
+    int nloss;
+    const double* losspart[NL];
+    int nrows[NL];
+};
+using ReduceOneArgs = ReduceOneArgsT<MAX_GROUPS>;
+constexpr int RONE_CHUNKS = 32, RONE_ENT = 32;
+constexpr int RONE_THREADS = 256;
+
+constexpr int PACK_BF_MAX_LAYERS = 16;
+struct PackBfArgs {
+    const float* theta;
+    unsigned* out_fwd;
+    unsigned* out_tr;
+    int nhh, hp;
+    float* packed;
+    const int* idx;
+    int n_gather;
+    int woff[PACK_BF_MAX_LAYERS], nout[PACK_BF_MAX_LAYERS], nin[PACK_BF_MAX_LAYERS];
+};
+AUX_DEV unsigned bf16_rne(float x) {
+    unsigned u;
+    __builtin_memcpy(&u, &x, 4);
+    if ((u & 0x7FFFFFFFu) > 0x7F800000u) return (u >> 16) | 0x40u;
+    u += 0x7FFFu + ((u >> 16) & 1u);
+    return u >> 16;
+}
+AUX_DEV float bf16_val(unsigned h) { const unsigned u = h << 16; float x; __builtin_memcpy(&x, &u, 4); return x; }
+AUX_DEV unsigned bf16_piece(float v, int piece) {
+    const unsigned h = bf16_rne(v);
+    if (piece == 0) return h;
+    const float r = v - bf16_val(h);
+    const unsigned m = bf16_rne(r);
+    if (piece == 1) return m;
+    return bf16_rne(r - bf16_val(m));
+}
+AUX_HD int pack_bf16_words(const PackBfArgs& a) { return a.nhh * (a.hp / 16) * (a.hp / 32) * 3 * 256; }
+AUX_DEV unsigned pack_bf16_word(int e, const PackBfArgs& a) {
+    const int mt = a.hp / 16, kbn = a.hp / 32;
+    const int total = pack_bf16_words(a);
+    const bool tr = e >= total;
+    int r = tr ? e - total : e;
+    const int j2 = r & 3; r >>= 2;
+    const int lane = r & 63; r >>= 6;
+    const int piece = r % 3; r /= 3;
+    const int kb = r % kbn; r /= kbn;
+    const int ta = r % mt; r /= mt;
+    const int hl = r;
+    const int g = lane >> 4, c = lane & 15;
+    unsigned word = 0;
+    for (int half = 0; half < 2; ++half) {
+        const int j = 2 * j2 + half;
+        const int other = 16 * (2 * kb + (j >> 2)) + 4 * g + (j & 3), mine = 16 * ta + c;
+        const int out = tr ? other : mine, in = tr ? mine : other;
+        const float v = (out < a.nout[hl] && in < a.nin[hl]) ? a.theta[a.woff[hl] + out + in * a.nout[hl]] : 0.f;
+        word |= bf16_piece(v, piece) << (16 * half);
+    }
+    return word;
+}
+AUX_DEV void pack_body(int i, float* packed, const int* idx, const float* theta) {
+    const int j = idx[i];
+    packed[i] = (j >= 0) ? theta[j] : 0.f;
+}
+AUX_HD int pack_image_elems(const PackBfArgs& a) { return a.n_gather + 2 * pack_bf16_words(a); }
+AUX_DEV unsigned pack_image_value(int e, const PackBfArgs& a) {
+    if (e >= pack_image_elems(a)) return 0u;
+    if (e >= a.n_gather) return pack_bf16_word(e - a.n_gather, a);
+    const int j = a.idx[e];
+    const float v = (j >= 0) ? a.theta[j] : 0.f;
+    unsigned u;
+    __builtin_memcpy(&u, &v, 4);
+    return u;
+}
+AUX_DEV void pack_image_store(int e, const PackBfArgs& a, unsigned u) {
+    if (e >= pack_image_elems(a)) return;
+    if (e >= a.n_gather) {
+        const int w = e - a.n_gather, total = pack_bf16_words(a);
+        (w >= total ? a.out_tr : a.out_fwd)[w >= total ? w - total : w] = u;
+        return;
+    }
+    float v;
+    __builtin_memcpy(&v, &u, 4);
+    a.packed[e] = v;
+}
+AUX_DEV void pack_image_body(int e, const PackBfArgs& a) { pack_image_store(e, a, pack_image_value(e, a)); }
+
+template <int NL> AUX_DEV void reduce_one_chunk(int e4, int ch, const ReduceOneArgsT<NL>& a, double (&s)[4]) {
+    const int per = (a.nblocks + RONE_CHUNKS - 1) / RONE_CHUNKS;
+    const int b0 = ch * per, b1 = (b0 + per < a.nblocks) ? b0 + per : a.nblocks;
+    s[0] = s[1] = s[2] = s[3] = 0.0;
+    const float* p = a.slabs + 4 * e4;
+    AUX_UNROLL8
+    for (int b = b0; b < b1; ++b) {
+        const F4 q = *reinterpret_cast<const F4*>(p + (size_t)b * a.slab);
+        s[0] += (double)q.x; s[1] += (double)q.y; s[2] += (double)q.z; s[3] += (double)q.w;
+    }
+}
+template <int NL> AUX_DEV double reduce_one_loss_part(int k, int t, int nthreads, const ReduceOneArgsT<NL>& a) {
+    double s = 0.0;
+    const int nloss = NL == 1 ? 1 : a.nloss;
+    for (int i = 0; i < nloss; ++i)
+        for (int r = t; r < a.nrows[i]; r += nthreads) s += a.losspart[i][(size_t)r * a.K + k];
+    return s;
+}
+constexpr int reduce_one_blocks(int nent, int K) { return (nent + RONE_ENT - 1) / RONE_ENT + K; }
+constexpr int RONE_LDS_DOUBLES = RONE_CHUNKS * (RONE_ENT + 1);
+
+#ifdef PINN_EMU
+template <int NL> inline void reduce_one_all(const ReduceOneArgsT<NL>& a) {
+    for (int e4 = 0; e4 < a.nent / 4; ++e4) {
+        double tot[4] = {0, 0, 0, 0}, s[4];
+        for (int ch = 0; ch < RONE_CHUNKS; ++ch) {
+            reduce_one_chunk(e4, ch, a, s);
+            for (int e = 0; e < 4; ++e) tot[e] += s[e];
+        }
+        for (int e = 0; e < 4; ++e)
+            if (a.ent_theta[4 * e4 + e] >= 0) a.out[a.ent_theta[4 * e4 + e]] = (float)tot[e];
+    }
+    for (int k = 0; k < a.K; ++k) {
+        double part[RONE_THREADS], s = 0.0;
+        for (int t = 0; t < RONE_THREADS; ++t) part[t] = reduce_one_loss_part(k, t, RONE_THREADS, a);
+        for (int st = RONE_THREADS / 2; st >= 1; st >>= 1)
+            for (int t = 0; t < st; ++t) part[t] += part[t + st];
+        s = part[0];
+        a.sums[k] = (float)s;
+        if (a.lossraw) a.lossraw[k] = s;
+    }
+}
+#else
+template <int NL> AUX_DEV void reduce_one_block(int vb, int tid, const ReduceOneArgsT<NL>& a, double* shp) {
+    double (*sh)[RONE_ENT + 1] = reinterpret_cast<double (*)[RONE_ENT + 1]>(shp);
+    const int nentblocks = (a.nent + RONE_ENT - 1) / RONE_ENT;
+    const bool live = tid < RONE_THREADS;
+    if (vb < nentblocks) {
+        if (live) {
+            const int j = tid & 7, ch = tid >> 3;
+            const int e4 = vb * (RONE_ENT / 4) + j;
+            double s[4] = {0.0, 0.0, 0.0, 0.0};
+            if (4 * e4 < a.nent) reduce_one_chunk(e4, ch, a, s);
+            for (int e = 0; e < 4; ++e) sh[ch][4 * j + e] = s[e];
+        }
+        __syncthreads();
+        if (tid < RONE_ENT) {
+            const int ent = vb * RONE_ENT + tid;
+            if (ent < a.nent) {
+                double tot = 0.0;
+                for (int c2 = 0; c2 < RONE_CHUNKS; ++c2) tot += sh[c2][tid];
+                const int th = a.ent_theta[ent];
+                if (th >= 0) a.out[th] = (float)tot;
+            }
+        }
+    } else {
+        const int k = vb - nentblocks;
+        double* part = shp;
+        if (live) part[tid] = reduce_one_loss_part(k, tid, RONE_THREADS, a);
+        __syncthreads();
+        for (int st = RONE_THREADS / 2; st >= 1; st >>= 1) {
+            if (tid < st) part[tid] += part[tid + st];
+            __syncthreads();
+        }
+        if (tid == 0) {
+            a.sums[k] = (float)part[0];
+            if (a.lossraw) a.lossraw[k] = part[0];
+        }
+    }
+}
+#endif
+
+constexpr int IL_MAX_PROD = 16, IL_MAX_R = 128;
+constexpr unsigned IL_SPIN_LIMIT = 1u << 21;
+constexpr int IL_LDS_FLOATS = 16 + 2 * RONE_LDS_DOUBLES;
+struct InLaunch {
+    int on;
+    int nprod, R;
+    unsigned t_start, t_packed, t_finish;
+    unsigned* ctr;
+    unsigned* hflag;
+    PackBfArgs pack;
+    const int* ent_theta;
+    float* out;
+    float* sums;
+    double* lossraw;
+    int slab, nent, P, K;
+};
+
+}
diff --git a/neuralpde.jl_amd/csrc/lbfgs.cpp b/neuralpde.jl_amd/csrc/lbfgs.cpp
--- a/neuralpde.jl_amd/csrc/lbfgs.cpp
+++ b/neuralpde.jl_amd/csrc/lbfgs.cpp
@@ -60,6 +60,7 @@
         } else {
             if (run_loss_grad(E, E.d_theta, E.hp_out, term_w, -1, false, E.hp_raw, false, true)) return 1;
             if (plat_sync(E.stream)) return fail(std::string("device error: ") + plat_last_error());
+            if (il_check(E)) return 1;
         }
         f = 0.0;
         for (int k = 0; k < K; ++k) f += (double)(term_w ? term_w[k] : 1.0f) * E.hp_raw[k] / (double)E.terms[k].n_norm;
@@ -180,6 +181,7 @@
     lbfgs_step(E, H, lbfgs::MODE_ADOPT, 0, 0, 0.0);
     if (plat_d2h(&H.ctl, H.d_ctl, sizeof(lbfgs::Ctl), E.stream)) return fail("D2H copy failed");
     if (plat_sync(E.stream)) return fail(std::string("device error: ") + plat_last_error());
+    if (il_check(E)) return 1;
     return 0;
 }
 
@@ -265,6 +267,7 @@
         }
         if (plat_d2h(&H.ctl, H.d_ctl, sizeof(lbfgs::Ctl), E.stream)) return fail(std::string(who) + ": D2H copy failed");
         if (plat_sync(E.stream)) return fail(std::string("device error: ") + plat_last_error());
+        if (il_check(E)) return 1;
         if (H.ctl.status < lbfgs::ST_CONVERGED) continue;
         if (H.ctl.status == lbfgs::ST_STALLED && floor_switch.eligible()) {
             const int sw = floor_switch.engage();
diff --git a/neuralpde.jl_amd/csrc/pinn_kernels.hpp b/neuralpde.jl_amd/csrc/pinn_kernels.hpp
--- a/neuralpde.jl_amd/csrc/pinn_kernels.hpp
+++ b/neuralpde.jl_amd/csrc/pinn_kernels.hpp
@@ -1,4 +1,5 @@
 #pragma once
+#include "inlaunch.hpp"
 #include "rprog.hpp"
 #include "vec.hpp"
 
@@ -191,6 +192,7 @@
     int sub_terms0, sub_tiles0;
     int scr_stride;
     TermDev terms[MAX_GROUP_TERMS];
+    aux::InLaunch il;
 };
 
 template <class V> DEV V sig_poly6(V s) {
diff --git a/neuralpde.jl_amd/csrc/pinn_kernels2.hpp b/neuralpde.jl_amd/csrc/pinn_kernels2.hpp
--- a/neuralpde.jl_amd/csrc/pinn_kernels2.hpp
+++ b/neuralpde.jl_amd/csrc/pinn_kernels2.hpp
@@ -1175,20 +1175,102 @@
 #endif
 }
 
+#ifdef PINN_EMU
+inline void il_head(const GroupArgs& ga, int blk, int w, float*) {
+    if (blk < ga.il.nprod && w == 0)
+        for (int e = blk; e < aux::pack_image_elems(ga.il.pack); e += ga.il.nprod) aux::pack_image_body(e, ga.il.pack);
+}
+inline void il_wait_packed(const GroupArgs&, float*) { wg_barrier(); }
+#else
+DEV void il_head(const GroupArgs& ga, int, int, float* lds) {
+    const aux::InLaunch& il = ga.il;
+    unsigned* word = reinterpret_cast<unsigned*>(lds);
+    if (threadIdx.x == 0) *word = __hip_atomic_fetch_add(il.ctr, 1u, __ATOMIC_RELAXED, __HIP_MEMORY_SCOPE_AGENT) - il.t_start;
+    __syncthreads();
+    const unsigned ticket = *word;
+    if (ticket < (unsigned)il.nprod) {
+        const int n = aux::pack_image_elems(il.pack), stride = il.nprod * (int)blockDim.x;
+        for (int e0 = (int)ticket * (int)blockDim.x + (int)threadIdx.x; e0 < n; e0 += 8 * stride) {
+            unsigned v[8];
+            PINN_UNROLL for (int u = 0; u < 8; ++u) v[u] = aux::pack_image_value(e0 + u * stride, il.pack);
+            PINN_UNROLL for (int u = 0; u < 8; ++u) aux::pack_image_store(e0 + u * stride, il.pack, v[u]);
+        }
+        asm volatile("s_waitcnt vmcnt(0)" ::: "memory");
+        __syncthreads();
+        if (threadIdx.x == 0) {
+            __builtin_amdgcn_fence(__ATOMIC_RELEASE, "agent");
+            asm volatile("s_waitcnt vmcnt(0)" ::: "memory");
+            __hip_atomic_fetch_add(il.ctr + 1, 1u, __ATOMIC_RELAXED, __HIP_MEMORY_SCOPE_AGENT);
+        }
+    }
+}
+DEV void il_spin(const unsigned* c, unsigned target, unsigned* hflag) {
+    unsigned spins = 0;
+    while ((int)(__hip_atomic_load(c, __ATOMIC_RELAXED, __HIP_MEMORY_SCOPE_AGENT) - target) < 0) {
+        __builtin_amdgcn_s_sleep(1);
+        if (++spins > aux::IL_SPIN_LIMIT) { __hip_atomic_store(hflag, 1u, __ATOMIC_RELAXED, __HIP_MEMORY_SCOPE_SYSTEM); break; }
+    }
+    __builtin_amdgcn_fence(__ATOMIC_ACQUIRE, "agent");
+    asm volatile("s_waitcnt vmcnt(0)" ::: "memory");
+}
+DEV void il_wait_packed(const GroupArgs& ga, float*) {
+    const aux::InLaunch& il = ga.il;
+    if (threadIdx.x == 0) il_spin(il.ctr + 1, il.t_packed + (unsigned)il.nprod, il.hflag);
+    __syncthreads();
+}
+#endif
+template <int NW>
+DEV void il_tail(const GroupArgs& ga, int blk, int nblocks, int w, float* lds) {
+    const aux::InLaunch& il = ga.il;
+    aux::ReduceOneArgsT<1> ro = {};
+    ro.slabs = ga.slabs; ro.slab = il.slab; ro.nblocks = nblocks; ro.nent = il.nent; ro.ent_theta = il.ent_theta;
+    ro.out = il.out; ro.sums = il.sums; ro.lossraw = il.lossraw; ro.P = il.P; ro.K = il.K;
+    ro.nloss = 1; ro.losspart[0] = ga.losspart; ro.nrows[0] = nblocks * NW;
+#ifdef PINN_EMU
+    wg_barrier();
+    if (blk == nblocks - 1 && w == 0) aux::reduce_one_all(ro);
+#else
+    unsigned* word = reinterpret_cast<unsigned*>(lds);
+    asm volatile("s_waitcnt vmcnt(0)" ::: "memory");
+    __syncthreads();
+    if (threadIdx.x == 0) {
+        __builtin_amdgcn_fence(__ATOMIC_RELEASE, "agent");
+        asm volatile("s_waitcnt vmcnt(0)" ::: "memory");
+        *word = __hip_atomic_fetch_add(il.ctr + 2, 1u, __ATOMIC_RELAXED, __HIP_MEMORY_SCOPE_AGENT) - il.t_finish;
+    }
+    __syncthreads();
+    const int rank = (int)*word - (nblocks - il.R);
+    if (rank < 0) return;
+    if (threadIdx.x == 0) il_spin(il.ctr + 2, il.t_finish + (unsigned)nblocks, il.hflag);
+    __syncthreads();
+    double* sh = reinterpret_cast<double*>(lds + 16);
+    const int nvb = aux::reduce_one_blocks(ro.nent, ro.K);
+    for (int vb = rank; vb < nvb; vb += il.R) {
+        aux::reduce_one_block(vb, (int)threadIdx.x, ro, sh);
+        __syncthreads();
+    }
+#endif
+}
+template <class S, int MODE> constexpr bool il_compiled() { return MODE == MODE_FUSED && S::BFIMG && S::LDS_WG >= aux::IL_LDS_FLOATS; }
+
 template <class S, int MODE, int ACTK>
 DEV void wave_main2(const GroupArgs& ga, int blk, int nblocks, int w, float* lds) {
     constexpr bool BWD = (MODE == MODE_FUSED || MODE == MODE_GRADIN || MODE == MODE_GRADREC);
     constexpr bool SUMS = (MODE == MODE_FUSED || MODE == MODE_LOSS);
     const int wave = blk * S::NW + w;
+    const bool il = il_compiled<S, MODE>() && ga.il.on;
+    if (il) il_head(ga, blk, w, lds);
     Acc2<typename S::Shape> ac;
     acc2_init<S>(ac, ga, blk, w, BWD);
     if (SUMS)
         for (int j = 0; j < ga.nterms; ++j) ga.losspart[(size_t)wave * ga.nterms_total + ga.terms[j].term_id] = 0.0;
+    if (il) il_wait_packed(ga, lds);
     wave_tiles2<S, MODE, ACTK>(ga, blk, nblocks, w, lds, ac, 0, ga.nterms, 0, ga.ntiles);
     if (SUMS && ac.cur_term >= 0)
         ga.losspart[(size_t)wave * ga.nterms_total + ga.terms[ac.cur_term].term_id] = wave_sum_dd(ac.lsum, veq(lane_id() >> 4, 0));
     if (!BWD) return;
     acc2_store<S>(ac, ga, blk, w, lds);
+    if (il) il_tail<S::NW>(ga, blk, nblocks, w, lds);
 }
 
 template <class S0, class S1, int ACTK, int MODE = MODE_FUSED>
@@ -1198,9 +1280,12 @@
     static_assert(S0::DW_NATURAL == S1::DW_NATURAL && S0::BFX_TR == S1::BFX_TR, "merged launches: one order of the dW tiles in the slab, one exchange-image layout");
     static_assert(MODE == MODE_FUSED || MODE == MODE_LOSS, "merged launches: the fused evaluation and the loss-only evaluation");
     const int wave = blk * S0::NW + w;
+    const bool il = il_compiled<S0, MODE>() && il_compiled<S1, MODE>() && ga.il.on;
+    if (il) il_head(ga, blk, w, lds);
     Acc2<typename S0::Shape> ac;
     acc2_init<S0>(ac, ga, blk, w, MODE == MODE_FUSED);
     for (int j = 0; j < ga.nterms; ++j) ga.losspart[(size_t)wave * ga.nterms_total + ga.terms[j].term_id] = 0.0;
+    if (il) il_wait_packed(ga, lds);
     wave_tiles2<S0, MODE, ACTK>(ga, blk, nblocks, w, lds, ac, 0, ga.sub_terms0, 0, ga.sub_tiles0);
     wg_barrier();
     wave_tiles2<S1, MODE, ACTK>(ga, blk, nblocks, w, lds, ac, ga.sub_terms0, ga.nterms, ga.sub_tiles0, ga.ntiles);
@@ -1209,6 +1294,7 @@
     if (MODE != MODE_FUSED) return;
     wg_barrier();
     acc2_store<S0, (S0::PG > S1::PG ? S0::PG : S1::PG)>(ac, ga, blk, w, lds);
+    if (il) il_tail<S0::NW>(ga, blk, nblocks, w, lds);
 }
 
 }
```

After: 234.1 million. -1.0%, worse.
